# anands-repo/hello

Measured on AMD Instinct MI355X. Metric: candidate sites/sec (whole node), higher is better.
Workload: dtype f32

## Files before the change

hello_amd/compiler.py:

```python
from __future__ import annotations

from dataclasses import dataclass, field
from typing import Dict, List, Optional, Tuple

import numpy as np

from . import netspec as ns
from . import weights as wts

ROWS_READS0, ROWS_READS1, ROWS_ALLELES, ROWS_SITES = 0, 1, 2, 3
SEG_R0A, SEG_R1A, SEG_AS = 0, 1, 2
BUF_NONE, BUF_READS0, BUF_READS1, BUF_REF, BUF_FIRST_SCRATCH = -1, 0, 1, 2, 3
OP_XATTN_FRONT = 11
(OP_CONV1D, OP_MAXPOOL, OP_SEGSUM, OP_MIX, OP_HEAD, OP_CONCAT, OP_ADD, OP_READCONV_FUSED, OP_LAYERNORM,
 OP_COMPRESSOR_FUSED) = range(1, 11)
FLAG_RELU, FLAG_SRC_U8, FLAG_SOFTMAX, FLAG_MIX_REST, FLAG_SOFTPLUS, FLAG_WINOGRAD, FLAG_BF16X3, FLAG_BF16X3_32 = 1, 2, 4, 8, 16, 32, 64, 128
FLAG_LANE_SHIFT, MAX_LANES = 8, 8
OP_NAMES = {1: "conv1d", 2: "maxpool", 3: "segsum", 4: "mix", 5: "head", 6: "concat", 7: "add",
            8: "readconv_fused", 9: "layernorm", 10: "compressor_fused", 11: "xattn_front"}


@dataclass
class Value:
    vid: int
    domain: int
    length: int
    channels: int
    u8: bool = False

    @property
    def floats_per_row(self):
        return self.length * self.channels


@dataclass
class Op:
    kind: int
    domain: int
    src0: int = BUF_NONE
    src1: int = BUF_NONE
    dst: int = BUF_NONE
    res: int = BUF_NONE
    cin: int = 0
    cout: int = 0
    k: int = 0
    stride: int = 1
    pad: int = 0
    lin: int = 0
    lout: int = 0
    flags: int = 0
    seg: int = 0
    c1: int = 0
    a0: float = 0.0
    a1: float = 0.0
    w_off: int = 0
    b_off: int = 0
    name: str = ""
    macs_per_row: int = 0
    exec_macs_per_row: float = 0.0


@dataclass
class Program:
    spec_name: str
    window: int
    channels0: int
    channels1: int
    n_experts: int
    has_meta: bool
    uses_ref: bool
    ops: List[Op]
    buffers: List[Tuple[int, int]]
    weights: np.ndarray
    fused_read_convolver: bool = False
    fused_compressor: bool = False
    winograd: bool = False
    arithmetic: str = "fp32"
    n_lanes: int = 1

    def describe(self) -> str:
        lines = [f"program {self.spec_name}: {len(self.ops)} ops, {len(self.buffers)} buffers, "
                 f"{self.weights.nbytes / 1e6:.2f} MB weights"]
        for i, o in enumerate(self.ops):
            lines.append(f"  {i:3d} {OP_NAMES[o.kind]:14s} dom={o.domain} {o.src0}->{o.dst} "
                         f"cin={o.cin} cout={o.cout} k={o.k} s={o.stride} L {o.lin}->{o.lout} {o.name}")
        return "\n".join(lines)


class _WeightBlob:
    def __init__(self):
        self.parts: List[np.ndarray] = []
        self.size = 0

    def add(self, arr: np.ndarray) -> int:
        arr = np.ascontiguousarray(arr, dtype=np.float32).ravel()
        pad = (-self.size) % 4
        if pad:
            self.parts.append(np.zeros(pad, np.float32))
            self.size += pad
        off = self.size
        self.parts.append(arr)
        self.size += arr.size
        return off

    def finish(self) -> np.ndarray:
        return np.concatenate(self.parts) if self.parts else np.zeros(0, np.float32)


def grouped_native(node) -> bool:
    return (node.groups > 1 and node.cin % node.groups == 0 and node.cout % node.groups == 0
            and (node.cout // node.groups) % 128 == 0 and (node.cin // node.groups) % 16 == 0)


def pack_conv(w: np.ndarray, b: np.ndarray, groups: int = 1, expand: bool = True):
    cout, cg, k = w.shape
    cin = cg * groups if expand else cg
    dense = np.zeros((cout, cin, k), np.float32)
    og = cout // groups
    if expand:
        for g in range(groups):
            dense[g * og:(g + 1) * og, g * cg:(g + 1) * cg] = w[g * og:(g + 1) * og]
    else:
        dense[:] = w
    kreal = k * cin
    kpad = -(-kreal // 32) * 32
    cpad = -(-cout // 32) * 32
    packed = np.zeros((cpad, kpad), np.float32)
    packed[:cout, :kreal] = dense.transpose(0, 2, 1).reshape(cout, kreal)
    bias = np.zeros(cpad, np.float32)
    bias[:cout] = b
    return packed, bias


def winograd_outputs_per_tile(length: int) -> int:
    return 3 if length % 3 == 0 else 2


from .readconv_pack import winograd_taps_f33


def pack_conv_winograd(w: np.ndarray, b: np.ndarray, length: int):
    from .readconv_pack import winograd_taps
    cout, cin, k = w.shape
    assert k == 3 and cin % 8 == 0
    u = winograd_taps_f33(w) if winograd_outputs_per_tile(length) == 3 else winograd_taps(w)
    t = u.shape[-1]
    packed = u.reshape(cout, cin // 8, 8, t).transpose(0, 1, 3, 2).reshape(cout, t * cin)
    return np.ascontiguousarray(packed, dtype=np.float32), b.astype(np.float32)


def _canonical_read_convolver_extras(nodes, cin, act="relu") -> int:
    try:
        ref = ns.read_convolver("x", in_channels=cin, act=act)
    except Exception:
        return -1

    def sig(n):
        if isinstance(n, ns.Conv):
            return ("c", n.cin, n.cout, n.k, n.stride, n.pad, n.groups, n.act, n.norm == "ln")
        if isinstance(n, ns.MaxPool):
            return ("p", n.k, n.stride, n.pad)
        if isinstance(n, ns.Residual):
            return ("r", tuple(sig(m) for m in n.body), tuple(sig(m) for m in n.shortcut))
        return ("?", type(n).__name__)

    if len(nodes) < len(ref) or cin not in (6, 7):
        return -1
    if not all(sig(a) == sig(b) for a, b in zip(nodes, ref)):
        return -1
    extras = nodes[len(ref):]
    if not all(sig(x) == sig(ref[-1]) for x in extras):
        return -1
    return len(extras)


def _is_canonical_read_convolver(nodes, cin) -> bool:
    return _canonical_read_convolver_extras(nodes, cin) == 0


ARITHMETICS = ("fp32", "bf16x3", "bf16x3+32")


class _Lowering:
    def __init__(self, spec: ns.ModelSpec, state, fused: bool, winograd: bool = True, arithmetic: str = "fp32"):
        if arithmetic not in ARITHMETICS:
            raise ValueError(f"arithmetic must be one of {ARITHMETICS}, not {arithmetic!r}")
        self.arithmetic = arithmetic
        self.used_bf16x3 = False
        self.used_xattn_front = False
        self.spec = spec
        self.state = state
        self.folded = wts.fold(spec, state)
        self.fused = fused
        self.winograd = bool(winograd)
        self.ops: List[Op] = []
        self.values: Dict[int, Value] = {}
        self.blob = _WeightBlob()
        self.next_vid = 1000
        self.used_fused = False
        self.used_fused_compressor = False
        self.uses_ref = False

    def new(self, domain, length, channels) -> Value:
        v = Value(self.next_vid, domain, length, channels)
        self.values[v.vid] = v
        self.next_vid += 1
        return v

    def input(self, buf, domain, length, channels) -> Value:
        v = Value(buf, domain, length, channels, u8=True)
        self.values[buf] = v
        return v

    @staticmethod
    def _winograd_ok(node: ns.Conv, x: Value) -> bool:
        return (node.k == 3 and node.stride == 1 and node.pad == 1 and (node.groups == 1 or grouped_native(node))
                and node.dilation == 1 and not x.u8 and node.cin % 8 == 0 and node.cout % 64 == 0)

    def conv(self, node: ns.Conv, x: Value, res: Optional[Value] = None) -> Value:
        if node.act not in ("relu", "none", "softplus"):
            raise NotImplementedError(f"activation {node.act!r} is not implemented by the HIP engine")
        if node.dilation != 1:
            raise NotImplementedError("dilated convs are not implemented by the HIP engine")
        assert x.channels == node.cin, (node.key, x.channels, node.cin)
        w, b = self.folded[node.key]
        wino = self.winograd and self._winograd_ok(node, x)
        native = grouped_native(node) and not x.u8
        packed, bias = (pack_conv_winograd(w, b, x.length) if wino else pack_conv(w, b, node.groups, expand=not native))
        lout = ns.out_length([node], x.length)
        m = winograd_outputs_per_tile(lout)
        y = self.new(x.domain, lout, node.cout)
        act_flag = {"relu": FLAG_RELU, "softplus": FLAG_SOFTPLUS, "none": 0}[node.act]
        layer_norm = node.norm == "ln"
        self.ops.append(Op(
            OP_CONV1D, x.domain, src0=x.vid, dst=y.vid, res=res.vid if (res is not None and not layer_norm) else BUF_NONE,
            cin=node.cin, cout=node.cout, k=node.k, stride=node.stride, pad=node.pad,
            lin=x.length, lout=lout,
            flags=(0 if layer_norm else act_flag) | (FLAG_SRC_U8 if x.u8 else 0) | (FLAG_WINOGRAD if wino else 0),
            c1=node.groups if native else 0,
            w_off=self.blob.add(packed), b_off=self.blob.add(bias), name=node.key,
            macs_per_row=lout * node.cout * (node.cin // node.groups) * node.k,
            exec_macs_per_row=float(-(-lout // m) * (m + 2) * node.cout * (node.cin // node.groups)) if wino else 0.0))
        if layer_norm:
            gamma, beta, eps = wts.layer_norm_params(node, self.state)
            z = self.new(x.domain, lout, node.cout)
            self.ops.append(Op(OP_LAYERNORM, x.domain, src0=y.vid, dst=z.vid, res=res.vid if res is not None else BUF_NONE,
                               cin=node.cout, cout=node.cout, lin=lout, lout=lout, flags=act_flag, a0=float(eps),
                               w_off=self.blob.add(gamma), b_off=self.blob.add(beta), name=node.bn_key + ".normer"))
            return z
        return y

    def net(self, nodes, x, head_slot: Optional[int] = None, softmax=False):
        from . import readconv_pack
        if (self.fused is True and self.winograd and isinstance(x, Value) and not x.u8 and (x.length, x.channels) == (36, 64)
                and readconv_pack.compressor_blocks(nodes) in readconv_pack.COMPRESSOR_BLOCKS):
            blocks = readconv_pack.compressor_blocks(nodes)
            y = self.new(x.domain, 18, 128)
            w_off = self.blob.add(readconv_pack.pack_compressor(nodes, self.folded))
            self.ops.append(Op(OP_COMPRESSOR_FUSED, x.domain, src0=x.vid, dst=y.vid, cin=64, cout=128, k=blocks, lin=36, lout=18,
                               flags=FLAG_WINOGRAD | FLAG_RELU, w_off=w_off, b_off=w_off, name=nodes[0].key.rsplit(".network", 1)[0],
                               macs_per_row=ns.macs(nodes, 36), exec_macs_per_row=readconv_pack.compressor_executed_macs(blocks)))
            self.used_fused_compressor = True
            return y
        front = readconv_pack.xattn_front_match(nodes) if (self.fused is True and self.winograd and isinstance(x, tuple)) else None
        if front is not None:
            allele, sites = x
            site = sites[front[0].pick]
            if (site is not None and (allele.length, allele.channels) == (18, 128) and allele.domain == ROWS_ALLELES
                    and site.domain == ROWS_SITES):
                mix, conv11, blk = front
                y2, sc = self.new(ROWS_ALLELES, 9, 256), self.new(ROWS_ALLELES, 9, 256)
                w_off = self.blob.add(readconv_pack.pack_xattn_front(conv11, blk, self.folded))
                self.ops.append(Op(OP_XATTN_FRONT, ROWS_ALLELES, src0=allele.vid, src1=site.vid, dst=y2.vid, res=sc.vid,
                                   cin=128, cout=256, k=3, stride=2, pad=1, lin=18, lout=9, flags=FLAG_RELU, seg=SEG_AS,
                                   a0=float(mix.coeffs[0]), a1=float(mix.coeffs[1]), w_off=w_off, b_off=w_off,
                                   name=conv11.key.rsplit(".network", 1)[0] + ".front",
                                   macs_per_row=ns.macs([conv11], 18) + ns.macs([blk.body[0]], 18) + ns.macs(blk.shortcut, 18),
                                   exec_macs_per_row=readconv_pack.xattn_front_executed_macs()))
                self.used_xattn_front = True
                x = self.conv(blk.body[1], y2, res=sc)
                nodes = nodes[3:]
        for node in nodes:
            if isinstance(node, ns.Conv):
                x = self.conv(node, x)
            elif isinstance(node, ns.MaxPool):
                lout = ns.out_length([node], x.length)
                y = self.new(x.domain, lout, x.channels)
                self.ops.append(Op(OP_MAXPOOL, x.domain, src0=x.vid, dst=y.vid, cin=x.channels,
                                   cout=x.channels, k=node.k, stride=node.stride, pad=node.pad,
                                   lin=x.length, lout=lout))
                x = y
            elif isinstance(node, ns.Residual):
                short = self.net(node.shortcut, x) if node.shortcut else x
                h = x
                for i, sub in enumerate(node.body):
                    last = i == len(node.body) - 1
                    if not isinstance(sub, ns.Conv):
                        raise NotImplementedError("residual bodies must be conv stacks")
                    h = self.conv(sub, h, res=short if last else None)
                x = h
            elif isinstance(node, ns.Head):
                w, b = self.folded[node.key]
                assert head_slot is not None
                self.ops.append(Op(OP_HEAD, x.domain, src0=x.vid, dst=head_slot, cin=x.channels,
                                   cout=node.cout, lin=x.length, lout=1,
                                   flags=FLAG_SOFTMAX if softmax else 0,
                                   w_off=self.blob.add(w), b_off=self.blob.add(b), name=node.key,
                                   macs_per_row=node.cin * node.cout))
                x = None
            elif isinstance(node, ns.Mix):
                allele, sites = x
                site = sites[node.pick]
                assert site is not None and site.domain == ROWS_SITES and allele.domain == ROWS_ALLELES
                y = self.new(ROWS_ALLELES, allele.length, allele.channels)
# ... 27 lines not shown
    def add(self, a: Value, b: Value) -> Value:
        y = self.new(a.domain, a.length, a.channels)
        self.ops.append(Op(OP_ADD, a.domain, src0=a.vid, src1=b.vid, dst=y.vid, cin=a.channels,
                           lin=a.length, lout=a.length))
        return y

    def read_frames(self, tech: int, stem: str = "read_convolver", suffix: str = "") -> Value:
        spec = self.spec
        name = f"{stem}{tech}{suffix}"
        nodes = spec.nets[name]
        cin = spec.channels[tech]
        buf = BUF_READS0 if tech == 0 else BUF_READS1
        dom = ROWS_READS0 if tech == 0 else ROWS_READS1
        seg = SEG_R0A if tech == 0 else SEG_R1A
        x = self.input(buf, dom, spec.window, cin)
        from . import readconv_pack
        extras = _canonical_read_convolver_extras(nodes, cin)
        softplus = False
        if extras < 0 and _canonical_read_convolver_extras(nodes, cin, "softplus") == 0:
            extras, softplus = 0, True
        fusable = (self.fused and readconv_pack.AVAILABLE and extras in readconv_pack.EXTRA_BLOCKS
                   and spec.window in readconv_pack.WINDOWS)
        if fusable and (spec.window != 150 or softplus):
            fusable = self.fused is True and self.winograd and extras == 0 and not (softplus and spec.window != 150)
        wide_blocks = readconv_pack.wide_trunk_nodes(nodes, cin)
        if (self.fused in (True, "trunk") and self.winograd and spec.window == 150 and wide_blocks is not None
                and readconv_pack.AVAILABLE):
            y = self.new(ROWS_ALLELES, 36, 128)
            w_off = self.blob.add(readconv_pack.pack_wide(nodes, wide_blocks, self.folded))
            if self.fused == "trunk":
                pooled = self.net(nodes[:readconv_pack.TRUNK_FIRST_NODE], x)
                assert (pooled.length, pooled.channels) == (71, 64)
                self.ops.append(Op(OP_READCONV_FUSED, ROWS_ALLELES, src0=pooled.vid, dst=y.vid, cin=64, cout=128, k=0, lin=71,
                                   lout=36, seg=seg, w_off=w_off, b_off=w_off, name=name + ".trunk", flags=FLAG_WINOGRAD,
                                   macs_per_row=ns.macs(wide_blocks, 71),
                                   exec_macs_per_row=readconv_pack.wide_trunk_executed_macs()))
            else:
                self.ops.append(Op(OP_READCONV_FUSED, ROWS_ALLELES, src0=buf, dst=y.vid, cin=cin, cout=128, k=0, lin=spec.window,
                                   lout=36, seg=seg, w_off=w_off, b_off=w_off, name=name, flags=FLAG_SRC_U8 | FLAG_WINOGRAD,
                                   macs_per_row=ns.macs(nodes, spec.window),
                                   exec_macs_per_row=readconv_pack.wide_executed_macs(cin)))
            self.used_fused = True
            return y
        if fusable:
            _, l1, _, l2, _, _ = readconv_pack.geometry(spec.window)
            y = self.new(ROWS_ALLELES, l2, 64)
            packed = readconv_pack.pack(nodes, self.folded, cin, winograd=self.winograd, window=spec.window)
            wflag = FLAG_WINOGRAD if self.winograd else 0
            if (self.arithmetic != "fp32" and self.fused is True and self.winograd and spec.window == 150 and extras == 0
                    and not softplus):
                packed = np.concatenate([packed, readconv_pack.pack_bf16x3(nodes, self.folded)])
                wflag |= FLAG_BF16X3 | (FLAG_BF16X3_32 if "+32" in self.arithmetic else 0)
                self.used_bf16x3 = True
            w_off = self.blob.add(packed)
            if self.fused == "trunk":
                pooled = self.net(nodes[:readconv_pack.TRUNK_FIRST_NODE], x)
                assert (pooled.length, pooled.channels) == (l1, 32)
                self.ops.append(Op(OP_READCONV_FUSED, ROWS_ALLELES, src0=pooled.vid, dst=y.vid, cin=32, cout=64,
                                   k=extras, lin=l1, lout=l2, seg=seg, w_off=w_off, b_off=w_off, name=name + ".trunk",
                                   flags=wflag,
                                   macs_per_row=ns.macs(nodes[readconv_pack.TRUNK_FIRST_NODE:], l1)))
            else:
                self.ops.append(Op(OP_READCONV_FUSED, ROWS_ALLELES, src0=buf, dst=y.vid, cin=cin, cout=64,
                                   k=extras, lin=spec.window, lout=l2, seg=seg, w_off=w_off, b_off=w_off, name=name,
                                   flags=FLAG_SRC_U8 | wflag | (FLAG_SOFTPLUS if softplus else 0),
                                   macs_per_row=ns.macs(nodes, spec.window),
                                   exec_macs_per_row=readconv_pack.executed_macs_per_read(self.winograd, extras,
                                                                                          spec.window)))
            self.used_fused = True
            return y
        return self.segsum(self.net(nodes, x), seg)

    def compress_and_predict(self, frames: Value, idx: int, slot: Optional[int]):
        spec = self.spec
        comp = spec.nets[f"compressor{idx}"]
        ca = self.net(comp, frames)
        xattn = f"xattn{idx}"
        needs_cs0 = spec.has(xattn) and any(isinstance(n, ns.Mix) and n.pick == 0 for n in spec.nets[xattn])
        cs0 = self.net(comp, self.segsum(frames, SEG_AS)) if needs_cs0 else None
        cs1 = self.segsum(ca, SEG_AS)
        if spec.has(xattn):
            self.net(spec.nets[xattn], (ca, (cs0, cs1)), head_slot=slot)
        return (cs0, cs1), ca

    def lower_merged(self):
        spec = self.spec
        hybrid = spec.has("readConv1")
        additive = spec.use_additive
        if hybrid and not additive:
            raise ValueError("hybrid MoEMergedAdvanced with useAdditive=False: the reference's own forward raises on it "
                             "(MixtureOfExpertsAdvanced.py:436)")

        def mix(allele: Value, site: Value, a0, a1, flags=0) -> Value:
            x = self.new(ROWS_ALLELES, allele.length, allele.channels)
            self.ops.append(Op(OP_MIX, ROWS_ALLELES, src0=allele.vid, src1=site.vid, dst=x.vid,
                               cin=allele.channels, lin=allele.length, lout=allele.length,
                               a0=a0, a1=a1, seg=SEG_AS, flags=flags))
            return x

        def expert(idx, allele: Value, site: Value):
            from . import readconv_pack
            nodes = spec.nets[f"expert{idx}"]
            front = (readconv_pack.xattn_front_match(nodes, mixed_ahead=True)
                     if (additive and self.fused is True and self.winograd
                         and (allele.length, allele.channels) == (18, 128)) else None)
            if front is not None:
                _, conv11, blk = front
                y2, sc = self.new(ROWS_ALLELES, 9, 256), self.new(ROWS_ALLELES, 9, 256)
                w_off = self.blob.add(readconv_pack.pack_xattn_front(conv11, blk, self.folded))
                self.ops.append(Op(OP_XATTN_FRONT, ROWS_ALLELES, src0=allele.vid, src1=site.vid, dst=y2.vid, res=sc.vid,
                                   cin=128, cout=256, k=3, stride=2, pad=1, lin=18, lout=9, flags=FLAG_RELU | FLAG_MIX_REST, seg=SEG_AS,
                                   a0=2.0, a1=-1.0, w_off=w_off, b_off=w_off, name=conv11.key.rsplit(".network", 1)[0] + ".front",
                                   macs_per_row=ns.macs([conv11], 18) + ns.macs([blk.body[0]], 18) + ns.macs(blk.shortcut, 18),
                                   exec_macs_per_row=readconv_pack.xattn_front_executed_macs()))
                self.used_xattn_front = True
                self.net(nodes[2:], self.conv(blk.body[1], y2, res=sc), head_slot=idx)
                return
            if additive:
                x = mix(allele, site, 2.0, -1.0, FLAG_MIX_REST)
            else:
                rest = mix(allele, site, -1.0, 1.0)
# ... 170 lines not shown
        ready = [i for i in range(n) if i not in done and preds[i] <= done]
        pick = max(ready, key=lambda i: (bottom[i], -i))
        done.add(pick)
        order.append(pick)
    return [ops[i] for i in order]


def _allocate(ops: List[Op], values: Dict[int, Value], reuse: bool = True):
    last_use: Dict[int, int] = {}
    for i, o in enumerate(ops):
        for v in (o.src0, o.src1, o.res):
            if v >= 1000:
                last_use[v] = i
    phys: List[Tuple[int, int]] = [(0, 0)] * BUF_FIRST_SCRATCH
    free: Dict[int, List[int]] = {d: [] for d in range(4)}
    assigned: Dict[int, int] = {}
    def place(vid):
        v = values[vid]
        need = v.floats_per_row
        pool = free[v.domain]
        if pool:
            fits = [p for p in pool if phys[p][1] >= need]
            pick = min(fits, key=lambda p: phys[p][1]) if fits else max(pool, key=lambda p: phys[p][1])
            pool.remove(pick)
            phys[pick] = (v.domain, max(phys[pick][1], need))
        else:
            pick = len(phys)
            phys.append((v.domain, need))
        assigned[vid] = pick

    for i, o in enumerate(ops):
        if o.kind == OP_XATTN_FRONT:
            place(o.dst)
            place(o.res)
            for vsrc in {o.src0, o.src1}:
                if reuse and vsrc >= 1000 and last_use.get(vsrc) == i and vsrc in assigned:
                    free[values[vsrc].domain].append(assigned[vsrc])
            continue
        if o.kind != OP_HEAD:
            place(o.dst)
        for vsrc in {o.src0, o.src1, o.res}:
            if reuse and vsrc >= 1000 and last_use.get(vsrc) == i and vsrc in assigned:
                free[values[vsrc].domain].append(assigned[vsrc])
    for o in ops:
        o.src0 = assigned.get(o.src0, o.src0)
        o.src1 = assigned.get(o.src1, o.src1)
        o.res = assigned.get(o.res, o.res)
        if o.kind != OP_HEAD:
            o.dst = assigned[o.dst]
    return phys


def compile_model(spec: ns.ModelSpec, state, fused: bool = True, winograd: bool = True, arithmetic: str = "fp32",
                  fold_site_sums: bool = True, lanes: bool = False) -> Program:
    low = _Lowering(spec, state, fused, winograd, arithmetic)
    n_experts, has_meta = low.lower()
    if arithmetic != "fp32" and not low.used_bf16x3:
        raise ValueError("arithmetic='bf16x3' / 'bf16x3+32' exists for the canonical 150 bp ReLU read convolver in the whole-kernel "
                         "Winograd form (fused=True, winograd=True): this model / these options do not run it")
    if fold_site_sums:
        low.ops = _fold_site_sums(low.ops)
        low.ops = _fold_concats(low.ops)
    n_lanes = assign_lanes(low.ops) if lanes else 1
    if n_lanes > 1:
        low.ops = schedule_lanes(low.ops)
    buffers = _allocate(low.ops, low.values, reuse=n_lanes == 1)
    return Program(
        spec_name=spec.name, window=spec.window, channels0=spec.channels[0],
        channels1=spec.channels[1] if spec.hybrid_inputs else 0,
        n_experts=n_experts, has_meta=has_meta, uses_ref=low.uses_ref, ops=low.ops,
        buffers=buffers, weights=low.blob.finish(), fused_read_convolver=low.used_fused,
        fused_compressor=low.used_fused_compressor, winograd=low.winograd, arithmetic=arithmetic, n_lanes=n_lanes)
```

hello_amd/csrc/engine.hip:

```cpp
#include <hip/hip_runtime.h>

#include <cstdarg>
#include <cstdio>
#include <cstring>
#include <new>
#include <stdexcept>
#include <string>
#include <vector>

#include "../../include/hello_mi355x.h"
#include "kernels.h"

namespace {

thread_local std::string g_last_error;

int fail(int code, const char* fmt, ...) {
    char buf[512];
    va_list ap;
    va_start(ap, fmt);
    vsnprintf(buf, sizeof(buf), fmt, ap);
    va_end(ap);
    g_last_error = buf;
    return code;
// ... 305 lines not shown
                                             "and cout / groups a multiple of 128 (a workgroup's channel block lies inside one group)", i, o.c1);
            if ((o.lin + 2 * o.pad - o.k) / o.stride + 1 != o.lout)
                return fail(HELLO_ERR_MODEL, "op %d: lout inconsistent", i);
            if (o.flags & (HELLO_FLAG_BF16X3 | HELLO_FLAG_BF16X3_32))
                return fail(HELLO_ERR_MODEL, "op %d: the bf16x3 arithmetic modes exist for the fused read convolver only (ABI 2 "
                                             "dropped the split-operand CONV1D)", i);
        }
        if (o.kind == HELLO_OP_COMPRESSOR_FUSED &&
            !(o.cin == 64 && o.cout == 128 && o.lin == 36 && o.lout == 18 && hello::compressor_supports_blocks(o.k) &&
              (o.flags & HELLO_FLAG_WINOGRAD) && o.w_off >= 0))
            return fail(HELLO_ERR_MODEL, "op %d: the fused compressor maps [36][64] rows to [18][128] with 2 to 4 identity blocks, "
                                         "Winograd form", i);
        if (o.kind == HELLO_OP_XATTN_FRONT &&
            !(o.domain == HELLO_ROWS_ALLELES && o.cin == 128 && o.cout == 256 && o.lin == 18 && o.lout == 9 && o.k == 3 && o.stride == 2 &&
              o.pad == 1 && o.seg == HELLO_SEG_ALLELES_TO_SITES && o.w_off >= 0 &&
              o.res >= HELLO_BUF_FIRST_SCRATCH && o.res != o.dst && o.res != o.src0 && o.res != o.src1 && o.dst != o.src0 && o.dst != o.src1 &&
              d->buffers[o.res].domain == HELLO_ROWS_ALLELES && d->buffers[o.res].floats_per_row >= 9 * 256 &&
              (o.src1 == HELLO_BUF_NONE || d->buffers[o.src1].domain == HELLO_ROWS_SITES)))
            return fail(HELLO_ERR_MODEL, "op %d: the fused expert front maps [18][128] allele rows (src0) and site rows (src1, or none: "
                                         "the sites' sums of src0) to two distinct [9][256] allele buffers, dst and res", i);
        if (o.kind == HELLO_OP_LAYERNORM && (o.cin <= 0 || o.cin > 512 || o.lin <= 0 || o.w_off < 0 || o.b_off < 0 || !(o.a0 > 0.f)))
            return fail(HELLO_ERR_MODEL, "op %d: bad LayerNorm (1..512 channels, eps > 0)", i);
        if ((o.kind == HELLO_OP_SEGSUM || o.kind == HELLO_OP_MIX || o.kind == HELLO_OP_READCONV_FUSED) &&
            (o.seg < 0 || o.seg > 2))
            return fail(HELLO_ERR_MODEL, "op %d: bad segment kind", i);
        if (o.kind == HELLO_OP_CONV1D && (o.flags & HELLO_FLAG_WINOGRAD) &&
            !(o.k == 3 && o.stride == 1 && o.pad == 1 && o.lin == o.lout && !(o.flags & HELLO_FLAG_SRC_U8) &&
              o.cin % 8 == 0 && o.cout % 64 == 0))
            return fail(HELLO_ERR_MODEL, "op %d: this convolution has no Winograd form (needs k 3, stride 1, pad 1, "
                                         "cin %% 8 == 0, cout %% 64 == 0, float input)", i);
        if (o.kind == HELLO_OP_READCONV_FUSED) {
            if (!hello::readconv_supports_window(d->window))
                return fail(HELLO_ERR_MODEL, "op %d: the fused read convolver takes 150 or 250 bp windows, not %d", i, d->window);
            const bool wide = o.cout == 128;
            const bool wide_shape = (o.flags & HELLO_FLAG_SRC_U8) ? ((o.cin == 6 || o.cin == 7) && o.lin == 150) : (o.cin == 64 && o.lin == 71);
            if (wide && !(d->window == 150 && wide_shape && o.lout == 36 && o.k == 0 && (o.flags & HELLO_FLAG_WINOGRAD) &&
                          !(o.flags & HELLO_FLAG_SOFTPLUS)))
                return fail(HELLO_ERR_MODEL, "op %d: the wide read convolver maps pileup bytes [150][6|7] or pooled [71][64] rows to "
                                             "[36][128] frames (150 bp, Winograd form, ReLU, no extra blocks)", i);
            if (!wide && (o.lout != hello::readconv_frame_rows(d->window) || o.cout != 64))
                return fail(HELLO_ERR_MODEL, "op %d: the fused read convolver yields [%d][64] frames", i,
                            hello::readconv_frame_rows(d->window));
            if ((o.flags & HELLO_FLAG_SOFTPLUS) &&
                !(d->window == 150 && (o.flags & HELLO_FLAG_WINOGRAD) && (o.flags & HELLO_FLAG_SRC_U8) && o.k == 0))
                return fail(HELLO_ERR_MODEL, "op %d: the Softplus read convolver runs whole (from the bytes), in Winograd "
                                             "form, on 150 bp windows, without extra blocks", i);
            if ((o.flags & HELLO_FLAG_BF16X3_32) && !(o.flags & HELLO_FLAG_BF16X3))
                return fail(HELLO_ERR_MODEL, "op %d: HELLO_FLAG_BF16X3_32 extends HELLO_FLAG_BF16X3", i);
            if ((o.flags & HELLO_FLAG_BF16X3) &&
                !(d->window == 150 && !wide && (o.flags & HELLO_FLAG_WINOGRAD) && (o.flags & HELLO_FLAG_SRC_U8) && o.k == 0 &&
                  !(o.flags & HELLO_FLAG_SOFTPLUS)))
                return fail(HELLO_ERR_MODEL, "op %d: the bf16x3 arithmetic mode exists for the canonical read convolver run whole "
                                             "(from the bytes) in Winograd form on 150 bp windows, ReLU, without extra blocks", i);
            if (d->window == 250 && !((o.flags & HELLO_FLAG_WINOGRAD) && (o.flags & HELLO_FLAG_SRC_U8) && o.k == 0))
                return fail(HELLO_ERR_MODEL, "op %d: 250 bp windows run whole (from the bytes), in Winograd form, "
                                             "without extra blocks", i);
        }
        if (o.kind == HELLO_OP_READCONV_FUSED && !hello::readconv_supports_extra_blocks(o.k))
            return fail(HELLO_ERR_MODEL, "op %d: the fused read convolver takes 0 or 2 extra blocks (k), got %d", i, o.k);
        if (int rc = validate_op_buffers(d, o, i)) return rc;
    }
    return 0;
}

struct LanePlan {
    int n_lanes = 1;
    std::vector<std::vector<int>> op_waits;
    std::vector<int> lane_tail;
    std::vector<char> read_elsewhere;
};

int lane_of_op(const hello_op& o) { return (o.flags & HELLO_FLAG_LANE_MASK) >> HELLO_FLAG_LANE_SHIFT; }

int analyse_lanes(const hello_model_desc* d, LanePlan& plan) {
    const int n_ops = d->n_ops;
    auto lane_of = [&](int i) { return lane_of_op(d->ops[i]); };
    for (int i = 0; i < n_ops; ++i) plan.n_lanes = lane_of(i) + 1 > plan.n_lanes ? lane_of(i) + 1 : plan.n_lanes;
    if (plan.n_lanes == 1) return 0;
    std::vector<int> writer(d->n_buffers, -1);
    plan.op_waits.assign(n_ops, {});
    plan.lane_tail.assign(plan.n_lanes, -1);
    plan.read_elsewhere.assign(n_ops, 0);
    for (int i = 0; i < n_ops; ++i) {
        const hello_op& o = d->ops[i];
        const bool front = o.kind == HELLO_OP_XATTN_FRONT;
        const int reads[3] = {o.src0, o.src1, front ? HELLO_BUF_NONE : o.res};
        for (int b : reads) {
            if (b < HELLO_BUF_FIRST_SCRATCH) continue;
            const int w = writer[b];
            if (w < 0) return fail(HELLO_ERR_MODEL, "laned program: op %d reads buffer %d before any op wrote it", i, b);
            if (lane_of(w) != lane_of(i)) {
                plan.op_waits[i].push_back(w);
                plan.read_elsewhere[w] = 1;
            }
        }
        const int writes[2] = {o.kind == HELLO_OP_HEAD ? HELLO_BUF_NONE : o.dst, front ? o.res : HELLO_BUF_NONE};
        for (int b : writes) {
            if (b < HELLO_BUF_FIRST_SCRATCH) continue;
            if (writer[b] >= 0)
                return fail(HELLO_ERR_MODEL, "laned program: ops %d and %d both write buffer %d (a program with lanes may not reuse buffers)", writer[b], i, b);
            writer[b] = i;
        }
        plan.lane_tail[lane_of(i)] = i;
    }
    return 0;
}
// ... 6 lines not shown
}

}

extern "C" {

const char* hello_last_error(void) { return g_last_error.c_str(); }
int hello_abi_version(void) { return HELLO_ABI_VERSION; }

int hello_engine_create(const hello_model_desc* desc, const void* folded_weights, size_t nbytes,
                        int hip_device, hello_engine** out) try {
    if (!out) return fail(HELLO_ERR_ARG, "out is NULL");
    *out = nullptr;
    if (int rc = validate_model(desc)) return rc;
    LanePlan lanes;
    if (int rc = analyse_lanes(desc, lanes)) return rc;
    if (!folded_weights || nbytes == 0 || (nbytes % 4)) return fail(HELLO_ERR_ARG, "bad weight blob");
    int n_dev = 0;
    if (hipGetDeviceCount(&n_dev) != hipSuccess || n_dev <= 0)
        return fail(HELLO_ERR_NOGPU, "no HIP device visible: the HIP engine cannot run");
    if (hip_device < 0 || hip_device >= n_dev) return fail(HELLO_ERR_ARG, "device %d out of range", hip_device);
    hipDeviceProp_t prop;
    HIP_TRY(hipGetDeviceProperties(&prop, hip_device));
    if (strncmp(prop.gcnArchName, "gfx950", 6) != 0)
        return fail(HELLO_ERR_NOGPU, "device %d is %s; this engine is built for gfx950 only", hip_device,
                    prop.gcnArchName);
    HIP_TRY(hipSetDevice(hip_device));

    hello_engine* e = new hello_engine();
    e->device = hip_device;
    e->desc = *desc;
    e->ops.assign(desc->ops, desc->ops + desc->n_ops);
    e->buffers.assign(desc->buffers, desc->buffers + desc->n_buffers);
    e->desc.ops = e->ops.data();
    e->desc.buffers = e->buffers.data();
    e->n_weight_floats = nbytes / 4;
    for (const hello_op& o : e->ops) {
        size_t w_end = 0, b_end = 0;
        if (o.kind == HELLO_OP_CONV1D) {
            const bool wino = (o.flags & HELLO_FLAG_WINOGRAD) != 0;
            const size_t cpad = wino ? (size_t)o.cout : (size_t)((o.cout + 31) / 32) * 32;
            const int cing = o.cin / (o.c1 > 1 ? o.c1 : 1);
            const size_t kpad = wino ? (size_t)(hello::conv1d_wino_outputs_per_tile(o.lin) + 2) * cing
                                     : (size_t)((o.k * cing + 31) / 32) * 32;
            w_end = (size_t)o.w_off + cpad * kpad;
            b_end = (size_t)o.b_off + cpad;
        } else if (o.kind == HELLO_OP_HEAD) {
            w_end = (size_t)o.w_off + (size_t)o.cout * o.cin;
            b_end = (size_t)o.b_off + o.cout;
        } else if (o.kind == HELLO_OP_LAYERNORM) {
            w_end = (size_t)o.w_off + o.cin;
            b_end = (size_t)o.b_off + o.cin;
        } else if (o.kind == HELLO_OP_COMPRESSOR_FUSED) {
            w_end = (size_t)o.w_off + hello::compressor_weight_floats(o.k);
            b_end = (size_t)o.b_off;
        } else if (o.kind == HELLO_OP_XATTN_FRONT) {
            w_end = (size_t)o.w_off + hello::xattn_front_weight_floats();
            b_end = (size_t)o.b_off;
        } else if (o.kind == HELLO_OP_READCONV_FUSED) {
            w_end = (size_t)o.w_off + (o.cout == 128 ? hello::readconv_wide_weight_floats()
                                                     : hello::readconv_weight_floats(o.k, (o.flags & HELLO_FLAG_WINOGRAD) != 0, desc->window));
            b_end = (size_t)o.b_off;
            if (o.cout == 128) e->wide_trunk[o.seg == HELLO_SEG_READS1_TO_ALLELES ? 1 : 0] = true;
        }
        if (w_end > e->n_weight_floats || b_end > e->n_weight_floats) {
            delete e;
            return fail(HELLO_ERR_MODEL, "a weight block runs past the end of the blob");
        }
    }
    e->scratch.resize(desc->n_buffers);
    hipError_t err = hipMalloc((void**)&e->d_weights, nbytes);
    if (err == hipSuccess) err = hipMemcpy(e->d_weights, folded_weights, nbytes, hipMemcpyHostToDevice);
    if (err == hipSuccess) err = hipStreamCreateWithFlags(&e->own_stream, hipStreamNonBlocking);
    if (err == hipSuccess) err = hipEventCreateWithFlags(&e->ev_staged, hipEventDisableTiming);
    if (err == hipSuccess) err = hipEventCreate(&e->ev_start);
    if (err == hipSuccess) err = hipEventCreate(&e->ev_stop);
    if (err != hipSuccess) {
        hello_engine_destroy(e);
        return fail(HELLO_ERR_HIP, "engine setup failed: %s", hipGetErrorString(err));
    }
    const int n_ops = (int)e->ops.size();
    e->n_lanes = lanes.n_lanes;
    e->partial_of.assign(n_ops, -1);
    int n_partial = e->n_lanes > 1 ? 0 : 2;
    for (int i = 0; i < n_ops; ++i)
        if (e->ops[i].kind == HELLO_OP_READCONV_FUSED)
            e->partial_of[i] = e->n_lanes > 1 ? n_partial++ : (e->ops[i].seg == HELLO_SEG_READS1_TO_ALLELES ? 1 : 0);
    e->d_partial.resize(n_partial);
    if (e->n_lanes > 1) {
        auto lane_of = [&](int i) { return lane_of_op(e->ops[i]); };
        e->op_waits = std::move(lanes.op_waits);
        e->lane_tail = std::move(lanes.lane_tail);
        const std::vector<char>& read_elsewhere = lanes.read_elsewhere;
        e->op_done.assign(n_ops, nullptr);
        e->lane_streams.assign(e->n_lanes, nullptr);
        for (int l = 1; l < e->n_lanes && err == hipSuccess; ++l) err = hipStreamCreateWithFlags(&e->lane_streams[l], hipStreamNonBlocking);
        for (int i = 0; i < n_ops && err == hipSuccess; ++i)
            if (read_elsewhere[i] || (lane_of(i) > 0 && e->lane_tail[lane_of(i)] == i)) err = hipEventCreateWithFlags(&e->op_done[i], hipEventDisableTiming);
        if (err == hipSuccess) err = hipEventCreateWithFlags(&e->ev_lanes_go, hipEventDisableTiming);
        if (err != hipSuccess) {
            hello_engine_destroy(e);
            return fail(HELLO_ERR_HIP, "lane setup failed: %s", hipGetErrorString(err));
        }
    }
    *out = e;
    return HELLO_OK;
} catch (...) {
    return hello::exception_status("hello_engine_create");
}

void hello_engine_destroy(hello_engine* e) {
    if (!e) return;
    (void)hipSetDevice(e->device);
    (void)hipDeviceSynchronize();
// ... 455 lines not shown
                if (!a.src) return fail(HELLO_ERR_ARG, "op %d reads an input the caller did not supply", op_index);
                if (a.wino) {
                    a.kpad = (hello::conv1d_wino_outputs_per_tile(o.lin) + 2) * a.cin;
                    a.cout_pad = o.cout;
                    if (!hello::conv1d_wino_supported(a))
                        return fail(HELLO_ERR_MODEL, "op %d: this convolution has no Winograd form", op_index);
                    HIP_TRY(hello::launch_conv1d_wino(a, stream));
                    break;
                }
                HIP_TRY(hello::launch_conv1d(a, stream));
                break;
            }
            case HELLO_OP_MAXPOOL:
                HIP_TRY(hello::launch_maxpool((const float*)ptr(o.src0), (float*)ptr(o.dst), rows, o.lin, o.lout,
                                              o.cin, o.k, o.stride, o.pad, stream));
                break;
            case HELLO_OP_SEGSUM: {
                const int32_t* off = o.seg == HELLO_SEG_READS0_TO_ALLELES ? e->roff0
                                     : o.seg == HELLO_SEG_READS1_TO_ALLELES ? e->roff1 : e->aoff;
                HIP_TRY(hello::launch_segsum((const float*)ptr(o.src0), (float*)ptr(o.dst), off, (int)rows,
                                             o.lin * o.cin, stream));
                break;
            }
            case HELLO_OP_MIX:
                HIP_TRY(hello::launch_mix((const float*)ptr(o.src0), (const float*)ptr(o.src1), (float*)ptr(o.dst),
                                          e->site_of_allele, rows, o.lin * o.cin, o.a0, o.a1,
                                          (o.flags & HELLO_FLAG_MIX_REST) != 0, stream));
                break;
            case HELLO_OP_HEAD: {
                float* outp;
                long long so, sr;
                if (o.dst == 3) { outp = d_meta; so = 1; sr = 3; }
                else { outp = d_logits + (long long)o.dst * A; so = 0; sr = 1; }
                HIP_TRY(hello::launch_head((const float*)ptr(o.src0), e->d_weights + o.w_off, e->d_weights + o.b_off,
                                           outp, rows, o.lin, o.cin, o.cout, so, sr,
                                           (o.flags & HELLO_FLAG_SOFTMAX) ? 1 : 0, stream));
                break;
            }
            case HELLO_OP_CONCAT:
                HIP_TRY(hello::launch_concat((const float*)ptr(o.src0), (const float*)ptr(o.src1), (float*)ptr(o.dst),
                                             rows * o.lin, o.cin, o.c1, stream));
                break;
            case HELLO_OP_ADD:
                HIP_TRY(hello::launch_add((const float*)ptr(o.src0), (const float*)ptr(o.src1), (float*)ptr(o.dst),
                                          rows * o.lin * o.cin, stream));
                break;
            case HELLO_OP_COMPRESSOR_FUSED: {
                hello::CompressorArgs a{};
                a.frames = (const float*)ptr(o.src0);
                a.dst = (float*)ptr(o.dst);
                a.w = e->d_weights + o.w_off;
                a.n_items = rows;
                a.blocks = o.k;
                HIP_TRY(hello::launch_compressor_fused(a, stream));
                break;
            }
            case HELLO_OP_XATTN_FRONT: {
                hello::XattnFrontArgs a{};
                a.alleles = (const float*)ptr(o.src0);
                a.sites = o.src1 == HELLO_BUF_NONE ? nullptr : (const float*)ptr(o.src1);
                a.owner = e->site_of_allele;
                a.site_off = e->aoff;
                a.y2 = (float*)ptr(o.dst);
                a.sc = (float*)ptr(o.res);
                a.w = e->d_weights + o.w_off;
                a.n_items = rows;
                a.a0 = o.a0;
                a.a1 = o.a1;
                a.rest = (o.flags & HELLO_FLAG_MIX_REST) ? 1 : 0;
                HIP_TRY(hello::launch_xattn_front(a, stream));
                break;
            }
            case HELLO_OP_LAYERNORM:
                HIP_TRY(hello::launch_layernorm((const float*)ptr(o.src0), (const float*)ptr(o.res), (float*)ptr(o.dst),
                                                e->d_weights + o.w_off, e->d_weights + o.b_off, rows * o.lin, o.cin, o.a0,
                                                (o.flags & HELLO_FLAG_RELU) ? 1 : ((o.flags & HELLO_FLAG_SOFTPLUS) ? 2 : 0), stream));
                break;
            case HELLO_OP_READCONV_FUSED: {
                const bool t1 = o.seg == HELLO_SEG_READS1_TO_ALLELES;
                hello::ReadConvArgs a{};
                if (o.flags & HELLO_FLAG_SRC_U8) {
                    a.reads = (const uint8_t*)ptr(o.src0);
                    a.channels = o.cin;
                } else {
                    a.pooled = (const float*)ptr(o.src0);
                }
                if (!ptr(o.src0)) return fail(HELLO_ERR_ARG, "op %d reads an input the caller did not supply", op_index);
                a.w = e->d_weights + o.w_off;
                a.partial = (float*)e->d_partial[e->partial_of[op_index]].p;
                a.allele_of_read = t1 ? e->allele_of_read1 : e->allele_of_read0;
                a.slot_of_group = t1 ? e->group_slot1 : e->group_slot0;
                a.n_reads = t1 ? R1 : R0;
                a.window = d.window;
                a.softplus = (o.flags & HELLO_FLAG_SOFTPLUS) ? 1 : 0;
                a.extra_blocks = o.k;
                a.winograd = (o.flags & HELLO_FLAG_WINOGRAD) ? 1 : 0;
                a.bf16x3 = (o.flags & HELLO_FLAG_BF16X3) ? ((o.flags & HELLO_FLAG_BF16X3_32) ? 2 : 1) : 0;
                const bool wide = o.cout == 128;
                if ((size_t)o.w_off + (wide ? hello::readconv_wide_weight_floats() : hello::readconv_weight_floats(o.k, a.winograd, d.window)) +
                        (a.bf16x3 ? hello::readconv_bf16x3_extra_floats(o.k) : 0) > e->n_weight_floats)
                    return fail(HELLO_ERR_MODEL, "op %d: fused read-convolver weight block truncated", op_index);
                {
                    const hello::ReadConvPlan& plan = t1 ? e->plan1 : e->plan0;
                    const int G = hello::readconv_reads_per_group(d.window);
                    const long long total = a.n_reads;
                    const long long bulk_reads = plan.rest_wgs ? plan.bulk_wgs * plan.groups_per_wg * G : total;
                    a.groups_per_wg = plan.groups_per_wg;
                    a.n_reads = bulk_reads;
                    int32_t stamp_lay[5] = {0, 0, 0, 0, 0};
                    const int stamp_waves = hello::readconv_stamp_waves();
                    if ((e->stamp_mode & 1) && !t1 && total > 0) {
                        if (wide || !a.reads) return fail(HELLO_ERR_ARG, "stamps: the canonical fused read convolver from the bytes only");
                        const long long wgs = plan.rest_wgs ? plan.bulk_wgs + plan.rest_wgs : (long long)((total + (long long)G * plan.groups_per_wg - 1) / ((long long)G * plan.groups_per_wg));
                        const int slots = hello::readconv_stamp_slots();
                        const size_t bytes = (size_t)wgs * stamp_waves * plan.groups_per_wg * slots * sizeof(uint64_t);
                        if (bytes > e->d_stamps.cap) {
                            HIP_TRY(hipStreamSynchronize(stream));
                            if (e->d_stamps.ensure(bytes)) return fail(HELLO_ERR_HIP, "device allocation of %zu bytes failed", bytes);
                        }
                        HIP_TRY(hipMemsetAsync(e->d_stamps.p, 0, bytes, stream));
                        a.stamps = (unsigned long long*)e->d_stamps.p;
                        a.stamp_groups = plan.groups_per_wg;
                        a.stamp_mode = e->stamp_mode;
                        const int32_t lay[5] = {(int32_t)wgs, stamp_waves, plan.groups_per_wg, slots, (int32_t)(plan.rest_wgs ? plan.bulk_wgs : wgs)};
                        for (int i = 0; i < 5; ++i) stamp_lay[i] = lay[i];
                        e->stamp_layout[0] = 0;
                    }
                    HIP_TRY(wide ? hello::launch_readconv_wide(a, stream) : hello::launch_readconv_fused(a, stream));
                    if (plan.rest_wgs) {
                        hello::ReadConvArgs b = a;
                        if (b.stamps) b.stamps += (size_t)plan.bulk_wgs * stamp_waves * plan.groups_per_wg * hello::readconv_stamp_slots();
                        if (b.reads) b.reads += bulk_reads * d.window * o.cin;
                        else b.pooled += bulk_reads * (long long)o.lin * o.cin;
                        b.allele_of_read += bulk_reads;
                        b.slot_of_group += plan.bulk_wgs;
                        b.groups_per_wg = 1;
                        b.n_reads = total - bulk_reads;
                        HIP_TRY(wide ? hello::launch_readconv_wide(b, stream) : hello::launch_readconv_fused(b, stream));
                    }
                    if (a.stamps)
                        for (int i = 0; i < 5; ++i) e->stamp_layout[i] = stamp_lay[i];
                }
                HIP_TRY(hello::launch_readconv_finalize((const float*)e->d_partial[e->partial_of[op_index]].p, t1 ? e->slot_off1 : e->slot_off0,
                                                        (float*)ptr(o.dst), A, o.lout, o.cout, stream));
                break;
            }
        }
        if (op_index == e->debug_op) {
            const size_t per_row = o.kind == HELLO_OP_CONCAT ? (size_t)o.lout * (o.cin + o.c1)
                                   : (o.kind == HELLO_OP_CONV1D || o.kind == HELLO_OP_READCONV_FUSED || o.kind == HELLO_OP_COMPRESSOR_FUSED || o.kind == HELLO_OP_XATTN_FRONT) ? (size_t)o.lout * o.cout
                                   : (o.kind == HELLO_OP_MAXPOOL ? (size_t)o.lout * o.cin : (size_t)o.lin * o.cin);
            const size_t n = (size_t)rows * per_row;
            if (n * sizeof(float) > e->d_debug.cap) {
// ... 327 lines not shown
```

hello_amd/csrc/kernels.h:

```cpp
#pragma once
#include <hip/hip_runtime.h>
#include <stdint.h>

namespace hello {

int device_cus();

struct ConvArgs {
    const void* src;
    const float* src2;
    int split;
    float* dst;
    const float* res;
    const float* w;
    const float* bias;
    long long m_total;
    int lin, lout, cin, cout, k, stride, pad;
    int cin_stride;
    int groups;
    int kpad;
    int cout_pad;
    int relu;
    int src_u8;
    unsigned wino_rows;
    int wino;
};
hipError_t launch_conv1d(const ConvArgs& a, hipStream_t stream);
bool conv1d_wino_supported(const ConvArgs& a);
int conv1d_wino_outputs_per_tile(int length);
hipError_t launch_conv1d_wino(const ConvArgs& a, hipStream_t stream);

hipError_t launch_maxpool(const float* src, float* dst, long long rows, int lin, int lout, int c,
                          int k, int stride, int pad, hipStream_t stream);

hipError_t launch_segsum(const float* src, float* dst, const int32_t* off, int n_seg, int row_floats,
                         hipStream_t stream);

hipError_t launch_mix(const float* src0, const float* src1, float* dst, const int32_t* owner,
                      long long rows, int row_floats, float a0, float a1, bool rest, hipStream_t stream);

hipError_t launch_head(const float* src, const float* w, const float* b, float* out, long long rows,
                       int len, int c, int cout, long long out_stride_o, long long out_stride_row,
                       int softmax, hipStream_t stream);

hipError_t launch_concat(const float* src0, const float* src1, float* dst, long long rows_x_len, int c0,
                         int c1, hipStream_t stream);

hipError_t launch_add(const float* src0, const float* src1, float* dst, long long n, hipStream_t stream);

hipError_t launch_layernorm(const float* src, const float* res, float* dst, const float* gamma, const float* beta,
                            long long positions, int c, float eps, int act, hipStream_t stream);

hipError_t launch_rcl_to_rlc(const uint8_t* src, uint8_t* dst, long long rows, int len, int c,
                             hipStream_t stream);

hipError_t launch_posteriors(const float* logits, const float* meta, const int32_t* allele_off,
                             const int64_t* pair_off, int n_sites, long long n_alleles, int n_experts,
                             long long n_pairs_total, float* out, hipStream_t stream);

struct ReadConvArgs {
    const uint8_t* reads;
    const float* pooled;
    int channels;
    const float* w;
    float* partial;
    const int32_t* allele_of_read;
    const int32_t* slot_of_group;
    int groups_per_wg;
    long long n_reads;
    int extra_blocks;
    int winograd;
    int window;
    int softplus;
    int bf16x3;
    unsigned long long* stamps;
    int stamp_groups;
    int stamp_mode;
};
int readconv_stamp_slots();
int readconv_stamp_waves();
bool readconv_supports_window(int window);
int readconv_reads_per_group(int window);
int readconv_frame_rows(int window);
int readconv_groups_per_workgroup(long long n_reads, int window);
struct ReadConvPlan {
    int groups_per_wg;
    long long bulk_wgs;
    long long rest_wgs;
};
ReadConvPlan readconv_plan(long long n_reads, int window);
ReadConvPlan readconv_wide_plan(long long n_reads);
int readconv_weight_floats(int extra_blocks, bool winograd, int window);
int readconv_bf16x3_extra_floats(int extra_blocks);
bool readconv_supports_extra_blocks(int extra_blocks);
hipError_t launch_readconv_fused(const ReadConvArgs& a, hipStream_t stream);
hipError_t launch_readconv_finalize(const float* partial, const int32_t* slot_off, float* frames, int n_alleles,
                                    int frame_rows, int channels, hipStream_t stream);
int readconv_wide_weight_floats();
int readconv_wide_reads_per_group();
hipError_t launch_readconv_wide(const ReadConvArgs& a, hipStream_t stream);

struct CompressorArgs {
    const float* frames;
    float* dst;
    const float* w;
    long long n_items;
    int blocks;
    int items_per_wg;
};
int small_launch_items_per_wg(long long n_items, int most);
int compressor_weight_floats(int blocks);
bool compressor_supports_blocks(int blocks);
hipError_t launch_compressor_fused(const CompressorArgs& a, hipStream_t stream);

struct XattnFrontArgs {
    const float* alleles;
    const float* sites;
    const int32_t* owner;
    const int32_t* site_off;
    float* y2;
    float* sc;
    const float* w;
    long long n_items;
    float a0, a1;
    int rest;
    int items_per_wg;
};
int xattn_front_weight_floats();
hipError_t launch_xattn_front(const XattnFrontArgs& a, hipStream_t stream);

struct FeaturizeArgs {
    const uint8_t* bases;
    const uint8_t* quals;
    const long long* read_off;
    const uint32_t* cigars;
    const long long* cigar_off;
    const long long* ref_start;
    const uint8_t* mapq;
    const int8_t* orientation;
    const uint8_t* hp;
    const int32_t* site_of_read;
    const uint8_t* ref;
    const long long* ref_off;
    const long long* window_start;
    const long long* asm_start;
    const long long* asm_stop;
    long long n_reads;
    int length, channels;
    uint8_t* out;
};
hipError_t launch_featurize(const FeaturizeArgs& a, hipStream_t stream);

struct SupportArgs {
    const long long* cigar_off;
    const uint8_t* mapq;
    const int8_t* orientation;
    const long long* allele_off;
    long long n_reads, n_alleles;
    long long* out;
};
hipError_t launch_allele_support(const SupportArgs& a, hipStream_t stream);

struct EvidenceArgs {
    const uint8_t* quals;
// ... 16 lines not shown
```

hello_amd/csrc/readconv_fused.hip:

```cpp
#include <cstdlib>
#include <type_traits>

#include "kernels.h"

namespace hello {

typedef float f32x4 __attribute__((ext_vector_type(4)));

namespace rc {

constexpr int S1_STEPS = 6;
template <bool WINO, bool F33 = false>
struct Offs {
    static constexpr int KT = WINO ? 4 : 3;
    static constexpr int W3232 = 2 * KT * 2 * 256, W3264 = 4 * 3 * 2 * 256, W3264S = 4 * 1 * 2 * 256;
    static constexpr int W6464 = 4 * KT * 4 * 256;
    static constexpr int W6464D = F33 ? 4 * 5 * 4 * 256 : W6464;
    static constexpr int W3232D = F33 ? 2 * 5 * 2 * 256 : W3232;
    static constexpr int OFF_B = 0;
    static constexpr int OFF_C1 = OFF_B + 6 * (W3232D + 32);
    static constexpr int OFF_SC = OFF_C1 + W3264 + 64;
    static constexpr int OFF_C2 = OFF_SC + W3264S + 64;
    static constexpr int OFF_D = OFF_C2 + W6464D + 64;
    static constexpr int W_TRUNK = OFF_D + 6 * (W6464D + 64);
// ... 3 lines not shown
    static constexpr int W_TOTAL = OFF_S3 + 2 * KT * 256 + 32;
    static constexpr int off_d(int blk) {
        return blk < 3 ? OFF_D + 2 * blk * (W6464D + 64) : W_TOTAL + 2 * (blk - 3) * (W6464D + 64);
    }
};

constexpr int cmax(int a, int b) { return a > b ? a : b; }
constexpr int STAMP_SLOTS = 48;

enum { ACT_RELU = 0, ACT_SOFTPLUS = 1 };
template <int G_, int NW_, int WIN_ = 150, int ACT_ = ACT_RELU>
struct Cfg {
    static constexpr int ACT = ACT_;
    static __device__ __forceinline__ float act(float x) {
        if constexpr (ACT_ == ACT_RELU) return fmaxf(x, 0.f);
        else return x > 20.f ? x : __logf(1.f + __expf(x));
    }
    static constexpr int G = G_;
    static constexpr int NW = NW_;
    static constexpr int THREADS = 64 * NW_;
    static constexpr int WINDOW = WIN_;
    static constexpr int L1 = (WIN_ - 6 - 3) / 2 + 1;
    static constexpr int RS1 = L1 + 1;
    static constexpr int L2 = (L1 - 1) / 2 + 1;
    static constexpr bool COMPACT = (L2 % 2) == 0;
    static constexpr int RS2 = COMPACT ? L2 : L2 + 1;
    static constexpr bool F33 = COMPACT && (RS2 % 3) == 0 && ((RS2 * G_) % 48) == 0;
    static constexpr bool F33_32 = F33 && (RS1 % 3) == 0 && ((RS1 * G_) % 96) == 0;
    static constexpr int NTT = (L1 + 6) / 7;
    static constexpr int WPR = NW_ / G_;
    static_assert(RS1 % 2 == 0 && RS2 % 2 == 0 && NW_ % G_ == 0, "pairs of rows must not straddle reads");
    static constexpr int T1 = (RS1 * G_ + 15) / 16;
    static constexpr int T2 = (RS2 * G_ + 15) / 16;
    static constexpr int ROWS1 = RS1 * G_ + 1;
    static constexpr int ROWS2 = RS2 * G_ + 2;
    static constexpr int SB = G_;
    static constexpr int SROWS = WIN_ * SB;
    static constexpr int ST12 = ((SROWS + 15) / 16 + 3) / 4 * 4;
    static constexpr int BUF_FLOATS = cmax(cmax(ROWS2 * 64, ROWS1 * 32), SROWS * 16);
    static constexpr int U8_BYTES = ((ST12 * 16 + 8) * 7 + 15) / 16 * 16;

    static constexpr int NSREG = cmax((T2 * 4 + NW_ - 1) / NW_, 2 * ((RS2 * G_ / 2 + 15) / 16));
    static constexpr int LDS_BYTES = cmax(2 * BUF_FLOATS * 4 + 64 + U8_BYTES,
                                          BUF_FLOATS * 4 + (T2 * 16 + 2) * 256 + 64);
};
}

using Geometry = rc::Cfg<4, 4, 150>;
using Geometry250 = rc::Cfg<2, 4, 250>;
using GeometrySoftplus = rc::Cfg<4, 4, 150, rc::ACT_SOFTPLUS>;
static_assert(Geometry::F33 && GeometrySoftplus::F33 && !Geometry250::F33, "weight packing rule of readconv_pack.py");
static_assert(Geometry::F33_32 && GeometrySoftplus::F33_32, "weight packing rule of readconv_pack.py");
int readconv_bf16x3_extra_floats(int extra_blocks) { return (1 + 2 * (3 + extra_blocks)) * 12288 + 6 * 3072; }
int readconv_weight_floats(int extra_blocks, bool winograd, int window) {
    if (!winograd) return rc::Offs<false>::off_d(3 + extra_blocks);
    return window == 150 ? rc::Offs<true, true>::off_d(3 + extra_blocks) : rc::Offs<true>::off_d(3 + extra_blocks);
}
bool readconv_supports_extra_blocks(int extra_blocks) { return extra_blocks == 0 || extra_blocks == 2; }

bool readconv_supports_window(int window) { return window == 150 || window == 250; }
int readconv_reads_per_group(int window) { return window == 250 ? Geometry250::G : Geometry::G; }
int readconv_stamp_slots() { return rc::STAMP_SLOTS; }
int readconv_stamp_waves() { return Geometry::NW; }
int readconv_frame_rows(int window) { return window == 250 ? Geometry250::L2 : Geometry::L2; }
int readconv_groups_per_workgroup(long long n_reads, int window) {
    const long long slots = 2LL * device_cus();
    const int G = readconv_reads_per_group(window);
    const long long groups = (n_reads + G - 1) / G;
    int best = 1;
    double best_cost = 1e300;
    for (int n = 1; n <= 8; ++n) {
        const long long wgs = (groups + n - 1) / n;
        const double cost = (double)((wgs + slots - 1) / slots) * n * (n > 1 ? 0.988 : 1.0);
        if (cost <= best_cost) {
            best_cost = cost;
            best = n;
        }
    }
    return best;
}

ReadConvPlan readconv_plan(long long n_reads, int window) {
    const long long slots = 2LL * device_cus();
    const int G = readconv_reads_per_group(window);
    const long long groups = (n_reads + G - 1) / G;
    ReadConvPlan best{1, groups, 0};
    double best_cost = 1e300;
    for (int n = 1; n <= 8; ++n) {
        const long long rounds = (groups / n) / slots;
        if (rounds == 0) continue;
        const long long bulk = rounds * slots, rest = groups - bulk * n;
        const double cost = (double)rounds * n * (n > 1 ? 0.988 : 1.0) + (double)((rest + slots - 1) / slots);
        if (cost <= best_cost) {
            best_cost = cost;
            best = ReadConvPlan{n, bulk, rest};
        }
    }
    if (best_cost == 1e300) {
        const int n = readconv_groups_per_workgroup(n_reads, window);
        best = ReadConvPlan{n, (groups + n - 1) / n, 0};
    }
    return best;
}

template <int C>
__device__ __forceinline__ int swz(int row) {
// ... 516 lines not shown
        *(f32x4*)(po[2] + kk * TOFF) = y2;
    };
    issue(std::integral_constant<int, 0>{});
    static_for<0, NU>([&](auto uc) {
        constexpr int u = decltype(uc)::value;
        constexpr int m = u / NT, k = u % NT;
        if constexpr (u + 1 < NU) {
            if (!PARTIAL || (u + 1) % NT < live_tiles) issue(std::integral_constant<int, u + 1>{});
        }
        if constexpr (k == 0) {
            const float* nw = (m + 1 < M) ? wl + (m + 1) * 5 * 256 : next_wl;
            if constexpr (m + 1 < M || !LAST) {
#pragma unroll
                for (int c = 0; c < 5; ++c) w[(m + 1) & 1][c] = *(const f32x4*)(nw + c * 256);
            }
        }
        __builtin_amdgcn_sched_barrier(0);
        if constexpr (m == M - 1 && k >= 1) {
            if (!PARTIAL || k - 1 < live_tiles) epi_store(std::integral_constant<int, (k >= 1 ? k - 1 : 0)>{});
        }
        if (!PARTIAL || k < live_tiles) {
            const f32x4(&d)[5] = ring[u & 1];
            const f32x4 s31 = pk_sub(d[3], d[1]);
            const f32x4 t02 = pk_sub(d[0], d[2]), p12 = pk_add(d[1], d[2]), m12 = pk_sub(d[1], d[2]), t42 = pk_sub(d[4], d[2]);
            const f32x4 two = {2.f, 2.f, 2.f, 2.f}, three = {3.f, 3.f, 3.f, 3.f};
            const f32x4 v0 = __builtin_elementwise_fma(t02, two, s31);
            const f32x4 v1 = pk_sub(s31, p12);
            const f32x4 v2 = __builtin_elementwise_fma(m12, three, s31);
            const f32x4 v4 = __builtin_elementwise_fma(s31, -two, t42);
            asm volatile("s_nop 1");
            __builtin_amdgcn_sched_barrier(0);
            f32x4(&a)[5] = acc[k];
            const f32x4(&wm)[5] = w[m & 1];
#pragma unroll
            for (int e = 0; e < 4; ++e) {
                const bool first = (m == 0) && (e == 0);
                a[0] = __builtin_amdgcn_mfma_f32_16x16x4f32(wm[0][e], v0[e], first ? zero4 : a[0], 0, 0, 0);
                a[1] = __builtin_amdgcn_mfma_f32_16x16x4f32(wm[1][e], v1[e], first ? b4 : a[1], 0, 0, 0);
                a[2] = __builtin_amdgcn_mfma_f32_16x16x4f32(wm[2][e], v2[e], first ? zero4 : a[2], 0, 0, 0);
                a[3] = __builtin_amdgcn_mfma_f32_16x16x4f32(wm[3][e], s31[e], first ? zero4 : a[3], 0, 0, 0);
                a[4] = __builtin_amdgcn_mfma_f32_16x16x4f32(wm[4][e], v4[e], first ? zero4 : a[4], 0, 0, 0);
            }
        }
        if constexpr (MODE == MODE_RESID_INPLACE && m == M - 1) {
#pragma unroll
            for (int r = 0; r < 3; ++r) res[r] = *(const f32x4*)(po[r] + k * TOFF);
        }
        if constexpr (u == NU - 1) {
            if (!PARTIAL || NT - 1 < live_tiles) epi_store(std::integral_constant<int, NT - 1>{});
        }
    });
}

enum { BF_PLAIN = 0, BF_RESID = 1 };
constexpr int BF16_DEPTH = 2;
constexpr bool BF16_DEFER = true;
template <class CF, int MODE, bool LAST, bool OUT_F32>
__device__ __forceinline__ void bf16x3_layer(const unsigned char* __restrict__ in, unsigned char* __restrict__ out,
                                             bf16x8 (&wh)[6], bf16x8 (&wl)[6], const unsigned short* __restrict__ next_w,
                                             const float* __restrict__ bias, f32x4 (&xres)[CF::NSREG], int wave, int lane) {
    constexpr int RS = CF::RS2, NT = RS * CF::G / 16, NU = NT * 6;
    static_assert(CF::COMPACT && (RS * CF::G) % 16 == 0 && CF::NW == 4 && NT <= CF::NSREG, "the compact 150 bp geometry");
    const int cb = wave, j = lane & 15, q = lane >> 4;
    const f32x4 b4 = *(const f32x4*)(bias + cb * 16 + 4 * q);
    const f32x4 zero4 = {0.f, 0.f, 0.f, 0.f};
    const unsigned char* ph[6];
    const unsigned char* pl[6];
#pragma unroll
    for (int s = 0; s < 6; ++s) {
        ph[s] = in + split_off(j + s / 2, 4 * (s & 1) + q, 0);
        pl[s] = in + split_off(j + s / 2, 4 * (s & 1) + q, 1);
    }
    const unsigned char* const zrow = in + 16 * q;
    constexpr int DEPTH = BF16_DEPTH;
    bf16x8 rh[DEPTH + 1], rl[DEPTH + 1];
    auto issue = [&](auto uc) {
        constexpr int u = decltype(uc)::value;
        constexpr int k = u / 6, s = u % 6, tap = s / 2;
        const unsigned char* a_h = ph[s] + k * 16 * 256;
        const unsigned char* a_l = pl[s] + k * 16 * 256;
        constexpr int first = ((16 * k + RS - 1) / RS) * RS - 16 * k, last = ((16 * k + RS) / RS) * RS - 1 - 16 * k;
        if constexpr (tap == 0 && 16 * k + first > 0 && first >= 0 && first < 16) {
            a_h = (j == first) ? zrow : a_h;
            a_l = (j == first) ? zrow : a_l;
        }
        if constexpr (tap == 2 && last < 16 && 16 * k + last < RS * CF::G - 1) {
            a_h = (j == last) ? zrow : a_h;
            a_l = (j == last) ? zrow : a_l;
        }
        rh[u % (DEPTH + 1)] = *(const bf16x8*)a_h;
        rl[u % (DEPTH + 1)] = *(const bf16x8*)a_l;
    };
    f32x4 acc_a[2] = {b4, b4}, acc_b[2] = {zero4, zero4};
    auto epilogue = [&](auto kc) {
        constexpr int k = decltype(kc)::value;
        f32x4 y;
#pragma unroll
        for (int e = 0; e < 4; ++e) y[e] = CF::act(acc_a[k & 1][e] + acc_b[k & 1][e]);
        if constexpr (MODE == BF_RESID) {
            y = y + xres[k];
            xres[k] = y;
        }
        if constexpr (OUT_F32) *(f32x4*)((float*)out + img_off<64, SW_3>(16 * k + j + 1, 4 * cb + q)) = y;
        else store_split(out, 16 * k + j + 1, 4 * cb + q, y);
        acc_a[k & 1] = b4;
        acc_b[k & 1] = zero4;
// ... 36 lines not shown
    for (int s = 0; s < 3; ++s) {
        ph[s] = in + 16 * pg * 128 + split_off32(j + s, q, 0);
        pl[s] = in + 16 * pg * 128 + split_off32(j + s, q, 1);
    }
    unsigned zmask = 0;
#pragma unroll
    for (int k = 0; k < NT; ++k) zmask |= ((((pg + 2 * k) * 16 + j) % RS) == RS - 1 ? 1u : 0u) << k;
    constexpr int DEPTH = BF16_DEPTH;
    bf16x8 rh[DEPTH + 1], rl[DEPTH + 1];
    auto issue = [&](auto uc) {
        constexpr int u = decltype(uc)::value;
        constexpr int k = u / 3, s = u % 3;
        rh[u % (DEPTH + 1)] = *(const bf16x8*)(ph[s] + k * 32 * 128);
        rl[u % (DEPTH + 1)] = *(const bf16x8*)(pl[s] + k * 32 * 128);
    };
    f32x4 acc_a[2] = {b4, b4}, acc_b[2] = {zero4, zero4};
    auto epilogue = [&](auto kc) {
        constexpr int k = decltype(kc)::value;
        f32x4 y;
#pragma unroll
        for (int e = 0; e < 4; ++e) y[e] = CF::act(acc_a[k & 1][e] + acc_b[k & 1][e]);
        if constexpr (MODE == BF_RESID) y = y + xres[k];
        if ((zmask >> k) & 1u) y = zero4;
        if constexpr (MODE == BF_RESID) xres[k] = y;
        const int row = 16 * (pg + 2 * k) + j + 1;
        if constexpr (OUT_F32) *(f32x4*)((float*)out + img_off<32, SW_W>(row, 4 * cb + q)) = y;
        else store_split32(out, row, 4 * cb + q, y);
        acc_a[k & 1] = b4;
        acc_b[k & 1] = zero4;
    };
    static_for<0, DEPTH>(issue);
    static_for<0, NU>([&](auto uc) {
        constexpr int u = decltype(uc)::value;
        constexpr int k = u / 3, s = u % 3;
        if constexpr (u + DEPTH < NU) issue(std::integral_constant<int, u + DEPTH>{});
        __builtin_amdgcn_sched_barrier(0);
        const bf16x8 xh = rh[u % (DEPTH + 1)], xl = rl[u % (DEPTH + 1)];
        acc_a[k & 1] = __builtin_amdgcn_mfma_f32_16x16x32_bf16(wh[s], xh, acc_a[k & 1], 0, 0, 0);
        acc_b[k & 1] = __builtin_amdgcn_mfma_f32_16x16x32_bf16(wh[s], xl, acc_b[k & 1], 0, 0, 0);
        acc_b[k & 1] = __builtin_amdgcn_mfma_f32_16x16x32_bf16(wl[s], xh, acc_b[k & 1], 0, 0, 0);
        if constexpr (!LAST && k == NT - 1) {
            wh[s] = *(const bf16x8*)(next_w + (s * 2) * 512);
            wl[s] = *(const bf16x8*)(next_w + (s * 2 + 1) * 512);
        }
        if constexpr (BF16_DEFER) {
            if constexpr (s == 1 && k >= 1) epilogue(std::integral_constant<int, (k >= 1 ? k - 1 : 0)>{});
            if constexpr (u == NU - 1) epilogue(std::integral_constant<int, NT - 1>{});
        } else if constexpr (u % (NU / NT) == NU / NT - 1) {
            epilogue(std::integral_constant<int, k>{});
        }
    });
}

template <class CF>
__device__ __forceinline__ void stem_conv1(const unsigned char* __restrict__ s_u8, float* __restrict__ c1,
                                           const float* __restrict__ W, int ch, float* __restrict__ dump, int wave,
                                           int lane) {
    using namespace rc;
    constexpr int NPAIR = CF::ST12 / 8;
    static_assert(CF::ST12 % 8 == 0, "stem tiles must split into pairs over 4 waves");
    const int j = lane & 15, q = lane >> 4;
    float w1[S1_STEPS];
#pragma unroll
    for (int s = 0; s < S1_STEPS; ++s) w1[s] = W[s * 64 + lane];
    const f32x4 b4 = *(const f32x4*)(W + S1_STEPS * 64 + 4 * q);
    const unsigned char* base = s_u8 + (16 * wave + j) * ch + q;
    const int tile_bytes = 16 * ch;
    unsigned char cur0[S1_STEPS], cur1[S1_STEPS], nxt0[S1_STEPS], nxt1[S1_STEPS];
#pragma unroll
    for (int s = 0; s < S1_STEPS; ++s) {
        cur0[s] = base[4 * s];
        cur1[s] = base[4 * tile_bytes + 4 * s];
    }
#pragma unroll
    for (int i = 0; i < NPAIR; ++i) {
        if (i + 1 < NPAIR) {
#pragma unroll
            for (int s = 0; s < S1_STEPS; ++s) {
                nxt0[s] = base[(8 * (i + 1)) * tile_bytes + 4 * s];
                nxt1[s] = base[(8 * (i + 1) + 4) * tile_bytes + 4 * s];
            }
        }
        __builtin_amdgcn_sched_barrier(0);
        f32x4 a0 = {0.f, 0.f, 0.f, 0.f}, a1 = {0.f, 0.f, 0.f, 0.f};
#pragma unroll
        for (int s = 0; s < S1_STEPS; ++s) {
            a0 = __builtin_amdgcn_mfma_f32_16x16x4f32(w1[s], (float)cur0[s], a0, 0, 0, 0);
            a1 = __builtin_amdgcn_mfma_f32_16x16x4f32(w1[s], (float)cur1[s], a1, 0, 0, 0);
        }
        const int r0 = 16 * (wave + 8 * i) + j, r1 = r0 + 64;
        f32x4 v0, v1;
#pragma unroll
        for (int e = 0; e < 4; ++e) {
            v0[e] = CF::act(a0[e] + b4[e]);
            v1[e] = CF::act(a1[e] + b4[e]);
        }
        *(f32x4*)(r0 < CF::SROWS ? c1 + r0 * 16 + 4 * (q ^ swz<16>(r0)) : dump) = v0;
        *(f32x4*)(r1 < CF::SROWS ? c1 + r1 * 16 + 4 * (q ^ swz<16>(r1)) : dump) = v1;
#pragma unroll
        for (int s = 0; s < S1_STEPS; ++s) {
            cur0[s] = nxt0[s];
            cur1[s] = nxt1[s];
        }
    }
}

template <class CF, int SOUT>
__device__ __forceinline__ void stem_conv3_pool(const float* __restrict__ in, float* __restrict__ out,
                                                const float* __restrict__ W3, float* __restrict__ dump, int wave,
                                                int lane, int n_here) {
    constexpr int WPR = CF::WPR;
    constexpr int NTT = CF::NTT / WPR;
    static_assert(CF::NTT % WPR == 0, "the pool tiles of a read must split evenly over its waves");
    const int j = lane & 15, q = lane >> 4;
    const int rd = wave / WPR, half = wave % WPR;
    f32x4 w[2][3];
#pragma unroll
    for (int blk = 0; blk < 2; ++blk)
#pragma unroll
        for (int tap = 0; tap < 3; ++tap) w[blk][tap] = *(const f32x4*)(W3 + ((blk * 3 + tap) * 64 + lane) * 4);
    f32x4 b4[2];
#pragma unroll
    for (int blk = 0; blk < 2; ++blk) b4[blk] = *(const f32x4*)(W3 + 2 * 3 * 256 + blk * 16 + 4 * q);
    const int lrow = rd * CF::WINDOW + 14 * half + j;
    const float* pin[8];
#pragma unroll
    for (int k = 0; k < 8; ++k) pin[k] = in + lrow * 16 + 4 * (q ^ (2 * (((lrow + k) >> 2) & 1)));
    const int orow = 1 + rd * CF::RS1 + 7 * half + (j >> 1);
    const bool lane_ok = ((j & 1) == 0) && (j <= 12) && (rd < n_here);
    const f32x4 zero4 = {0.f, 0.f, 0.f, 0.f};

    f32x4 ring[2][3];
    f32x4 acc[2][2][2];
    auto issue = [&](auto tc) {
        constexpr int tt = decltype(tc)::value;
#pragma unroll
        for (int tap = 0; tap < 3; ++tap) {
            constexpr int c0 = 14 * WPR * tt;
            ring[tt & 1][tap] = *(const f32x4*)(pin[(c0 + tap) & 7] + (c0 + tap) * 16);
        }
    };
    auto epilogue = [&](auto tc) {
        constexpr int tt = decltype(tc)::value;
        const int row = orow + 7 * WPR * tt;
        const bool ok = lane_ok && (row - 1 - rd * CF::RS1 < CF::L1);
#pragma unroll
        for (int blk = 0; blk < 2; ++blk) {
            const f32x4 sum = acc[tt & 1][blk][0] + acc[tt & 1][blk][1];
            f32x4 v;
#pragma unroll
            for (int e = 0; e < 4; ++e) {
                v[e] = CF::act(fmaxf(fmaxf(sum[e], row_shl(sum[e], 1)), row_shl(sum[e], 2)));
            }
// ... 121 lines not shown
    auto issue = [&](auto tc) {
        constexpr int k = decltype(tc)::value;
#pragma unroll
        for (int i = 0; i < 4; ++i) {
            constexpr int c0 = 30 * WPR * k;
            ring[k & 1][i] = *(const f32x4*)(pin[(c0 + i) & 7] + (c0 + i) * 16);
        }
    };
    auto epilogue = [&](auto tc) {
        constexpr int k = decltype(tc)::value;
        const int pos = opos + 15 * WPR * k;
        const bool ok = lane_ok && (pos < CF::L1);
#pragma unroll
        for (int blk = 0; blk < 2; ++blk) {
            const f32x4(&a)[4] = acc[k & 1][blk];
            const f32x4 y0 = (a[0] + a[1]) + a[2];
            const f32x4 y1 = (a[1] - a[2]) - a[3];
            f32x4 v;
#pragma unroll
            for (int e = 0; e < 4; ++e) v[e] = CF::act(fmaxf(fmaxf(y0[e], y1[e]), row_shl(y0[e], 1)));
            float* ptr = out + img_off<32, SOUT>(1 + rd * CF::RS1 + pos, 4 * blk + q);
            *(f32x4*)(ok ? ptr : dump) = v;
        }
    };
    issue(std::integral_constant<int, 0>{});
    static_for<0, NK>([&](auto tc) {
        constexpr int k = decltype(tc)::value;
        constexpr bool tail = (k == NK - 1) && (NTR % WPR != 0);
        if constexpr (k + 1 < NK) issue(std::integral_constant<int, k + 1>{});
        __builtin_amdgcn_sched_barrier(0);
        if constexpr (k >= 1) epilogue(std::integral_constant<int, (k >= 1 ? k - 1 : 0)>{});
        if (!tail || last_here) {
            const f32x4 d0 = ring[k & 1][0], d1 = ring[k & 1][1], d2 = ring[k & 1][2], d3 = ring[k & 1][3];
            const f32x4 t0 = pk_sub(d0, d2), t1 = pk_add(d1, d2), t2 = pk_sub(d2, d1), t3 = pk_sub(d1, d3);
            asm volatile("s_nop 1");
            __builtin_amdgcn_sched_barrier(0);
#pragma unroll
            for (int e = 0; e < 4; ++e)
#pragma unroll
                for (int blk = 0; blk < 2; ++blk) {
                    f32x4(&a)[4] = acc[k & 1][blk];
                    a[0] = __builtin_amdgcn_mfma_f32_16x16x4f32(w[blk][0][e], t0[e], e == 0 ? zero4 : a[0], 0, 0, 0);
                    a[1] = __builtin_amdgcn_mfma_f32_16x16x4f32(w[blk][1][e], t1[e], e == 0 ? b4[blk] : a[1], 0, 0, 0);
                    a[2] = __builtin_amdgcn_mfma_f32_16x16x4f32(w[blk][2][e], t2[e], e == 0 ? zero4 : a[2], 0, 0, 0);
                    a[3] = __builtin_amdgcn_mfma_f32_16x16x4f32(w[blk][3][e], t3[e], e == 0 ? zero4 : a[3], 0, 0, 0);
                }
        }
        if constexpr (k == NK - 1) {
            if (!tail || last_here) epilogue(std::integral_constant<int, NK - 1>{});
        }
    });
}

template <class CF, bool STEM, int NB64, bool WINO, bool BF16 = false, bool BF16_32 = false, bool STAMP = false>
__global__ __launch_bounds__(CF::THREADS, 2) void readconv_kernel(ReadConvArgs a) {
    using namespace rc;
    constexpr bool F33 = WINO && CF::F33;
    static_assert(!BF16 || (F33 && CF::ACT == ACT_RELU), "bf16x3: the 150 bp ReLU geometry of the Winograd kernel");
    static_assert(!BF16_32 || BF16, "the 32-channel split layers extend the bf16x3 mode");
    using O = Offs<WINO, F33>;
    constexpr int L1 = CF::L1, RS1 = CF::RS1, L2 = CF::L2, RS2 = CF::RS2;
    static_assert(CF::COMPACT || WINO, "the zero-row 64-channel geometry is implemented for the Winograd form only");
    constexpr int W3232 = O::W3232, W3264 = O::W3264, W3264S = O::W3264S, W6464 = O::W6464;
    constexpr int OFF_B = O::OFF_B, OFF_C1 = O::OFF_C1, OFF_SC = O::OFF_SC, OFF_C2 = O::OFF_C2;
    constexpr int OFF_S1 = O::OFF_S1, OFF_S2 = O::OFF_S2, OFF_S3 = O::OFF_S3;
    constexpr int SWX = WINO ? SW_W : SW_OLD;
    constexpr int NVA = WINO ? 8 : 6, NVB = WINO ? 16 : 12;
    constexpr int G = CF::G, T1 = CF::T1, T2 = CF::T2, BUF_FLOATS = CF::BUF_FLOATS, THREADS = CF::THREADS;
    static_assert(CF::NW == 4, "the layer schedule below maps 4 waves to (2 blocks x 2 groups) / (4 blocks)");
    extern __shared__ __attribute__((aligned(16))) float smem[];
    float* bufA = smem;
    float* bufB = smem + BUF_FLOATS;
    float* dump = smem + 2 * BUF_FLOATS + 12;
    unsigned char* s_u8 = (unsigned char*)(smem + 2 * BUF_FLOATS + 16);

    const int tid0 = threadIdx.x;
    const int wave0 = __builtin_amdgcn_readfirstlane(tid0 >> 6);
    const float* __restrict__ W = a.w;

    unsigned pad1 = 0, pad1f = 0;
    unsigned pad2 = 0, pad2w = 0;
    if (!CF::COMPACT) {
        const int j = tid0 & 15;
#pragma unroll
        for (int k = 0; k < T2; ++k) pad2 |= (((k * 16 + j) % RS2) >= L2 ? 1u : 0u) << k;
#pragma unroll
        for (int k = 0; k < (RS2 * G / 2 + 15) / 16; ++k) pad2w |= (((k * 16 + j) % (RS2 / 2)) == RS2 / 2 - 1 ? 1u : 0u) << k;
    }
    {
        const int j = tid0 & 15;
        const int pg1 = wave0 / 2;
        if (WINO) {
#pragma unroll
            for (int k = 0; k < (T1 / 2 + 1) / 2; ++k) {
                pad1 |= ((((pg1 + 2 * k) * 16 + j) % (RS1 / 2)) == RS1 / 2 - 1 ? 1u : 0u) << k;
                pad1f |= ((((1 - pg1 + 2 * k) * 16 + j) % (RS1 / 2)) == RS1 / 2 - 1 ? 1u : 0u) << k;
            }
        } else {
#pragma unroll
            for (int k = 0; k < T1 / 2; ++k) pad1 |= ((((pg1 + 2 * k) * 16 + j) % RS1) >= L1 ? 1u : 0u) << k;
        }
    }

    float* const X = STEM ? bufB : bufA;
    float* const H = STEM ? bufA : bufB;
    f32x4 sreg[CF::NSREG];
    f32x4 wA[NVA], wB[NVB], w2[2];
    f32x4 w3[2][5];
    f32x4 (&w6)[6] = reinterpret_cast<f32x4 (&)[6]>(wA);
    f32x4 (&w12)[12] = reinterpret_cast<f32x4 (&)[12]>(wB);
// ... 5 lines not shown
    constexpr int NF = (L2 * 16 + THREADS - 1) / THREADS;
    f32x4 carry[NF];
#pragma unroll
    for (int i = 0; i < NF; ++i) carry[i] = f32x4{0.f, 0.f, 0.f, 0.f};
    auto flush = [&]() {
#pragma unroll
        for (int i = 0; i < NF; ++i) {
            const int f = tid0 + THREADS * i;
            if (f < L2 * 16)
                *(f32x4*)(a.partial + ((long long)(slot0 + cur - first_allele) * L2 + (f >> 4)) * 64 + 4 * (f & 15)) = carry[i];
            carry[i] = f32x4{0.f, 0.f, 0.f, 0.f};
        }
    };

    for (int grp = 0; grp < a.groups_per_wg; ++grp) {
    int opaque_zero;
    asm volatile("s_mov_b32 %0, 0" : "=s"(opaque_zero));
    const int tid = tid0 + opaque_zero;
    const int wave = __builtin_amdgcn_readfirstlane(wave0 + opaque_zero);
    const int lane = tid & 63;
    const int cb2 = wave % 2, cb4 = wave;
    const long long read0 = wg_read0 + (long long)grp * G;
    if (read0 >= a.n_reads) break;
    unsigned long long* const stamp_base = STAMP ? a.stamps + (((long long)blockIdx.x * CF::NW + wave) * a.stamp_groups + grp) * STAMP_SLOTS : nullptr;
    auto stamp = [&](int slot) {
        if constexpr (STAMP) {
            const unsigned long long t = __builtin_amdgcn_s_memtime();
            if (grp < a.stamp_groups && lane == 0) stamp_base[slot] = t;
        }
    };
    auto barrier = [&](int id) {
        stamp(1 + 2 * id);
        __syncthreads();
        stamp(2 + 2 * id);
    };
    if constexpr (STAMP) {
        stamp(0);
        const unsigned long long rt = __builtin_amdgcn_s_memrealtime();
        const unsigned hw = __builtin_amdgcn_s_getreg((31 << 11) | 4), xcc = __builtin_amdgcn_s_getreg((31 << 11) | 20);
        if (grp < a.stamp_groups && lane == 0) {
            stamp_base[41] = (unsigned long long)hw | ((unsigned long long)xcc << 32);
            stamp_base[42] = rt;
        }
    }
    const int n_here = (int)((a.n_reads - read0) < G ? (a.n_reads - read0) : G);
    if constexpr (F33) {
        static_assert(!F33 || CF::F33_32, "the F(3,3) kernel runs its 32-channel blocks in F(3,3) form too");
#pragma unroll
        for (int c = 0; c < 5; ++c) w3[0][c] = *(const f32x4*)(W + OFF_B + cb2 * (10 * 256) + lane * 4 + c * 256);
    } else {
        load_weights<NVA>(wA, W + OFF_B, cb2, lane);
    }
    if (STEM) {
        const int ch = a.channels;
        const int n_bytes = n_here * CF::WINDOW * ch;
        const unsigned char* src = a.reads + read0 * CF::WINDOW * ch;
        constexpr int NDW = (CF::U8_BYTES / 4 + THREADS - 1) / THREADS;
        if ((reinterpret_cast<unsigned long long>(src) & 3ull) == 0) {
            unsigned v[NDW];
#pragma unroll
            for (int k = 0; k < NDW; ++k) {
                const int d = tid + THREADS * k;
                unsigned x = 0;
                if (4 * d + 4 <= n_bytes) {
                    x = ((const unsigned*)src)[d];
                } else if (4 * d < n_bytes) {
                    for (int b = 0; b < n_bytes - 4 * d; ++b) x |= (unsigned)src[4 * d + b] << (8 * b);
                }
                v[k] = x;
            }
#pragma unroll
            for (int k = 0; k < NDW; ++k) {
                const int d = tid + THREADS * k;
                if (4 * d < CF::U8_BYTES) ((unsigned*)s_u8)[d] = v[k];
            }
        } else {
            for (int i = tid; i < CF::U8_BYTES; i += THREADS) s_u8[i] = (i < n_bytes) ? src[i] : (unsigned char)0;
        }
        f32x4 ws2[3];
        if constexpr (!WINO) load_weights<3>(ws2, W + OFF_S2, 0, lane);
        barrier(0);
        stem_conv1<CF>(s_u8, bufB, W + OFF_S1, ch, dump, wave, lane);
        barrier(1);
        if constexpr (WINO) stem_conv2_wino<CF>(bufB, bufA, W + OFF_S2, dump, wave, lane);
        else conv_layer<CF, 16, 16, 3, 1, 0, 1, 1, 0, CF::ST12, MODE_PLAIN, false, GEOM_STEM, 16, CF::SROWS>(
            bufB, bufA, ws2, nullptr, W + OFF_S2 + 3 * 256, sreg, 0u, dump, wave, lane);
        barrier(2);
        if (tid < 8 * (G + 1)) {
            const int row = (tid >> 3) * RS1;
            *(f32x4*)(X + img_off<32, SWX>(row, tid & 7)) = f32x4{0.f, 0.f, 0.f, 0.f};
        }
        if constexpr (WINO) stem_conv3_pool_wino<CF, SWX>(bufA, X, W + OFF_S3, dump, wave, lane, n_here);
        else stem_conv3_pool<CF, SWX>(bufA, X, W + OFF_S3, dump, wave, lane, n_here);
        barrier(3);
        if (tid < 8) ((f32x4*)H)[tid] = f32x4{0.f, 0.f, 0.f, 0.f};
    } else {
        for (int i = tid; i < BUF_FLOATS / 4; i += THREADS) ((f32x4*)bufA)[i] = f32x4{0.f, 0.f, 0.f, 0.f};
        if (tid < 16) ((f32x4*)bufB)[tid] = f32x4{0.f, 0.f, 0.f, 0.f};
        barrier(0);
        const f32x4* src = (const f32x4*)(a.pooled + read0 * (L1 * 32));
        const int n4 = n_here * L1 * 8;
        for (int f = tid; f < n4; f += THREADS) {
            const int rd = f / (L1 * 8);
            const int rem = f - rd * (L1 * 8);
            const int p = rem >> 3, c = rem & 7;
            const int row = 1 + rd * RS1 + p;
            *(f32x4*)(bufA + img_off<32, SWX>(row, c)) = src[f];
        }
    }

    auto slice = [&](int off, int cb, int nv) { return W + off + cb * nv * 256 + lane * 4; };

    if constexpr (STEM && !BF16_32) {
        stamp(1 + 2 * 4);
        stamp(2 + 2 * 4);
    } else {
        barrier(4);
    }
    const unsigned short* const WS32 = (const unsigned short*)(W + O::off_d(NB64)) + (1 + 2 * NB64) * 24576 + cb2 * 3072 + lane * 8;
    bf16x8 cwh[3], cwl[3];
    if constexpr (BF16_32) {
        const int j = lane & 15, q = lane >> 4, pg = wave / 2;
#pragma unroll
        for (int st = 0; st < 3; ++st) {
            cwh[st] = *(const bf16x8*)(WS32 + (st * 2) * 512);
            cwl[st] = *(const bf16x8*)(WS32 + (st * 2 + 1) * 512);
        }
#pragma unroll
        for (int k = 0; k < RS1 * G / 32; ++k)
            sreg[k] = *(const f32x4*)(X + img_off<32, SWX>(16 * (pg + 2 * k) + j + 1, 4 * cb2 + q));
        __syncthreads();
#pragma unroll
        for (int k = 0; k < RS1 * G / 32; ++k) store_split32((unsigned char*)X, 16 * (pg + 2 * k) + j + 1, 4 * cb2 + q, sreg[k]);
        __syncthreads();
    }
#pragma unroll
    for (int blk = 0; blk < 3; ++blk) {
        const int off_a = OFF_B + (2 * blk) * (O::W3232D + 32), off_b = off_a + (O::W3232D + 32);
        if constexpr (BF16_32) {
            bf16x3_layer32<CF, BF_PLAIN, false, false>((const unsigned char*)X, (unsigned char*)H, cwh, cwl,
                                                       WS32 + (2 * blk + 1) * 6144, W + off_a + O::W3232D, sreg, wave, lane);
            __syncthreads();
            if (blk < 2)
                bf16x3_layer32<CF, BF_RESID, false, false>((const unsigned char*)H, (unsigned char*)X, cwh, cwl,
                                                           WS32 + (2 * blk + 2) * 6144, W + off_b + O::W3232D, sreg, wave, lane);
            else
                bf16x3_layer32<CF, BF_RESID, true, true>((const unsigned char*)H, (unsigned char*)X, cwh, cwl, nullptr,
                                                         W + off_b + O::W3232D, sreg, wave, lane);
            __syncthreads();
            continue;
        }
        const float* nxt = (blk < 2) ? slice(off_b + (W3232 + 32), cb2, NVA) : slice(OFF_C1, cb4, 6);
        if constexpr (F33) {
            auto slice32 = [&](int off) { return W + off + cb2 * (10 * 256) + lane * 4; };
            wino3_layer<CF, 32, MODE_PLAIN, false>(X, H, w3, slice32(off_a), slice32(off_b), W + off_a + O::W3232D, wave, lane);
            barrier(5 + 2 * blk);
            if (blk < 2)
                wino3_layer<CF, 32, MODE_RESID_INPLACE, false>(H, X, w3, slice32(off_b), slice32(off_b + (O::W3232D + 32)),
                                                               W + off_b + O::W3232D, wave, lane);
            else
                wino3_layer<CF, 32, MODE_RESID_INPLACE, true>(H, X, w3, slice32(off_b), nullptr, W + off_b + O::W3232D, wave, lane);
        } else if constexpr (WINO) {
            wino_layer<CF, 32, MODE_PLAIN, true>(X, H, wA, slice(off_b, cb2, NVA), W + off_a + W3232, pad1, dump, wave, lane);
            barrier(5 + 2 * blk);
            wino_layer<CF, 32, MODE_RESID_INPLACE, true, true>(H, X, wA, nxt, W + off_b + W3232, pad1f, dump, wave, lane);
        } else {
            conv_layer<CF, 32, 32, 3, 1, 1, RS1, RS1, L1, T1, MODE_PLAIN, true>(
                X, H, w6, slice(off_b, cb2, 6), W + off_a + W3232, sreg, pad1, dump, wave, lane);
            barrier(5 + 2 * blk);
            conv_layer<CF, 32, 32, 3, 1, 1, RS1, RS1, L1, T1, MODE_RESID_INPLACE, true>(
                H, X, w6, nxt, W + off_b + W3232, sreg, pad1, dump, wave, lane);
        }
        barrier(6 + 2 * blk);
    }

    if constexpr (F33) {
        load_weights<6>(w6, W + OFF_C1, cb4, lane);
    } else {
        load_weights<NVB>(wB, W + OFF_C2, cb4, lane);
    }
    load_weights<2>(w2, W + OFF_SC, cb4, lane);
    if (tid < 32) ((f32x4*)H)[(tid & 15) + (tid >> 4) * (RS2 * G + 1) * 16] = f32x4{0.f, 0.f, 0.f, 0.f};
    conv_layer<CF, 32, 64, 3, 2, 1, RS1, RS2, L2, T2, MODE_PLAIN, false, GEOM_TRUNK, 16, RS2 * CF::G, false, SWX,
               BF16 ? SW_SPLIT : (F33 ? SW_3 : SWX)>(X, H, w6, nullptr, W + OFF_C1 + W3264, sreg, pad2, dump, wave, lane);
    const unsigned short* const WS16 = (const unsigned short*)(W + O::off_d(NB64)) + cb4 * 6144 + lane * 8;
    bf16x8 bwh[6], bwl[6];
    if constexpr (BF16) {
        conv_layer<CF, 32, 64, 1, 2, 0, RS1, RS2, L2, T2, MODE_TO_REGS, false, GEOM_TRUNK, 16, RS2 * CF::G, false, SWX, SWX>(
            X, nullptr, w2, nullptr, W + OFF_SC + W3264S, sreg, pad2, dump, wave, lane);
#pragma unroll
        for (int st = 0; st < 6; ++st) {
            bwh[st] = *(const bf16x8*)(WS16 + (st * 2) * 512);
            bwl[st] = *(const bf16x8*)(WS16 + (st * 2 + 1) * 512);
        }
    } else if constexpr (F33) {
        static_assert(!F33 || CF::NSREG >= 3 * (RS2 * CF::G / 48), "shortcut tiles kept in registers");
        conv_layer<CF, 32, 64, 1, 2, 0, RS1, RS2, L2, 3 * (RS2 * CF::G / 48), MODE_TO_REGS, false, GEOM_WTRIPLE, 16, RS2 * CF::G,
                   false, SWX, SWX>(X, nullptr, w2, nullptr, W + OFF_SC + W3264S, sreg, pad2, dump, wave, lane);
#pragma unroll
        for (int c = 0; c < 5; ++c) w3[0][c] = *(const f32x4*)(W + OFF_C2 + cb4 * (20 * 256) + lane * 4 + c * 256);
    } else if constexpr (WINO) {
        conv_layer<CF, 32, 64, 1, 2, 0, RS1, RS2, L2, CF::NSREG, MODE_TO_REGS, false, GEOM_WPAIR, 16, RS2 * CF::G, false, SWX,
                   SWX>(X, nullptr, w2, nullptr, W + OFF_SC + W3264S, sreg, pad2, dump, wave, lane);
    } else {
        conv_layer<CF, 32, 64, 1, 2, 0, RS1, RS2, L2, T2, MODE_TO_REGS, false, GEOM_TRUNK, 16, RS2 * CF::G, false, SWX, SWX>(
            X, nullptr, w2, nullptr, W + OFF_SC + W3264S, sreg, pad2, dump, wave, lane);
    }
    barrier(11);
    if (tid < 32) ((f32x4*)X)[(tid & 15) + (tid >> 4) * (RS2 * G + 1) * 16] = f32x4{0.f, 0.f, 0.f, 0.f};
    auto slice3 = [&](int off) { return W + off + cb4 * (20 * 256) + lane * 4; };
    if constexpr (BF16) {
        bf16x3_layer<CF, BF_RESID, false, false>((const unsigned char*)H, (unsigned char*)X, bwh, bwl, WS16 + 24576,
                                                 W + OFF_C2 + O::W6464D, sreg, wave, lane);
    } else if constexpr (F33) {
        {
            const int j = lane & 15, q = lane >> 4;
#pragma unroll
            for (int t = 0; t < 3 * (RS2 * G / 48); ++t)
                *(f32x4*)(X + img_off_triple<64, SW_3>(t / 3, j, (t % 3) + 1, 4 * cb4 + q)) = sreg[t];
        }
        wino3_layer<CF, 64, MODE_RESID_INPLACE, false>(H, X, w3, slice3(OFF_C2), slice3(O::off_d(0)), W + OFF_C2 + O::W6464D, wave,
                                                       lane);
    } else if constexpr (WINO) {
        wino_layer<CF, 64, MODE_ADD_REGS, true>(H, X, wB, slice(O::off_d(0), cb4, NVB), W + OFF_C2 + W6464, pad2w, dump, wave,
                                                lane, sreg);
    } else {
        conv_layer<CF, 64, 64, 3, 1, 1, RS2, RS2, L2, T2, MODE_ADD_REGS, true, GEOM_TRUNK, 16, RS2 * CF::G, true, SWX, SWX>(
            H, X, w12, slice(O::off_d(0), cb4, NVB), W + OFF_C2 + W6464, sreg, pad2, dump, wave, lane);
    }
    barrier(12);

#pragma unroll
    for (int blk = 0; blk < NB64; ++blk) {
        const int off_a = O::off_d(blk), off_b = off_a + (O::W6464D + 64);
        if constexpr (BF16) {
            bf16x3_layer<CF, BF_PLAIN, false, false>((const unsigned char*)X, (unsigned char*)H, bwh, bwl,
                                                     WS16 + (2 + 2 * blk) * 24576, W + off_a + O::W6464D, sreg, wave, lane);
            __syncthreads();
            if (blk < NB64 - 1)
                bf16x3_layer<CF, BF_RESID, false, false>((const unsigned char*)H, (unsigned char*)X, bwh, bwl,
                                                         WS16 + (3 + 2 * blk) * 24576, W + off_b + O::W6464D, sreg, wave, lane);
            else
                bf16x3_layer<CF, BF_RESID, true, true>((const unsigned char*)H, (unsigned char*)X, bwh, bwl, nullptr,
                                                       W + off_b + O::W6464D, sreg, wave, lane);
        } else if constexpr (F33) {
            wino3_layer<CF, 64, MODE_PLAIN, false>(X, H, w3, slice3(off_a), slice3(off_b), W + off_a + O::W6464D, wave, lane);
            barrier(13 + 2 * blk);
// ... 12 lines not shown
                wino_layer<CF, 64, MODE_RESID_INPLACE, false>(H, X, wB, nullptr, W + off_b + W6464, pad2w, dump, wave, lane);
        } else {
            conv_layer<CF, 64, 64, 3, 1, 1, RS2, RS2, L2, T2, MODE_PLAIN, true, GEOM_TRUNK, 16, RS2 * CF::G, true>(
                X, H, w12, slice(off_b, cb4, 12), W + off_a + W6464, sreg, pad2, dump, wave, lane);
            barrier(13 + 2 * blk);
            if (blk < NB64 - 1)
                conv_layer<CF, 64, 64, 3, 1, 1, RS2, RS2, L2, T2, MODE_RESID_INPLACE, true, GEOM_TRUNK, 16, RS2 * CF::G, true>(
                    H, X, w12, slice(O::off_d(blk + 1), cb4, 12), W + off_b + W6464, sreg, pad2, dump, wave, lane);
            else
                conv_layer<CF, 64, 64, 3, 1, 1, RS2, RS2, L2, T2, MODE_RESID_INPLACE, false, GEOM_TRUNK, 16, RS2 * CF::G, true>(
                    H, X, w12, nullptr, W + off_b + W6464, sreg, pad2, dump, wave, lane);
        }
        barrier(14 + 2 * blk);
    }

    static_assert(G <= 4, "the allele select below");
    int allele_of[G];
#pragma unroll
    for (int rd = 0; rd < G; ++rd) {
        const long long r = read0 + rd < a.n_reads ? read0 + rd : a.n_reads - 1;
        allele_of[rd] = __builtin_amdgcn_readfirstlane(a.allele_of_read[r]);
    }
#pragma nounroll
    for (int rd = 0; rd < n_here; ++rd) {
        const int al = rd == 0 ? allele_of[0] : rd == 1 ? allele_of[1 % G] : rd == 2 ? allele_of[2 % G] : allele_of[3 % G];
        if (al != cur) {
            flush();
            cur = al;
        }
#pragma unroll
        for (int i = 0; i < NF; ++i) {
            const int f = tid + THREADS * i;
            if (f < L2 * 16) {
                const f32x4 v = *(const f32x4*)(X + img_off<64, F33 ? SW_3 : SWX>(1 + rd * RS2 + (f >> 4), f & 15));
#pragma unroll
                for (int e = 0; e < 4; ++e) carry[i][e] += v[e];
            }
        }
    }
    barrier(19);
    if constexpr (STAMP) {
        const unsigned long long rt = __builtin_amdgcn_s_memrealtime();
        if (grp < a.stamp_groups && lane == 0) stamp_base[43] = rt;
    }
    }
    flush();
    if constexpr (STAMP) {
        static_assert(!STAMP || (NB64 == 3 && STEM && WINO && !BF16), "stamps: the default fp32 Winograd schedule (20 barriers per group)");
        const unsigned long long t = __builtin_amdgcn_s_memtime();
        if ((tid0 & 63) == 0) a.stamps[(((long long)blockIdx.x * CF::NW + wave0) * a.stamp_groups) * STAMP_SLOTS + 44] = t;
    }
}

template <class CF, int NB64, bool WINO, bool STEM_ONLY = false, bool BF16 = false, bool BF16_32 = false>
static hipError_t launch_cfg(const ReadConvArgs& a, hipStream_t stream) {
    static bool configured_on[64] = {};
    int dev = 0;
    if (hipGetDevice(&dev) != hipSuccess || dev < 0 || dev >= 64) return hipErrorInvalidDevice;
    bool& configured = configured_on[dev];
    if (!configured) {
        hipError_t e = hipSuccess;
        if constexpr (!STEM_ONLY)
            e = hipFuncSetAttribute((const void*)readconv_kernel<CF, false, NB64, WINO, BF16, BF16_32>,
                                    hipFuncAttributeMaxDynamicSharedMemorySize, CF::LDS_BYTES);
        if (e == hipSuccess)
            e = hipFuncSetAttribute((const void*)readconv_kernel<CF, true, NB64, WINO, BF16, BF16_32>,
                                    hipFuncAttributeMaxDynamicSharedMemorySize, CF::LDS_BYTES);
        if (e != hipSuccess) return e;
        configured = true;
    }
    if (a.groups_per_wg < 1) return hipErrorInvalidValue;
    const long long per_wg = (long long)CF::G * a.groups_per_wg;
    const unsigned groups = (unsigned)((a.n_reads + per_wg - 1) / per_wg);
    if (a.stamps) {
        if constexpr (std::is_same<CF, Geometry>::value && NB64 == 3 && WINO && !BF16 && !STEM_ONLY) {
            if (!a.reads || (a.channels != 6 && a.channels != 7) || a.stamp_groups < 1) return hipErrorInvalidValue;
            static bool stamped_on[64] = {};
            if (!stamped_on[dev]) {
                const hipError_t e = hipFuncSetAttribute((const void*)readconv_kernel<CF, true, NB64, WINO, false, false, true>,
                                                         hipFuncAttributeMaxDynamicSharedMemorySize, 100 * 1024);
                if (e != hipSuccess) return e;
                stamped_on[dev] = true;
            }
            const int lds = (a.stamp_mode & 2) ? 100 * 1024 : CF::LDS_BYTES;
            hipLaunchKernelGGL((readconv_kernel<CF, true, NB64, WINO, false, false, true>), dim3(groups), dim3(CF::THREADS), lds, stream, a);
            return hipGetLastError();
        } else {
            return hipErrorInvalidValue;
        }
    }
    if (a.reads) {
        if (a.channels != 6 && a.channels != 7) return hipErrorInvalidValue;
        hipLaunchKernelGGL((readconv_kernel<CF, true, NB64, WINO, BF16, BF16_32>), dim3(groups), dim3(CF::THREADS), CF::LDS_BYTES, stream, a);
    } else if constexpr (!STEM_ONLY) {
        hipLaunchKernelGGL((readconv_kernel<CF, false, NB64, WINO, BF16, BF16_32>), dim3(groups), dim3(CF::THREADS), CF::LDS_BYTES, stream, a);
    } else {
        return hipErrorInvalidValue;
    }
    return hipGetLastError();
}

hipError_t launch_readconv_fused(const ReadConvArgs& a, hipStream_t stream) {
    if (a.n_reads <= 0) return hipSuccess;
    if (a.window == 250) {
        if (!a.reads || !a.winograd || a.extra_blocks != 0) return hipErrorInvalidValue;
        return launch_cfg<Geometry250, 3, true, true>(a, stream);
    }
    if (a.window != 150) return hipErrorInvalidValue;
    if (a.bf16x3) {
        if (!a.reads || !a.winograd || a.extra_blocks != 0 || a.softplus) return hipErrorInvalidValue;
        return a.bf16x3 > 1 ? launch_cfg<Geometry, 3, true, true, true, true>(a, stream)
                            : launch_cfg<Geometry, 3, true, true, true, false>(a, stream);
    }
    if (a.softplus) {
        if (!a.reads || !a.winograd || a.extra_blocks != 0) return hipErrorInvalidValue;
        return launch_cfg<GeometrySoftplus, 3, true, true>(a, stream);
    }
    if (a.extra_blocks == 0) return a.winograd ? launch_cfg<Geometry, 3, true>(a, stream) : launch_cfg<Geometry, 3, false>(a, stream);
    if (a.extra_blocks == 2) return a.winograd ? launch_cfg<Geometry, 5, true>(a, stream) : launch_cfg<Geometry, 5, false>(a, stream);
    return hipErrorInvalidValue;
}

__global__ void readconv_finalize_kernel(const float* __restrict__ partial, const int32_t* __restrict__ slot_off,
                                         float* __restrict__ frames, int frame_f4) {
    const int al = blockIdx.x;
    const int lo = slot_off[al], hi = slot_off[al + 1];
    for (int f = threadIdx.x; f < frame_f4; f += blockDim.x) {
        f32x4 acc = *(const f32x4*)(partial + ((long long)lo * frame_f4 + f) * 4);
        for (int s = lo + 1; s < hi; ++s) {
            const f32x4 v = *(const f32x4*)(partial + ((long long)s * frame_f4 + f) * 4);
#pragma unroll
            for (int e = 0; e < 4; ++e) acc[e] += v[e];
        }
        *(f32x4*)(frames + ((long long)al * frame_f4 + f) * 4) = acc;
    }
}

hipError_t launch_readconv_finalize(const float* partial, const int32_t* slot_off, float* frames, int n_alleles,
                                    int frame_rows, int channels, hipStream_t stream) {
    if (n_alleles <= 0) return hipSuccess;
    if (channels <= 0 || (channels % 4)) return hipErrorInvalidValue;
    hipLaunchKernelGGL(readconv_finalize_kernel, dim3(n_alleles), dim3(192), 0, stream, partial, slot_off, frames,
                       frame_rows * (channels / 4));
    return hipGetLastError();
}

namespace cc {
struct Cfg {
    static constexpr int ACT = rc::ACT_RELU;
    static __device__ __forceinline__ float act(float x) { return fmaxf(x, 0.f); }
    static constexpr int G = 8;
    static constexpr int NW = 8;
    static constexpr int THREADS = 64 * NW;
    static constexpr int L0 = 36, L1 = 18;
    static constexpr int NSREG = 3 * (L1 * G / 48);
    static constexpr int BUF_FLOATS = rc::cmax((L0 * G + 2) * 64, (L1 * G + 2) * 128);
    static constexpr int LDS_BYTES = 2 * BUF_FLOATS * 4 + 64;
    static constexpr int W11 = 4 * 1 * 4 * 256, WS = 8 * 3 * 4 * 256, WSC = 8 * 1 * 4 * 256, WB = 8 * 8 * 5 * 256;
    static constexpr int OFF_11 = 0, OFF_S = OFF_11 + W11 + 64, OFF_SC = OFF_S + WS + 128, OFF_B = OFF_SC + WSC + 128;
    static constexpr int off_conv(int i) { return OFF_B + i * (WB + 128); }
    static constexpr int total(int blocks) { return off_conv(1 + 2 * blocks); }
};
}

int compressor_weight_floats(int blocks) { return cc::Cfg::total(blocks); }
bool compressor_supports_blocks(int blocks) { return blocks >= 2 && blocks <= 4; }

template <int NB>
__global__ __launch_bounds__(cc::Cfg::THREADS, 2) void compressor_kernel(CompressorArgs a) {
    using CF = cc::Cfg;
    constexpr int G = CF::G, L0 = CF::L0, L1 = CF::L1;
    extern __shared__ __attribute__((aligned(16))) float smem[];
    float* const bufA = smem;
    float* const bufB = smem + CF::BUF_FLOATS;
    float* const dump = smem + 2 * CF::BUF_FLOATS;
    const int tid = threadIdx.x, lane = tid & 63;
    const int wave = __builtin_amdgcn_readfirstlane(tid >> 6);
    const long long item0 = (long long)blockIdx.x * a.items_per_wg;
    const int n_here = (int)((a.n_items - item0) < a.items_per_wg ? (a.n_items - item0) : a.items_per_wg);
    const float* __restrict__ W = a.w;
    const f32x4 zero4 = {0.f, 0.f, 0.f, 0.f};

    f32x4 w11[4];
    load_weights<4>(w11, W + CF::OFF_11, wave % 4, lane);
    {
        const f32x4* src = (const f32x4*)(a.frames + item0 * (L0 * 64));
        constexpr int NLD = G * L0 * 16 / CF::THREADS;
        static_assert(NLD * CF::THREADS == G * L0 * 16, "the input image divides evenly over the threads");
        f32x4 v[NLD];
#pragma unroll
        for (int k = 0; k < NLD; ++k) {
            const int f = tid + CF::THREADS * k;
            v[k] = (f / (L0 * 16)) < n_here ? src[f] : zero4;
        }
#pragma unroll
        for (int k = 0; k < NLD; ++k) {
            const int f = tid + CF::THREADS * k;
            *(f32x4*)(bufA + img_off<64, SW_OLD>(1 + (f >> 4), f & 15)) = v[k];
        }
        if (tid < 16) ((f32x4*)bufA)[tid] = zero4;
        else if (tid < 32) ((f32x4*)bufB)[tid - 16] = zero4;
    }
    __syncthreads();
    f32x4 sreg[CF::NSREG];
    const bool full = n_here == G;
    const int live0 = (n_here * L0 + 15) / 16, live1 = (n_here * L1 + 15) / 16;
    if (full)
        conv_layer<CF, 64, 64, 1, 1, 0, L0, L0, L0, L0 * G / 16, MODE_PLAIN, false, GEOM_TRUNK, 16, L0 * G, false, SW_OLD, SW_W>(
            bufA, bufB, w11, nullptr, W + CF::OFF_11 + CF::W11, sreg, 0u, dump, wave, lane);
    else
        conv_layer<CF, 64, 64, 1, 1, 0, L0, L0, L0, L0 * G / 16, MODE_PLAIN, false, GEOM_TRUNK, 16, L0 * G, false, SW_OLD, SW_W, true>(
            bufA, bufB, w11, nullptr, W + CF::OFF_11 + CF::W11, sreg, 0u, dump, wave, lane, 0, (live0 - wave / 4 + 1) / 2);
    f32x4 ws[12], wsc[4];
    load_weights<12>(ws, W + CF::OFF_S, wave, lane);
    load_weights<4>(wsc, W + CF::OFF_SC, wave, lane);
    __syncthreads();
    if (tid < 64) ((f32x4*)bufA)[(tid & 31) + (tid >> 5) * (L1 * G + 1) * 32] = zero4;
    if (full)
        conv_layer<CF, 64, 128, 3, 2, 1, L0, L1, L1, L1 * G / 16, MODE_PLAIN, false, GEOM_TRUNK, 16, L1 * G, true, SW_W, SW_3>(
            bufB, bufA, ws, nullptr, W + CF::OFF_S + CF::WS, sreg, 0u, dump, wave, lane);
    else
        conv_layer<CF, 64, 128, 3, 2, 1, L0, L1, L1, L1 * G / 16, MODE_PLAIN, false, GEOM_TRUNK, 16, L1 * G, true, SW_W, SW_3, true>(
            bufB, bufA, ws, nullptr, W + CF::OFF_S + CF::WS, sreg, 0u, dump, wave, lane, 0, live1);
    conv_layer<CF, 64, 128, 1, 2, 0, L0, L1, L1, CF::NSREG, MODE_TO_REGS, false, GEOM_WTRIPLE, 16, L1 * G, false, SW_W, SW_3>(
        bufB, nullptr, wsc, nullptr, W + CF::OFF_SC + CF::WSC, sreg, 0u, dump, wave, lane);
    f32x4 w3[2][5];
    auto slice = [&](int off) { return W + off + wave * (8 * 5 * 256) + lane * 4; };
#pragma unroll
    for (int c = 0; c < 5; ++c) w3[0][c] = *(const f32x4*)(slice(CF::off_conv(0)) + c * 256);
    __syncthreads();
    if (tid < 64) ((f32x4*)bufB)[(tid & 31) + (tid >> 5) * (L1 * G + 1) * 32] = zero4;
    {
        const int j = lane & 15, q = lane >> 4;
#pragma unroll
        for (int t = 0; t < CF::NSREG; ++t)
            *(f32x4*)(bufB + img_off_triple<128, SW_3>(t / 3, j, (t % 3) + 1, 4 * wave + q)) = sreg[t];
    }
    const int live_tiles = (6 * n_here + 15) / 16;
    auto f33_layers = [&](auto partial) {
        constexpr bool PARTIAL = decltype(partial)::value;
        wino3_layer<CF, 128, MODE_RESID_INPLACE, false, L1, SW_3, true, PARTIAL>(
            bufA, bufB, w3, slice(CF::off_conv(0)), slice(CF::off_conv(1)), W + CF::off_conv(0) + CF::WB, wave, lane, live_tiles);
        __syncthreads();
        static_for<0, NB>([&](auto bc) {
            constexpr int blk = decltype(bc)::value;
            constexpr int off_a = CF::off_conv(1 + 2 * blk), off_b = CF::off_conv(2 + 2 * blk);
            wino3_layer<CF, 128, MODE_PLAIN, false, L1, SW_3, true, PARTIAL>(bufB, bufA, w3, slice(off_a), slice(off_b),
                                                                            W + off_a + CF::WB, wave, lane, live_tiles);
            __syncthreads();
            if constexpr (blk < NB - 1)
                wino3_layer<CF, 128, MODE_RESID_INPLACE, false, L1, SW_3, true, PARTIAL>(
                    bufA, bufB, w3, slice(off_b), slice(CF::off_conv(3 + 2 * blk)), W + off_b + CF::WB, wave, lane, live_tiles);
            else
                wino3_layer<CF, 128, MODE_RESID_INPLACE, true, L1, SW_3, true, PARTIAL>(bufA, bufB, w3, slice(off_b), nullptr,
                                                                                       W + off_b + CF::WB, wave, lane, live_tiles);
            __syncthreads();
        });
    };
    if (live_tiles == L1 * G / 48) f33_layers(std::false_type{});
    else f33_layers(std::true_type{});
    f32x4* dst = (f32x4*)(a.dst + item0 * (L1 * 128));
    for (int f = tid; f < n_here * L1 * 32; f += CF::THREADS)
        dst[f] = *(const f32x4*)(bufB + img_off<128, SW_3>(1 + (f >> 5), f & 31));
}

int small_launch_items_per_wg(long long n_items, int most) {
    const long long cus = device_cus();
    const long long n = (n_items + cus - 1) / cus;
    return (int)(n < 1 ? 1 : (n <= 2 ? n : most));
}

hipError_t launch_compressor_fused(const CompressorArgs& args, hipStream_t stream) {
    if (args.n_items <= 0) return hipSuccess;
    CompressorArgs a = args;
    if (a.items_per_wg == 0) a.items_per_wg = small_launch_items_per_wg(a.n_items, cc::Cfg::G);
    if (!compressor_supports_blocks(a.blocks) || !a.frames || !a.dst || !a.w || a.items_per_wg < 1 || a.items_per_wg > cc::Cfg::G) return hipErrorInvalidValue;
    static bool configured_on[64] = {};
    int dev = 0;
    if (hipGetDevice(&dev) != hipSuccess || dev < 0 || dev >= 64) return hipErrorInvalidDevice;
    if (!configured_on[dev]) {
        hipError_t e = hipFuncSetAttribute((const void*)compressor_kernel<2>, hipFuncAttributeMaxDynamicSharedMemorySize, cc::Cfg::LDS_BYTES);
        if (e == hipSuccess)
            e = hipFuncSetAttribute((const void*)compressor_kernel<3>, hipFuncAttributeMaxDynamicSharedMemorySize, cc::Cfg::LDS_BYTES);
        if (e == hipSuccess)
            e = hipFuncSetAttribute((const void*)compressor_kernel<4>, hipFuncAttributeMaxDynamicSharedMemorySize, cc::Cfg::LDS_BYTES);
        if (e != hipSuccess) return e;
        configured_on[dev] = true;
    }
    const unsigned grid = (unsigned)((a.n_items + a.items_per_wg - 1) / a.items_per_wg);
    if (a.blocks == 2) hipLaunchKernelGGL(compressor_kernel<2>, dim3(grid), dim3(cc::Cfg::THREADS), cc::Cfg::LDS_BYTES, stream, a);
    else if (a.blocks == 3) hipLaunchKernelGGL(compressor_kernel<3>, dim3(grid), dim3(cc::Cfg::THREADS), cc::Cfg::LDS_BYTES, stream, a);
    else hipLaunchKernelGGL(compressor_kernel<4>, dim3(grid), dim3(cc::Cfg::THREADS), cc::Cfg::LDS_BYTES, stream, a);
    return hipGetLastError();
}


namespace xf {
struct Cfg {
    static constexpr int ACT = rc::ACT_RELU;
    static __device__ __forceinline__ float act(float x) { return fmaxf(x, 0.f); }
    static constexpr int G = 8, NW = 8, THREADS = 64 * NW;
    static constexpr int L = 18, LO = 9;
    static constexpr int NSREG = 1;
    static constexpr int A_FLOATS = (L * G + 2) * 128;
    static constexpr int B_ROWS = 2 * (16 * 5) + 2;
    static constexpr int LDS_BYTES = (A_FLOATS + B_ROWS * 128) * 4 + 64;
    static constexpr int W11 = 8 * 1 * 8 * 256, WS = 16 * 3 * 8 * 256, WSC = 16 * 1 * 8 * 256;
    static constexpr int OFF_11 = 0, OFF_S = OFF_11 + W11 + 128, OFF_SC = OFF_S + WS + 256, TOTAL = OFF_SC + WSC + 256;
};
struct Cfg16 : Cfg {
    static constexpr int NW = 16;
};
struct CfgLinear : Cfg16 {
    static __device__ __forceinline__ float act(float x) { return x; }
};
}

int xattn_front_weight_floats() { return xf::Cfg::TOTAL; }

__global__ __launch_bounds__(xf::Cfg::THREADS, 2) void xattn_front_kernel(XattnFrontArgs a) {
    using CF = xf::Cfg;
    using CF16 = xf::Cfg16;
    constexpr int G = CF::G, L = CF::L, LO = CF::LO;
    extern __shared__ __attribute__((aligned(16))) float smem[];
    float* const bufA = smem;
    float* const bufB = smem + CF::A_FLOATS;
    float* const dump = smem + CF::A_FLOATS + CF::B_ROWS * 128;
    const int tid = threadIdx.x, lane = tid & 63;
    const int wave = __builtin_amdgcn_readfirstlane(tid >> 6);
    const long long item0 = (long long)blockIdx.x * a.items_per_wg;
    const int n_here = (int)((a.n_items - item0) < a.items_per_wg ? (a.n_items - item0) : a.items_per_wg);
    const float* __restrict__ W = a.w;
    const f32x4 zero4 = {0.f, 0.f, 0.f, 0.f};
    f32x4 sreg[CF::NSREG];

    f32x4 w11[8];
    load_weights<8>(w11, W + CF::OFF_11, wave, lane);
    {
        constexpr int NLD = G * L * 32 / CF::THREADS;
        static_assert(NLD * CF::THREADS == G * L * 32, "the input image divides evenly over the threads");
        const f32x4* src = (const f32x4*)(a.alleles + item0 * (L * 128));
        f32x4 va[NLD], vs[NLD];
// ... 459 lines not shown
```

hello_amd/engine.py:

```python
from __future__ import annotations

import ctypes as C
import logging
import os
from typing import Optional, Sequence, Tuple

import numpy as np

from . import compiler
from . import netspec as ns

_log = logging.getLogger(__name__)

_LIB_PATH = os.environ.get("HELLO_LIB") or os.path.join(os.path.dirname(os.path.abspath(__file__)),
                                                        "libhello_mi355x.so")
HELLO_IN_DEVICE, HELLO_OUT_DEVICE, HELLO_LAYOUT_RCL = 1, 2, 4
ABI_VERSION = 2
LANES_MAX_SITES = 64

class HelloOp(C.Structure):
    _fields_ = [("kind", C.c_int32), ("domain", C.c_int32), ("src0", C.c_int32), ("src1", C.c_int32),
                ("dst", C.c_int32), ("res", C.c_int32), ("cin", C.c_int32), ("cout", C.c_int32),
                ("k", C.c_int32), ("stride", C.c_int32), ("pad", C.c_int32), ("lin", C.c_int32),
                ("lout", C.c_int32), ("flags", C.c_int32), ("seg", C.c_int32), ("c1", C.c_int32),
# ... 51 lines not shown
        lib.hello_engine_allele_support.restype = C.c_int
    if hasattr(lib, "hello_engine_allele_evidence"):
        lib.hello_engine_allele_evidence.argtypes = [vp] * 11 + [i64, i64, i64, vp, i32, vp]
        lib.hello_engine_allele_evidence.restype = C.c_int
    lib.hello_engine_stream.argtypes = [vp]
    lib.hello_engine_stream.restype = C.c_void_p
    lib.hello_engine_destroy.argtypes = [vp]
    lib.hello_engine_destroy.restype = None
    for fn in ("hello_engine_create", "hello_engine_forward", "hello_engine_posteriors",
               "hello_engine_synchronize", "hello_engine_last_forward_ms", "hello_engine_set_profiling",
               "hello_engine_op_times_ms", "hello_engine_set_profiling_filter", "hello_engine_debug_capture",
               "hello_engine_debug_read") + diagnostics:
        getattr(lib, fn).restype = C.c_int
    _lib = lib
    return lib


def _check(rc):
    if rc != 0:
        raise RuntimeError(f"hello_mi355x: {load_library().hello_last_error().decode()} (status {rc})")


def _is_torch(x):
    return type(x).__module__.startswith("torch")


def _i32_host(x) -> np.ndarray:
    if _is_torch(x):
        x = x.detach().cpu().numpy()
    return np.ascontiguousarray(np.asarray(x), dtype=np.int32)


def n_pairs(alleles_per_site) -> int:
    a = np.asarray(alleles_per_site, dtype=np.int64)
    return int((a * (a + 1) // 2).sum())


def model_desc(program: "compiler.Program"):
    ops = (HelloOp * len(program.ops))()
    for dst, o in zip(ops, program.ops):
        for name, _ in HelloOp._fields_:
            setattr(dst, name, getattr(o, name))
    bufs = (HelloBuffer * len(program.buffers))()
    for dst, (dom, fpr) in zip(bufs, program.buffers):
        dst.domain, dst.floats_per_row = dom, fpr
    desc = HelloModelDesc(ABI_VERSION, program.window, program.channels0, program.channels1, program.n_experts, int(program.has_meta),
                          int(program.uses_ref), len(program.buffers), bufs, len(program.ops), ops)
    return desc, (ops, bufs)


class Engine:

    def __init__(self, spec: ns.ModelSpec, state, device: int = 0, fused: bool = True, winograd: bool = True,
                 program: Optional["compiler.Program"] = None, arithmetic: Optional[str] = None, lanes_max_sites: Optional[int] = None):
        self.lib = load_library()
        self.spec = spec
        self.lanes_max_sites = lanes_max_sites
        self._lanes_recipe = None if program is not None else dict(state=state, fused=fused, winograd=winograd, arithmetic=arithmetic or "fp32")
        if program is None:
            program = compiler.compile_model(spec, state, fused=fused, winograd=winograd, arithmetic=arithmetic or "fp32")
        self.program = program
        p = self.program
        self.device = device
        self.handle, self._desc_arrays = self._create(p)
        self.lanes_handle = None
        self.lanes_program = None
        self._sequential_only = 0
        self.n_experts = p.n_experts
        self.has_meta = p.has_meta
        self._own = None

    def _create(self, program):
        desc, keep = model_desc(program)
        blob = np.ascontiguousarray(program.weights, dtype=np.float32)
        handle = C.c_void_p()
        _check(self.lib.hello_engine_create(C.byref(desc), blob.ctypes.data, blob.nbytes, self.device, C.byref(handle)))
        return handle, keep

    def small_launch_handle(self):
        if self._sequential_only or self._lanes_recipe is None:
            return self.handle
        if self.lanes_handle is None:
            r = self._lanes_recipe
            prog = compiler.compile_model(self.spec, r["state"], fused=r["fused"], winograd=r["winograd"], arithmetic=r["arithmetic"], lanes=True)
            if prog.n_lanes == 1:
                self._lanes_recipe = None
                return self.handle
            self.lanes_handle, self._lanes_desc_arrays = self._create(prog)
            self.lanes_program = prog
            self._lanes_recipe = dict(r, state=None)
        return self.lanes_handle

    class _OnStream:

        def __init__(self, engine, device, stream):
            import torch
            self.current = None
            if not stream:
                cur = torch.cuda.current_stream(device)
                if cur.cuda_stream == 0:
                    if engine._own is None:
                        engine._own = torch.cuda.ExternalStream(engine.lib.hello_engine_stream(engine.handle), device=device)
                    self.current, self.own = cur, engine._own
                    stream = engine._own.cuda_stream
                else:
                    stream = cur.cuda_stream
            self.handle = stream

        def __enter__(self):
            if self.current is not None:
                self.own.wait_stream(self.current)
            return self.handle

        def __exit__(self, *exc):
            if self.current is not None:
                self.current.wait_stream(self.own)
            return False

    def on_stream(self, device, stream=None):
        return Engine._OnStream(self, device, stream)

    def close(self):
        if getattr(self, "lanes_handle", None):
            self.lib.hello_engine_destroy(self.lanes_handle)
            self.lanes_handle = None
        if getattr(self, "handle", None):
            self.lib.hello_engine_destroy(self.handle)
            self.handle = None

    def __del__(self):
        try:
            self.close()
        except Exception:
            pass

    def forward(self, reads0, reads_per_allele0, alleles_per_site, reads1=None, reads_per_allele1=None,
                ref_onehot=None, stream: Optional[int] = None, layout_rcl: bool = False,
# ... 186 lines not shown
```

hello_amd/readconv_pack.py:

```python
import numpy as np

from . import netspec as ns

AVAILABLE = True
TRUNK_FIRST_NODE = 4
EXTRA_BLOCKS = (0, 2)


def _pack_conv(w: np.ndarray, b: np.ndarray) -> np.ndarray:
    cout, cin, k = w.shape
    lanes = np.arange(64)
    out_idx = (np.arange(cout // 16)[:, None] * 16 + (lanes & 15)[None, :])
    in_idx = (np.arange(cin // 16)[:, None, None] * 16 + 4 * (lanes >> 4)[None, :, None]
              + np.arange(4)[None, None, :])
    packed = w[out_idx[:, None, None, :, None], in_idx[None, None, :, :, :], np.arange(k)[None, :, None, None, None]]
    return np.concatenate([packed.astype(np.float32).ravel(), b.astype(np.float32).ravel()])


def trunk_convs(nodes):
    blocks = nodes[TRUNK_FIRST_NODE:TRUNK_FIRST_NODE + 7]
    assert len(blocks) == 7 and all(isinstance(b, ns.Residual) for b in blocks)
    order = []
    for blk in blocks[:3]:
        order += [blk.body[0], blk.body[1]]
    strided = blocks[3]
    order += [strided.body[0], strided.shortcut[0], strided.body[1]]
    for blk in blocks[4:]:
        order += [blk.body[0], blk.body[1]]
    return order


def _pack_first_conv(w: np.ndarray, b: np.ndarray, steps: int = 6) -> np.ndarray:
    cout, cin, k = w.shape
    assert cout == 16 and k == 3 and 3 * cin <= 4 * steps
    flat = np.zeros((cout, 4 * steps), np.float32)
    flat[:, :3 * cin] = w.transpose(0, 2, 1).reshape(cout, 3 * cin)
    lanes = np.arange(64)
    packed = flat[(lanes & 15)[None, :], 4 * np.arange(steps)[:, None] + (lanes >> 4)[None, :]]
    return np.concatenate([packed.ravel(), b.astype(np.float32).ravel()])


WINDOWS = (150, 250)


def geometry(window: int):
    l1 = (window - 9) // 2 + 1
    l2 = (l1 - 1) // 2 + 1
    return (4 if window == 150 else 2), l1, l1 + 1, l2, (l2 if l2 % 2 == 0 else l2 + 1), (l1 + 6) // 7


def executed_macs_per_read(winograd: bool, extra_blocks: int = 0, window: int = 150) -> float:
    g, l1, rs1, _, rs2, ntt = geometry(window)
    t_stem12 = -(-(-(-window * g // 16)) // 4) * 4
    conv3 = g * (-(-l1 // 15)) * 2 * 4 * 4 if winograd else g * ntt * 2 * 3 * 4
    conv2 = -(-(-(-(window * g // 2) // 16)) // 4) * 4 * 16 if winograd else t_stem12 * 3 * 4
    stem = t_stem12 * 6 + conv2 + conv3
    t1, t2 = -(-rs1 * g // 16), -(-rs2 * g // 16)
    n64 = 6 + 2 * extra_blocks
    if winograd:
        w1, w2 = -(-(rs1 // 2) * g // 16), -(-(rs2 // 2) * g // 16)
        strided = t2 * 4 * 6 * 4 + 2 * w2 * 4 * 2 * 4 + w2 * 4 * 4 * 16
        if f33(winograd, window):
            strided = t2 * 4 * 6 * 4 + 3 * (rs2 * g // 48) * 4 * 2 * 4 + (rs2 * g // 48) * 4 * 4 * 20
        per64 = (rs2 * g // 48) * 4 * 4 * 20 if f33(winograd, window) else w2 * 4 * 4 * 16
        per32 = (rs1 * g // 48) * 2 * 2 * 20 if f33(winograd, window) else w1 * 2 * 2 * 16
        blocks = 6 * per32 + n64 * per64
    else:
        strided = t2 * 4 * 6 * 4 + t2 * 4 * 2 * 4 + t2 * 4 * 12 * 4
        blocks = 6 * (t1 * 2 * 6 * 4) + n64 * (t2 * 4 * 12 * 4)
    return (stem + strided + blocks) * 1024.0 / g


def winograd_taps(w: np.ndarray) -> np.ndarray:
    g = w.astype(np.float64)
    u = np.stack([g[..., 0], (g[..., 0] + g[..., 1] + g[..., 2]) / 2, (g[..., 0] - g[..., 1] + g[..., 2]) / 2,
                  g[..., 2]], axis=-1)
    return u.astype(np.float32)


def winograd_taps_f33(w: np.ndarray) -> np.ndarray:
    g = w.astype(np.float64)
    g0, g1, g2 = g[..., 0], g[..., 1], g[..., 2]
    u = np.stack([g0 / 2, -(g0 + g1 + g2) / 2, (-g0 + g1 - g2) / 6, (g0 + 2 * g1 + 4 * g2) / 6, g2], axis=-1)
    return u.astype(np.float32)


def f33(winograd: bool, window: int) -> bool:
    return bool(winograd) and window == 150


def _pack_conv_f33(w: np.ndarray, b: np.ndarray) -> np.ndarray:
    u = winograd_taps_f33(w)
    cout, cin, _ = u.shape
    n = (cout // 16) * 5 * (cin // 16) * 256
    blocks = _pack_conv(u, b)[:n].reshape(cout // 16, 5, cin // 16, 64, 4)
    return np.concatenate([blocks.transpose(0, 2, 1, 3, 4).ravel(), b.astype(np.float32).ravel()])


def pack(nodes, folded, cin=None, winograd: bool = False, window: int = 150) -> np.ndarray:
    convs = trunk_convs(nodes)
    strided = {6, 7}
    use33 = f33(winograd, window)

    def one(i, c):
        w, b = folded[c.key]
        if use33 and i not in strided:
            return _pack_conv_f33(w, b)
        return _pack_conv(winograd_taps(w), b) if (winograd and i not in strided) else _pack_conv(w, b)

    parts = [one(i, c) for i, c in enumerate(convs)]
    stem = nodes[:3]
    parts.append(_pack_first_conv(*folded[stem[0].key]))
    w2, b2 = folded[stem[1].key]
    parts.append(_pack_conv(winograd_taps(w2), b2) if winograd else _pack_conv(w2, b2))
    w3, b3 = folded[stem[2].key]
    parts.append(_pack_conv(winograd_taps(w3), b3) if winograd else _pack_conv(w3, b3))
    extras = nodes[TRUNK_FIRST_NODE + 7:]
    assert len(extras) in EXTRA_BLOCKS
    for blk in extras:
        parts += [one(9, blk.body[0]), one(9, blk.body[1])]
    blob = np.concatenate(parts)
    kt = 4 if winograd else 3
    w32, w64 = 2 * kt * 2 * 256, 4 * kt * 4 * 256
# ... 55 lines not shown
                    for part in (hi, lo):
                        parts.append(part[out_idx[cb][:, None], in_idx[h], tap].ravel())
    out32 = np.arange(2)[:, None] * 16 + (lanes & 15)[None, :]
    in32 = 8 * (lanes >> 4)[:, None] + np.arange(8)[None, :]
    for c in convs[:6]:
        w, _ = folded[c.key]
        assert w.shape == (32, 32, 3), w.shape
        w = w.astype(np.float32)
        hi = to_bf16_bits(w)
        lo = to_bf16_bits(w - (hi.astype(np.uint32) << np.uint32(16)).view(np.float32))
        for cb in range(2):
            for tap in range(3):
                for part in (hi, lo):
                    parts.append(part[out32[cb][:, None], in32, tap].ravel())
    bits = np.concatenate(parts).astype(np.uint16)
    assert bits.size == len(layers) * 24576 + 6 * 6144
    return bits.view(np.float32).copy()


COMPRESSOR_BLOCKS = (2, 3, 4)


def compressor_blocks(nodes) -> int:
    def conv_is(n, cin, cout, k, stride, pad, act):
        return (isinstance(n, ns.Conv) and (n.cin, n.cout, n.k, n.stride, n.pad, n.dilation, n.groups, n.act) ==
                (cin, cout, k, stride, pad, 1, 1, act) and n.norm != "ln")
    if len(nodes) < 3 or not conv_is(nodes[0], 64, 64, 1, 1, 0, "relu"):
        return -1
    st = nodes[1]
    if not (isinstance(st, ns.Residual) and len(st.body) == 2 and len(st.shortcut) == 1 and
            conv_is(st.body[0], 64, 128, 3, 2, 1, "relu") and conv_is(st.body[1], 128, 128, 3, 1, 1, "relu") and
            conv_is(st.shortcut[0], 64, 128, 1, 2, 0, "none")):
        return -1
    for blk in nodes[2:]:
        if not (isinstance(blk, ns.Residual) and len(blk.body) == 2 and not blk.shortcut and
                all(conv_is(c, 128, 128, 3, 1, 1, "relu") for c in blk.body)):
            return -1
    return len(nodes) - 2


def pack_compressor(nodes, folded) -> np.ndarray:
    assert compressor_blocks(nodes) in COMPRESSOR_BLOCKS
    st = nodes[1]
    parts = [_pack_conv(*folded[nodes[0].key]), _pack_conv(*folded[st.body[0].key]), _pack_conv(*folded[st.shortcut[0].key]),
             _pack_conv_f33(*folded[st.body[1].key])]
    for blk in nodes[2:]:
        parts += [_pack_conv_f33(*folded[blk.body[0].key]), _pack_conv_f33(*folded[blk.body[1].key])]
    blob = np.concatenate(parts)
    n = len(nodes) - 2
    assert blob.size == (4096 + 64) + (24576 + 128) + (8192 + 128) + (1 + 2 * n) * (81920 + 128), blob.size
    return blob


def compressor_executed_macs(blocks: int) -> float:
    return 36 * 64 * 64 + 18 * 128 * 192 + 18 * 128 * 64 + (1 + 2 * blocks) * 6 * 5 * 128 * 128


def wide_trunk_nodes(nodes, cin):
    def conv_is(n, ci, co, k, stride, pad, act):
        return (isinstance(n, ns.Conv) and (n.cin, n.cout, n.k, n.stride, n.pad, n.dilation, n.groups, n.act) ==
                (ci, co, k, stride, pad, 1, 1, act) and n.norm != "ln")
    if len(nodes) != TRUNK_FIRST_NODE + 7 or cin not in (6, 7):
        return None
    stem = nodes[:TRUNK_FIRST_NODE]
    if not (conv_is(stem[0], cin, 32, 3, 1, 0, "relu") and conv_is(stem[1], 32, 32, 3, 1, 0, "relu") and
            conv_is(stem[2], 32, 64, 3, 1, 0, "relu") and isinstance(stem[3], ns.MaxPool) and
            (stem[3].k, stem[3].stride, stem[3].pad) == (3, 2, 0)):
        return None
    blocks = nodes[TRUNK_FIRST_NODE:]

    def identity(blk, c):
        return (isinstance(blk, ns.Residual) and len(blk.body) == 2 and not blk.shortcut and
                all(conv_is(x, c, c, 3, 1, 1, "relu") for x in blk.body))
    st = blocks[3]
    if not (all(identity(b, 64) for b in blocks[:3]) and all(identity(b, 128) for b in blocks[4:]) and
            isinstance(st, ns.Residual) and len(st.body) == 2 and len(st.shortcut) == 1 and
            conv_is(st.body[0], 64, 128, 3, 2, 1, "relu") and conv_is(st.body[1], 128, 128, 3, 1, 1, "relu") and
            conv_is(st.shortcut[0], 64, 128, 1, 2, 0, "none")):
        return None
    return blocks


def _pack_first_conv_wide(w: np.ndarray, b: np.ndarray, steps: int = 6) -> np.ndarray:
    cout, cin, k = w.shape
    assert cout == 32 and k == 3 and 3 * cin <= 4 * steps
    flat = np.zeros((cout, 4 * steps), np.float32)
    flat[:, :3 * cin] = w.transpose(0, 2, 1).reshape(cout, 3 * cin)
    lanes = np.arange(64)
    packed = flat[(16 * np.arange(2)[:, None, None] + (lanes & 15)[None, None, :]),
                  (4 * np.arange(steps)[None, :, None] + (lanes >> 4)[None, None, :])]
    return np.concatenate([packed.ravel(), b.astype(np.float32).ravel()])


def pack_wide(nodes, blocks, folded) -> np.ndarray:
    stem = nodes[:3]
    parts = [pack_wide_trunk(blocks, folded), _pack_first_conv_wide(*folded[stem[0].key])]
    for conv in stem[1:]:
        w, b = folded[conv.key]
        parts.append(_pack_conv(winograd_taps(w), b))
    blob = np.concatenate(parts)
    assert blob.size == parts[0].size + (768 + 32) + (4096 + 32) + (8192 + 64), blob.size
    return blob


def wide_executed_macs(cin: int) -> float:
    return wide_trunk_executed_macs() + 40 * 16 * 24 * 32 / 4 + 19 * 16 * 4 * 32 * 32 / 4 + 5 * 16 * 4 * 32 * 64


# ... 16 lines not shown
```

include/hello_mi355x.h:

```cpp
#ifndef HELLO_MI355X_H
#define HELLO_MI355X_H

#include <stddef.h>
#include <stdint.h>

#ifdef __cplusplus
extern "C" {
#endif

#define HELLO_ABI_VERSION 2

typedef enum hello_status {
    HELLO_OK = 0,
    HELLO_ERR_ARG = -1,
    HELLO_ERR_SHAPE = -2,
    HELLO_ERR_MODEL = -3,
    HELLO_ERR_HIP = -4,
    HELLO_ERR_NOGPU = -5,
    HELLO_ERR_NOMEM = -6
} hello_status;


typedef enum hello_domain {
    HELLO_ROWS_READS0 = 0,
    HELLO_ROWS_READS1 = 1,
    HELLO_ROWS_ALLELES = 2,
    HELLO_ROWS_SITES = 3
} hello_domain;

typedef enum hello_segment {
    HELLO_SEG_READS0_TO_ALLELES = 0,
    HELLO_SEG_READS1_TO_ALLELES = 1,
    HELLO_SEG_ALLELES_TO_SITES = 2
} hello_segment;

#define HELLO_BUF_NONE   (-1)
#define HELLO_BUF_READS0 0
#define HELLO_BUF_READS1 1
#define HELLO_BUF_REF    2
#define HELLO_BUF_FIRST_SCRATCH 3

typedef enum hello_op_kind {
    HELLO_OP_CONV1D = 1,
    HELLO_OP_MAXPOOL = 2,
    HELLO_OP_SEGSUM = 3,
    HELLO_OP_MIX = 4,
    HELLO_OP_HEAD = 5,
    HELLO_OP_CONCAT = 6,
    HELLO_OP_ADD = 7,
    HELLO_OP_READCONV_FUSED = 8
    ,
    HELLO_OP_LAYERNORM = 9
    ,
    HELLO_OP_COMPRESSOR_FUSED = 10
    ,
    HELLO_OP_XATTN_FRONT = 11
} hello_op_kind;

#define HELLO_FLAG_RELU     1
#define HELLO_FLAG_SRC_U8   2
#define HELLO_FLAG_SOFTMAX  4
#define HELLO_FLAG_SOFTPLUS 16
#define HELLO_FLAG_WINOGRAD 32
#define HELLO_FLAG_BF16X3   64
#define HELLO_FLAG_BF16X3_32 128
#define HELLO_FLAG_MIX_REST 8
#define HELLO_FLAG_LANE_SHIFT 8
#define HELLO_FLAG_LANE_MASK  (7 << HELLO_FLAG_LANE_SHIFT)
#define HELLO_MAX_LANES 8

typedef struct hello_op {
    int32_t kind;
    int32_t domain;
    int32_t src0, src1;
    int32_t dst;
    int32_t res;
    int32_t cin, cout;
    int32_t k, stride, pad;
    int32_t lin, lout;
    int32_t flags;
    int32_t seg;
    int32_t c1;
    float a0, a1;
    int64_t w_off;
    int64_t b_off;
} hello_op;

typedef struct hello_buffer {
    int32_t domain;
    int32_t floats_per_row;
} hello_buffer;

typedef struct hello_model_desc {
    int32_t abi_version;
    int32_t window;
    int32_t channels0, channels1;
    int32_t n_experts;
    int32_t has_meta;
    int32_t uses_ref;
    int32_t n_buffers;
    const hello_buffer* buffers;
    int32_t n_ops;
    const hello_op* ops;
} hello_model_desc;

typedef struct hello_engine hello_engine;

#define HELLO_IN_DEVICE   1
#define HELLO_OUT_DEVICE  2
#define HELLO_LAYOUT_RCL  4

int hello_engine_create(const hello_model_desc* desc, const void* folded_weights, size_t nbytes,
                        int hip_device, hello_engine** out);

int hello_engine_forward(hello_engine* engine,
                         const uint8_t* reads0, const int32_t* reads_per_allele0,
                         const uint8_t* reads1, const int32_t* reads_per_allele1,
                         const int32_t* alleles_per_site, const uint8_t* ref_onehot,
                         int32_t n_sites, int32_t n_alleles, int64_t n_reads0, int64_t n_reads1,
// ... 386 lines not shown
```

Measured before the change: 489,500.

## Add polyphase Winograd form for stride-2 convolutions in read convolver and compressor

```diff
diff --git a/hello_amd/compiler.py b/hello_amd/compiler.py
--- a/hello_amd/compiler.py
+++ b/hello_amd/compiler.py
@@ -15,6 +15,7 @@
 (OP_CONV1D, OP_MAXPOOL, OP_SEGSUM, OP_MIX, OP_HEAD, OP_CONCAT, OP_ADD, OP_READCONV_FUSED, OP_LAYERNORM,
  OP_COMPRESSOR_FUSED) = range(1, 11)
 FLAG_RELU, FLAG_SRC_U8, FLAG_SOFTMAX, FLAG_MIX_REST, FLAG_SOFTPLUS, FLAG_WINOGRAD, FLAG_BF16X3, FLAG_BF16X3_32 = 1, 2, 4, 8, 16, 32, 64, 128
+FLAG_POLYPHASE = 2048
 FLAG_LANE_SHIFT, MAX_LANES = 8, 8
 OP_NAMES = {1: "conv1d", 2: "maxpool", 3: "segsum", 4: "mix", 5: "head", 6: "concat", 7: "add",
             8: "readconv_fused", 9: "layernorm", 10: "compressor_fused", 11: "xattn_front"}
@@ -76,6 +77,7 @@
     fused_compressor: bool = False
     winograd: bool = False
     arithmetic: str = "fp32"
+    strided: str = "direct"
     n_lanes: int = 1
 
     def describe(self) -> str:
@@ -182,10 +184,17 @@
 
 
 class _Lowering:
-    def __init__(self, spec: ns.ModelSpec, state, fused: bool, winograd: bool = True, arithmetic: str = "fp32"):
+    def __init__(self, spec: ns.ModelSpec, state, fused: bool, winograd: bool = True, arithmetic: str = "fp32",
+                 strided: str = "polyphase"):
         if arithmetic not in ARITHMETICS:
             raise ValueError(f"arithmetic must be one of {ARITHMETICS}, not {arithmetic!r}")
+        from .readconv_pack import STRIDED_FORMS
+        if strided not in STRIDED_FORMS:
+            raise ValueError(f"strided must be one of {STRIDED_FORMS}, not {strided!r}")
         self.arithmetic = arithmetic
+        self.strided = strided
+        self.used_polyphase = False
+        self.used_polyphase_compressor = False
         self.used_bf16x3 = False
         self.used_xattn_front = False
         self.spec = spec
@@ -256,10 +265,16 @@
                 and readconv_pack.compressor_blocks(nodes) in readconv_pack.COMPRESSOR_BLOCKS):
             blocks = readconv_pack.compressor_blocks(nodes)
             y = self.new(x.domain, 18, 128)
-            w_off = self.blob.add(readconv_pack.pack_compressor(nodes, self.folded))
+            packed = readconv_pack.pack_compressor(nodes, self.folded)
+            poly = self.strided == "polyphase+compressor"
+            if poly:
+                packed = np.concatenate([packed, readconv_pack.pack_compressor_polyphase(nodes, self.folded)])
+                self.used_polyphase_compressor = True
+            w_off = self.blob.add(packed)
             self.ops.append(Op(OP_COMPRESSOR_FUSED, x.domain, src0=x.vid, dst=y.vid, cin=64, cout=128, k=blocks, lin=36, lout=18,
-                               flags=FLAG_WINOGRAD | FLAG_RELU, w_off=w_off, b_off=w_off, name=nodes[0].key.rsplit(".network", 1)[0],
-                               macs_per_row=ns.macs(nodes, 36), exec_macs_per_row=readconv_pack.compressor_executed_macs(blocks)))
+                               flags=FLAG_WINOGRAD | FLAG_RELU | (FLAG_POLYPHASE if poly else 0), w_off=w_off, b_off=w_off,
+                               name=nodes[0].key.rsplit(".network", 1)[0], macs_per_row=ns.macs(nodes, 36),
+                               exec_macs_per_row=readconv_pack.compressor_executed_macs(blocks, polyphase=poly)))
             self.used_fused_compressor = True
             return y
         front = readconv_pack.xattn_front_match(nodes) if (self.fused is True and self.winograd and isinstance(x, tuple)) else None
@@ -393,6 +408,14 @@
                 packed = np.concatenate([packed, readconv_pack.pack_bf16x3(nodes, self.folded)])
                 wflag |= FLAG_BF16X3 | (FLAG_BF16X3_32 if "+32" in self.arithmetic else 0)
                 self.used_bf16x3 = True
+            carry = (self.strided != "direct" and self.fused is True and
+                     readconv_pack.polyphase_available(self.winograd, spec.window, extras, softplus))
+            poly = carry and not (wflag & FLAG_BF16X3)
+            if carry:
+                packed = np.concatenate([packed, readconv_pack.pack_polyphase(nodes, self.folded)])
+            if poly:
+                wflag |= FLAG_POLYPHASE
+                self.used_polyphase = True
             w_off = self.blob.add(packed)
             if self.fused == "trunk":
                 pooled = self.net(nodes[:readconv_pack.TRUNK_FIRST_NODE], x)
@@ -406,8 +429,8 @@
                                    k=extras, lin=spec.window, lout=l2, seg=seg, w_off=w_off, b_off=w_off, name=name,
                                    flags=FLAG_SRC_U8 | wflag | (FLAG_SOFTPLUS if softplus else 0),
                                    macs_per_row=ns.macs(nodes, spec.window),
-                                   exec_macs_per_row=readconv_pack.executed_macs_per_read(self.winograd, extras,
-                                                                                          spec.window)))
+                                   exec_macs_per_row=(readconv_pack.polyphase_executed_macs_per_read(cin, extras) if poly else
+                                                      readconv_pack.executed_macs_per_read(self.winograd, extras, spec.window))))
             self.used_fused = True
             return y
         return self.segsum(self.net(nodes, x), seg)
@@ -684,8 +707,8 @@
 
 
 def compile_model(spec: ns.ModelSpec, state, fused: bool = True, winograd: bool = True, arithmetic: str = "fp32",
-                  fold_site_sums: bool = True, lanes: bool = False) -> Program:
-    low = _Lowering(spec, state, fused, winograd, arithmetic)
+                  fold_site_sums: bool = True, lanes: bool = False, strided: str = "polyphase") -> Program:
+    low = _Lowering(spec, state, fused, winograd, arithmetic, strided)
     n_experts, has_meta = low.lower()
     if arithmetic != "fp32" and not low.used_bf16x3:
         raise ValueError("arithmetic='bf16x3' / 'bf16x3+32' exists for the canonical 150 bp ReLU read convolver in the whole-kernel "
@@ -702,4 +725,6 @@
         channels1=spec.channels[1] if spec.hybrid_inputs else 0,
         n_experts=n_experts, has_meta=has_meta, uses_ref=low.uses_ref, ops=low.ops,
         buffers=buffers, weights=low.blob.finish(), fused_read_convolver=low.used_fused,
-        fused_compressor=low.used_fused_compressor, winograd=low.winograd, arithmetic=arithmetic, n_lanes=n_lanes)
+        fused_compressor=low.used_fused_compressor, winograd=low.winograd, arithmetic=arithmetic,
+        strided=("polyphase+compressor" if low.used_polyphase_compressor else "polyphase" if low.used_polyphase else "direct"),
+        n_lanes=n_lanes)
diff --git a/hello_amd/csrc/engine.hip b/hello_amd/csrc/engine.hip
--- a/hello_amd/csrc/engine.hip
+++ b/hello_amd/csrc/engine.hip
@@ -381,6 +381,11 @@
                   !(o.flags & HELLO_FLAG_SOFTPLUS)))
                 return fail(HELLO_ERR_MODEL, "op %d: the bf16x3 arithmetic mode exists for the canonical read convolver run whole "
                                              "(from the bytes) in Winograd form on 150 bp windows, ReLU, without extra blocks", i);
+            if ((o.flags & HELLO_FLAG_POLYPHASE) &&
+                !(d->window == 150 && !wide && (o.flags & HELLO_FLAG_WINOGRAD) && (o.flags & HELLO_FLAG_SRC_U8) &&
+                  !(o.flags & (HELLO_FLAG_SOFTPLUS | HELLO_FLAG_BF16X3))))
+                return fail(HELLO_ERR_MODEL, "op %d: the polyphase strided convolution exists for the canonical read convolver run whole "
+                                             "(from the bytes) in fp32 Winograd form on 150 bp windows, ReLU", i);
             if (d->window == 250 && !((o.flags & HELLO_FLAG_WINOGRAD) && (o.flags & HELLO_FLAG_SRC_U8) && o.k == 0))
                 return fail(HELLO_ERR_MODEL, "op %d: 250 bp windows run whole (from the bytes), in Winograd form, "
                                              "without extra blocks", i);
@@ -493,7 +498,8 @@
             w_end = (size_t)o.w_off + o.cin;
             b_end = (size_t)o.b_off + o.cin;
         } else if (o.kind == HELLO_OP_COMPRESSOR_FUSED) {
-            w_end = (size_t)o.w_off + hello::compressor_weight_floats(o.k);
+            w_end = (size_t)o.w_off + hello::compressor_weight_floats(o.k) +
+                    ((o.flags & HELLO_FLAG_POLYPHASE) ? hello::compressor_polyphase_extra_floats() : 0);
             b_end = (size_t)o.b_off;
         } else if (o.kind == HELLO_OP_XATTN_FRONT) {
             w_end = (size_t)o.w_off + hello::xattn_front_weight_floats();
@@ -501,6 +507,7 @@
         } else if (o.kind == HELLO_OP_READCONV_FUSED) {
             w_end = (size_t)o.w_off + (o.cout == 128 ? hello::readconv_wide_weight_floats()
                                                      : hello::readconv_weight_floats(o.k, (o.flags & HELLO_FLAG_WINOGRAD) != 0, desc->window));
+            if (o.flags & HELLO_FLAG_POLYPHASE) w_end += hello::readconv_polyphase_extra_floats();
             b_end = (size_t)o.b_off;
             if (o.cout == 128) e->wide_trunk[o.seg == HELLO_SEG_READS1_TO_ALLELES ? 1 : 0] = true;
         }
@@ -1062,6 +1069,7 @@
                 a.w = e->d_weights + o.w_off;
                 a.n_items = rows;
                 a.blocks = o.k;
+                a.polyphase = (o.flags & HELLO_FLAG_POLYPHASE) ? 1 : 0;
                 HIP_TRY(hello::launch_compressor_fused(a, stream));
                 break;
             }
@@ -1106,9 +1114,11 @@
                 a.extra_blocks = o.k;
                 a.winograd = (o.flags & HELLO_FLAG_WINOGRAD) ? 1 : 0;
                 a.bf16x3 = (o.flags & HELLO_FLAG_BF16X3) ? ((o.flags & HELLO_FLAG_BF16X3_32) ? 2 : 1) : 0;
+                a.polyphase = (o.flags & HELLO_FLAG_POLYPHASE) ? 1 : 0;
                 const bool wide = o.cout == 128;
                 if ((size_t)o.w_off + (wide ? hello::readconv_wide_weight_floats() : hello::readconv_weight_floats(o.k, a.winograd, d.window)) +
-                        (a.bf16x3 ? hello::readconv_bf16x3_extra_floats(o.k) : 0) > e->n_weight_floats)
+                        (a.bf16x3 ? hello::readconv_bf16x3_extra_floats(o.k) : 0) +
+                        (a.polyphase ? hello::readconv_polyphase_extra_floats() : 0) > e->n_weight_floats)
                     return fail(HELLO_ERR_MODEL, "op %d: fused read-convolver weight block truncated", op_index);
                 {
                     const hello::ReadConvPlan& plan = t1 ? e->plan1 : e->plan0;
diff --git a/hello_amd/csrc/kernels.h b/hello_amd/csrc/kernels.h
--- a/hello_amd/csrc/kernels.h
+++ b/hello_amd/csrc/kernels.h
@@ -73,6 +73,7 @@
     int window;
     int softplus;
     int bf16x3;
+    int polyphase;
     unsigned long long* stamps;
     int stamp_groups;
     int stamp_mode;
@@ -92,6 +93,7 @@
 ReadConvPlan readconv_wide_plan(long long n_reads);
 int readconv_weight_floats(int extra_blocks, bool winograd, int window);
 int readconv_bf16x3_extra_floats(int extra_blocks);
+int readconv_polyphase_extra_floats();
 bool readconv_supports_extra_blocks(int extra_blocks);
 hipError_t launch_readconv_fused(const ReadConvArgs& a, hipStream_t stream);
 hipError_t launch_readconv_finalize(const float* partial, const int32_t* slot_off, float* frames, int n_alleles,
@@ -107,9 +109,11 @@
     long long n_items;
     int blocks;
     int items_per_wg;
+    int polyphase;
 };
 int small_launch_items_per_wg(long long n_items, int most);
 int compressor_weight_floats(int blocks);
+int compressor_polyphase_extra_floats();
 bool compressor_supports_blocks(int blocks);
 hipError_t launch_compressor_fused(const CompressorArgs& a, hipStream_t stream);
 
diff --git a/hello_amd/csrc/readconv_fused.hip b/hello_amd/csrc/readconv_fused.hip
--- a/hello_amd/csrc/readconv_fused.hip
+++ b/hello_amd/csrc/readconv_fused.hip
@@ -79,6 +79,10 @@
 static_assert(Geometry::F33 && GeometrySoftplus::F33 && !Geometry250::F33, "weight packing rule of readconv_pack.py");
 static_assert(Geometry::F33_32 && GeometrySoftplus::F33_32, "weight packing rule of readconv_pack.py");
 int readconv_bf16x3_extra_floats(int extra_blocks) { return (1 + 2 * (3 + extra_blocks)) * 12288 + 6 * 3072; }
+namespace rc {
+constexpr int POLY_W1 = 4 * 2 * 256, POLY_U = 4 * 2 * 4 * 256;
+}
+int readconv_polyphase_extra_floats() { return rc::POLY_W1 + rc::POLY_U; }
 int readconv_weight_floats(int extra_blocks, bool winograd, int window) {
     if (!winograd) return rc::Offs<false>::off_d(3 + extra_blocks);
     return window == 150 ? rc::Offs<true, true>::off_d(3 + extra_blocks) : rc::Offs<true>::off_d(3 + extra_blocks);
@@ -701,6 +705,132 @@
     });
 }
 
+template <class CF, int CIN, int RS_OUT, bool MASK = false, bool PARTIAL = false>
+__device__ __forceinline__ void poly_odd_layer(const float* __restrict__ in, const f32x4 (&w)[CIN / 16][4], f32x4 (&acc)[3][4],
+                                               int lane, int live_tiles = 1 << 30) {
+    static_assert(RS_OUT % 3 == 0 && RS_OUT * CF::G == 144 && (CIN == 32 || CIN == 64), "3 tiles of 16 triples of whole items");
+    constexpr int NT = 3, M = CIN / 16, NU = M * NT, TOFF = 96 * CIN;
+    constexpr int TPI = RS_OUT / 3;
+    const int j = lane & 15, q = lane >> 4;
+    const f32x4 zero4 = {0.f, 0.f, 0.f, 0.f};
+    const float* pin[M][4];
+#pragma unroll
+    for (int m = 0; m < M; ++m)
+#pragma unroll
+        for (int i = 0; i < 4; ++i) pin[m][i] = in + img_off<CIN, SW_W>(6 * j + 2 * i, 4 * m + q);
+    f32x4 ring[2][4];
+    auto issue = [&](auto uc) {
+        constexpr int u = decltype(uc)::value;
+        constexpr int m = u / NT, k = u % NT;
+        bool first = false;
+        if constexpr (MASK) {
+            static_for<0, 16>([&](auto jc) {
+                constexpr int jj = decltype(jc)::value;
+                if constexpr ((16 * k + jj) % TPI == 0) first = first || (j == jj);
+            });
+        }
+#pragma unroll
+        for (int i = 0; i < 4; ++i) {
+            const float* ptr = pin[m][i] + k * TOFF;
+            if (MASK && i == 0) ptr = first ? in + 4 * (4 * m + q) : ptr;
+            ring[u & 1][i] = *(const f32x4*)ptr;
+        }
+    };
+    issue(std::integral_constant<int, 0>{});
+    static_for<0, NU>([&](auto uc) {
+        constexpr int u = decltype(uc)::value;
+        constexpr int m = u / NT, k = u % NT;
+        if constexpr (u + 1 < NU) {
+            if (!PARTIAL || (u + 1) % NT < live_tiles) issue(std::integral_constant<int, u + 1>{});
+        }
+        __builtin_amdgcn_sched_barrier(0);
+        if (PARTIAL && k >= live_tiles) return;
+        const f32x4(&d)[4] = ring[u & 1];
+        const f32x4 v0 = pk_sub(d[0], d[2]), v1 = pk_add(d[1], d[2]), v2 = pk_sub(d[2], d[1]), v3 = pk_sub(d[3], d[1]);
+        asm volatile("s_nop 1");
+        __builtin_amdgcn_sched_barrier(0);
+        f32x4(&a)[4] = acc[k];
+#pragma unroll
+        for (int e = 0; e < 4; ++e) {
+            const bool first = (m == 0) && (e == 0);
+            a[0] = __builtin_amdgcn_mfma_f32_16x16x4f32(w[m][0][e], v0[e], first ? zero4 : a[0], 0, 0, 0);
+            a[1] = __builtin_amdgcn_mfma_f32_16x16x4f32(w[m][1][e], v1[e], first ? zero4 : a[1], 0, 0, 0);
+            a[2] = __builtin_amdgcn_mfma_f32_16x16x4f32(w[m][2][e], v2[e], first ? zero4 : a[2], 0, 0, 0);
+            a[3] = __builtin_amdgcn_mfma_f32_16x16x4f32(w[m][3][e], v3[e], first ? zero4 : a[3], 0, 0, 0);
+        }
+    });
+}
+
+template <class CF, int CIN, int COUT, bool PARTIAL = false>
+__device__ __forceinline__ void poly_even_layer(const float* __restrict__ in, float* __restrict__ out, const f32x4 (&wc)[CIN / 16],
+                                                const f32x4 (&wsc)[CIN / 16], const float* __restrict__ bias_c,
+                                                const float* __restrict__ bias_sc, const f32x4 (&z)[3][4],
+                                                f32x4 (&sreg)[CF::NSREG], int wave, int lane, int live_tiles = 1 << 30) {
+    static_assert(CF::NW * 16 == COUT && CF::NSREG >= 9 && (CIN == 32 || CIN == 64), "a wave per 16-channel block, 3 tiles of 16 triples");
+    constexpr int NT = 3, M = CIN / 16, NU = NT * M, TIN = 96 * CIN, TOUT = 48 * COUT;
+    const int cb = wave, j = lane & 15, q = lane >> 4;
+    const f32x4 b4c = *(const f32x4*)(bias_c + cb * 16 + 4 * q), b4s = *(const f32x4*)(bias_sc + cb * 16 + 4 * q);
+    const float* pin[M][3];
+#pragma unroll
+    for (int m = 0; m < M; ++m)
+#pragma unroll
+        for (int u = 0; u < 3; ++u) pin[m][u] = in + img_off<CIN, SW_W>(6 * j + 2 * u + 1, 4 * m + q);
+    float* po[3];
+#pragma unroll
+    for (int u = 0; u < 3; ++u) po[u] = out + img_off_triple<COUT, SW_3>(0, j, 1 + u, 4 * cb + q);
+    f32x4 ring[2][3], cen[2][3];
+    auto issue = [&](auto sc) {
+        constexpr int s = decltype(sc)::value;
+        constexpr int t = s / M, m = s % M;
+#pragma unroll
+        for (int u = 0; u < 3; ++u) ring[s & 1][u] = *(const f32x4*)(pin[m][u] + t * TIN);
+    };
+    auto epi_store = [&](auto tc) {
+        constexpr int tt = decltype(tc)::value;
+        const f32x4(&a)[4] = z[tt];
+        const f32x4 sum = a[1] + a[2];
+        f32x4 y0 = (a[0] + sum) + cen[tt & 1][0];
+        f32x4 y1 = (a[1] - a[2]) + cen[tt & 1][1];
+        f32x4 y2 = (sum + a[3]) + cen[tt & 1][2];
+#pragma unroll
+        for (int e = 0; e < 4; ++e) {
+            y0[e] = CF::act(y0[e]);
+            y1[e] = CF::act(y1[e]);
+            y2[e] = CF::act(y2[e]);
+        }
+        *(f32x4*)(po[0] + tt * TOUT) = y0;
+        *(f32x4*)(po[1] + tt * TOUT) = y1;
+        *(f32x4*)(po[2] + tt * TOUT) = y2;
+    };
+    issue(std::integral_constant<int, 0>{});
+    static_for<0, NU>([&](auto sc) {
+        constexpr int s = decltype(sc)::value;
+        constexpr int t = s / M, m = s % M;
+        if constexpr (s + 1 < NU) {
+            if (!PARTIAL || (s + 1) / M < live_tiles) issue(std::integral_constant<int, s + 1>{});
+        }
+        __builtin_amdgcn_sched_barrier(0);
+        if constexpr (m == 1 && t >= 1) {
+            if (!PARTIAL || t - 1 < live_tiles) epi_store(std::integral_constant<int, (t >= 1 ? t - 1 : 0)>{});
+        }
+        if (!PARTIAL || t < live_tiles) {
+            const f32x4(&x)[3] = ring[s & 1];
+#pragma unroll
+            for (int e = 0; e < 4; ++e) {
+                const bool first = (m == 0) && (e == 0);
+#pragma unroll
+                for (int u = 0; u < 3; ++u) {
+                    sreg[3 * t + u] = __builtin_amdgcn_mfma_f32_16x16x4f32(wsc[m][e], x[u][e], first ? b4s : sreg[3 * t + u], 0, 0, 0);
+                    cen[t & 1][u] = __builtin_amdgcn_mfma_f32_16x16x4f32(wc[m][e], x[u][e], first ? b4c : cen[t & 1][u], 0, 0, 0);
+                }
+            }
+        }
+        if constexpr (s == NU - 1) {
+            if (!PARTIAL || NT - 1 < live_tiles) epi_store(std::integral_constant<int, NT - 1>{});
+        }
+    });
+}
+
 enum { BF_PLAIN = 0, BF_RESID = 1 };
 constexpr int BF16_DEPTH = 2;
 constexpr bool BF16_DEFER = true;
@@ -843,23 +973,22 @@
     });
 }
 
-template <class CF>
+template <class CF, int NSTEP = rc::S1_STEPS>
 __device__ __forceinline__ void stem_conv1(const unsigned char* __restrict__ s_u8, float* __restrict__ c1,
                                            const float* __restrict__ W, int ch, float* __restrict__ dump, int wave,
                                            int lane) {
-    using namespace rc;
     constexpr int NPAIR = CF::ST12 / 8;
     static_assert(CF::ST12 % 8 == 0, "stem tiles must split into pairs over 4 waves");
     const int j = lane & 15, q = lane >> 4;
-    float w1[S1_STEPS];
-#pragma unroll
-    for (int s = 0; s < S1_STEPS; ++s) w1[s] = W[s * 64 + lane];
-    const f32x4 b4 = *(const f32x4*)(W + S1_STEPS * 64 + 4 * q);
+    float w1[NSTEP];
+#pragma unroll
+    for (int s = 0; s < NSTEP; ++s) w1[s] = W[s * 64 + lane];
+    const f32x4 b4 = *(const f32x4*)(W + rc::S1_STEPS * 64 + 4 * q);
     const unsigned char* base = s_u8 + (16 * wave + j) * ch + q;
     const int tile_bytes = 16 * ch;
-    unsigned char cur0[S1_STEPS], cur1[S1_STEPS], nxt0[S1_STEPS], nxt1[S1_STEPS];
-#pragma unroll
-    for (int s = 0; s < S1_STEPS; ++s) {
+    unsigned char cur0[NSTEP], cur1[NSTEP], nxt0[NSTEP], nxt1[NSTEP];
+#pragma unroll
+    for (int s = 0; s < NSTEP; ++s) {
         cur0[s] = base[4 * s];
         cur1[s] = base[4 * tile_bytes + 4 * s];
     }
@@ -867,7 +996,7 @@
     for (int i = 0; i < NPAIR; ++i) {
         if (i + 1 < NPAIR) {
 #pragma unroll
-            for (int s = 0; s < S1_STEPS; ++s) {
+            for (int s = 0; s < NSTEP; ++s) {
                 nxt0[s] = base[(8 * (i + 1)) * tile_bytes + 4 * s];
                 nxt1[s] = base[(8 * (i + 1) + 4) * tile_bytes + 4 * s];
             }
@@ -875,7 +1004,7 @@
         __builtin_amdgcn_sched_barrier(0);
         f32x4 a0 = {0.f, 0.f, 0.f, 0.f}, a1 = {0.f, 0.f, 0.f, 0.f};
 #pragma unroll
-        for (int s = 0; s < S1_STEPS; ++s) {
+        for (int s = 0; s < NSTEP; ++s) {
             a0 = __builtin_amdgcn_mfma_f32_16x16x4f32(w1[s], (float)cur0[s], a0, 0, 0, 0);
             a1 = __builtin_amdgcn_mfma_f32_16x16x4f32(w1[s], (float)cur1[s], a1, 0, 0, 0);
         }
@@ -889,7 +1018,7 @@
         *(f32x4*)(r0 < CF::SROWS ? c1 + r0 * 16 + 4 * (q ^ swz<16>(r0)) : dump) = v0;
         *(f32x4*)(r1 < CF::SROWS ? c1 + r1 * 16 + 4 * (q ^ swz<16>(r1)) : dump) = v1;
 #pragma unroll
-        for (int s = 0; s < S1_STEPS; ++s) {
+        for (int s = 0; s < NSTEP; ++s) {
             cur0[s] = nxt0[s];
             cur1[s] = nxt1[s];
         }
@@ -1117,10 +1246,11 @@
     });
 }
 
-template <class CF, bool STEM, int NB64, bool WINO, bool BF16 = false, bool BF16_32 = false, bool STAMP = false>
-__global__ __launch_bounds__(CF::THREADS, 2) void readconv_kernel(ReadConvArgs a) {
+template <class CF, bool STEM, int NB64, bool WINO, bool BF16, bool BF16_32, bool STAMP, bool POLY = false, int CH = 0>
+__device__ __forceinline__ void readconv_body(const ReadConvArgs& a) {
     using namespace rc;
     constexpr bool F33 = WINO && CF::F33;
+    static_assert(!POLY || (F33 && STEM && !BF16 && (CH == 6 || CH == 7)), "polyphase: the fp32 F(3,3) kernel from the bytes");
     static_assert(!BF16 || (F33 && CF::ACT == ACT_RELU), "bf16x3: the 150 bp ReLU geometry of the Winograd kernel");
     static_assert(!BF16_32 || BF16, "the 32-channel split layers extend the bf16x3 mode");
     using O = Offs<WINO, F33>;
@@ -1232,7 +1362,7 @@
         load_weights<NVA>(wA, W + OFF_B, cb2, lane);
     }
     if (STEM) {
-        const int ch = a.channels;
+        const int ch = CH ? CH : a.channels;
         const int n_bytes = n_here * CF::WINDOW * ch;
         const unsigned char* src = a.reads + read0 * CF::WINDOW * ch;
         constexpr int NDW = (CF::U8_BYTES / 4 + THREADS - 1) / THREADS;
@@ -1260,7 +1390,7 @@
         f32x4 ws2[3];
         if constexpr (!WINO) load_weights<3>(ws2, W + OFF_S2, 0, lane);
         barrier(0);
-        stem_conv1<CF>(s_u8, bufB, W + OFF_S1, ch, dump, wave, lane);
+        stem_conv1<CF, (CH == 6 ? 5 : S1_STEPS)>(s_u8, bufB, W + OFF_S1, ch, dump, wave, lane);
         barrier(1);
         if constexpr (WINO) stem_conv2_wino<CF>(bufB, bufA, W + OFF_S2, dump, wave, lane);
         else conv_layer<CF, 16, 16, 3, 1, 0, 1, 1, 0, CF::ST12, MODE_PLAIN, false, GEOM_STEM, 16, CF::SROWS>(
@@ -1354,6 +1484,22 @@
         barrier(6 + 2 * blk);
     }
 
+    if constexpr (POLY) {
+        const float* const WP = W + O::off_d(NB64);
+        f32x4 wu[2][4], wc[2];
+#pragma unroll
+        for (int m = 0; m < 2; ++m)
+#pragma unroll
+            for (int c = 0; c < 4; ++c) wu[m][c] = *(const f32x4*)(WP + POLY_W1 + (((cb4 * 2 + m) * 4 + c) * 64 + lane) * 4);
+        load_weights<2>(wc, WP, cb4, lane);
+        load_weights<2>(w2, W + OFF_SC, cb4, lane);
+        if (tid < 32) ((f32x4*)H)[(tid & 15) + (tid >> 4) * (RS2 * G + 1) * 16] = f32x4{0.f, 0.f, 0.f, 0.f};
+        f32x4 zacc[3][4];
+        poly_odd_layer<CF, 32, RS2>(X, wu, zacc, lane);
+        poly_even_layer<CF, 32, 64>(X, H, wc, w2, W + OFF_C1 + W3264, W + OFF_SC + W3264S, zacc, sreg, wave, lane);
+#pragma unroll
+        for (int c = 0; c < 5; ++c) w3[0][c] = *(const f32x4*)(W + OFF_C2 + cb4 * (20 * 256) + lane * 4 + c * 256);
+    } else {
     if constexpr (F33) {
         load_weights<6>(w6, W + OFF_C1, cb4, lane);
     } else {
@@ -1363,6 +1509,7 @@
     if (tid < 32) ((f32x4*)H)[(tid & 15) + (tid >> 4) * (RS2 * G + 1) * 16] = f32x4{0.f, 0.f, 0.f, 0.f};
     conv_layer<CF, 32, 64, 3, 2, 1, RS1, RS2, L2, T2, MODE_PLAIN, false, GEOM_TRUNK, 16, RS2 * CF::G, false, SWX,
                BF16 ? SW_SPLIT : (F33 ? SW_3 : SWX)>(X, H, w6, nullptr, W + OFF_C1 + W3264, sreg, pad2, dump, wave, lane);
+    }
     const unsigned short* const WS16 = (const unsigned short*)(W + O::off_d(NB64)) + cb4 * 6144 + lane * 8;
     bf16x8 bwh[6], bwl[6];
     if constexpr (BF16) {
@@ -1373,6 +1520,7 @@
             bwh[st] = *(const bf16x8*)(WS16 + (st * 2) * 512);
             bwl[st] = *(const bf16x8*)(WS16 + (st * 2 + 1) * 512);
         }
+    } else if constexpr (POLY) {
     } else if constexpr (F33) {
         static_assert(!F33 || CF::NSREG >= 3 * (RS2 * CF::G / 48), "shortcut tiles kept in registers");
         conv_layer<CF, 32, 64, 1, 2, 0, RS1, RS2, L2, 3 * (RS2 * CF::G / 48), MODE_TO_REGS, false, GEOM_WTRIPLE, 16, RS2 * CF::G,
@@ -1491,52 +1639,71 @@
     }
 }
 
+template <class CF, bool STEM, int NB64, bool WINO, bool BF16 = false, bool BF16_32 = false, bool STAMP = false>
+__global__ __launch_bounds__(CF::THREADS, 2) void readconv_kernel(ReadConvArgs a) {
+    readconv_body<CF, STEM, NB64, WINO, BF16, BF16_32, STAMP>(a);
+}
+
+template <class CF, int NB64, int CH, bool STAMP = false>
+__global__ __launch_bounds__(CF::THREADS, 2) void readconv_poly_kernel(ReadConvArgs a) {
+    readconv_body<CF, true, NB64, true, false, false, STAMP, true, CH>(a);
+}
+
+using RcEntry = void (*)(ReadConvArgs);
+static hipError_t launch_entries(RcEntry stem, RcEntry trunk, RcEntry stamped, int reads_per_group, int threads, int lds_bytes,
+                                 bool (&configured_on)[64], bool (&stamped_on)[64], const ReadConvArgs& a, hipStream_t stream) {
+    int dev = 0;
+    if (hipGetDevice(&dev) != hipSuccess || dev < 0 || dev >= 64) return hipErrorInvalidDevice;
+    if (!configured_on[dev]) {
+        for (RcEntry k : {trunk, stem}) {
+            if (!k) continue;
+            const hipError_t e = hipFuncSetAttribute((const void*)k, hipFuncAttributeMaxDynamicSharedMemorySize, lds_bytes);
+            if (e != hipSuccess) return e;
+        }
+        configured_on[dev] = true;
+    }
+    if (a.groups_per_wg < 1) return hipErrorInvalidValue;
+    const long long per_wg = (long long)reads_per_group * a.groups_per_wg;
+    const unsigned groups = (unsigned)((a.n_reads + per_wg - 1) / per_wg);
+    if (a.stamps) {
+        if (!stamped || !a.reads || (a.channels != 6 && a.channels != 7) || a.stamp_groups < 1) return hipErrorInvalidValue;
+        if (!stamped_on[dev]) {
+            const hipError_t e = hipFuncSetAttribute((const void*)stamped, hipFuncAttributeMaxDynamicSharedMemorySize, 100 * 1024);
+            if (e != hipSuccess) return e;
+            stamped_on[dev] = true;
+        }
+        hipLaunchKernelGGL(stamped, dim3(groups), dim3(threads), (a.stamp_mode & 2) ? 100 * 1024 : lds_bytes, stream, a);
+        return hipGetLastError();
+    }
+    RcEntry k = trunk;
+    if (a.reads) {
+        if (a.channels != 6 && a.channels != 7) return hipErrorInvalidValue;
+        k = stem;
+    }
+    if (!k) return hipErrorInvalidValue;
+    hipLaunchKernelGGL(k, dim3(groups), dim3(threads), lds_bytes, stream, a);
+    return hipGetLastError();
+}
+
+template <int NB64, int CH>
+static hipError_t launch_poly(const ReadConvArgs& a, hipStream_t stream) {
+    using CF = Geometry;
+    static bool configured_on[64] = {}, stamped_on[64] = {};
+    RcEntry stamped = nullptr;
+    if constexpr (NB64 == 3) stamped = readconv_poly_kernel<CF, NB64, CH, true>;
+    return launch_entries(readconv_poly_kernel<CF, NB64, CH>, nullptr, stamped, CF::G, CF::THREADS, CF::LDS_BYTES, configured_on,
+                          stamped_on, a, stream);
+}
+
 template <class CF, int NB64, bool WINO, bool STEM_ONLY = false, bool BF16 = false, bool BF16_32 = false>
 static hipError_t launch_cfg(const ReadConvArgs& a, hipStream_t stream) {
-    static bool configured_on[64] = {};
-    int dev = 0;
-    if (hipGetDevice(&dev) != hipSuccess || dev < 0 || dev >= 64) return hipErrorInvalidDevice;
-    bool& configured = configured_on[dev];
-    if (!configured) {
-        hipError_t e = hipSuccess;
-        if constexpr (!STEM_ONLY)
-            e = hipFuncSetAttribute((const void*)readconv_kernel<CF, false, NB64, WINO, BF16, BF16_32>,
-                                    hipFuncAttributeMaxDynamicSharedMemorySize, CF::LDS_BYTES);
-        if (e == hipSuccess)
-            e = hipFuncSetAttribute((const void*)readconv_kernel<CF, true, NB64, WINO, BF16, BF16_32>,
-                                    hipFuncAttributeMaxDynamicSharedMemorySize, CF::LDS_BYTES);
-        if (e != hipSuccess) return e;
-        configured = true;
-    }
-    if (a.groups_per_wg < 1) return hipErrorInvalidValue;
-    const long long per_wg = (long long)CF::G * a.groups_per_wg;
-    const unsigned groups = (unsigned)((a.n_reads + per_wg - 1) / per_wg);
-    if (a.stamps) {
-        if constexpr (std::is_same<CF, Geometry>::value && NB64 == 3 && WINO && !BF16 && !STEM_ONLY) {
-            if (!a.reads || (a.channels != 6 && a.channels != 7) || a.stamp_groups < 1) return hipErrorInvalidValue;
-            static bool stamped_on[64] = {};
-            if (!stamped_on[dev]) {
-                const hipError_t e = hipFuncSetAttribute((const void*)readconv_kernel<CF, true, NB64, WINO, false, false, true>,
-                                                         hipFuncAttributeMaxDynamicSharedMemorySize, 100 * 1024);
-                if (e != hipSuccess) return e;
-                stamped_on[dev] = true;
-            }
-            const int lds = (a.stamp_mode & 2) ? 100 * 1024 : CF::LDS_BYTES;
-            hipLaunchKernelGGL((readconv_kernel<CF, true, NB64, WINO, false, false, true>), dim3(groups), dim3(CF::THREADS), lds, stream, a);
-            return hipGetLastError();
-        } else {
-            return hipErrorInvalidValue;
-        }
-    }
-    if (a.reads) {
-        if (a.channels != 6 && a.channels != 7) return hipErrorInvalidValue;
-        hipLaunchKernelGGL((readconv_kernel<CF, true, NB64, WINO, BF16, BF16_32>), dim3(groups), dim3(CF::THREADS), CF::LDS_BYTES, stream, a);
-    } else if constexpr (!STEM_ONLY) {
-        hipLaunchKernelGGL((readconv_kernel<CF, false, NB64, WINO, BF16, BF16_32>), dim3(groups), dim3(CF::THREADS), CF::LDS_BYTES, stream, a);
-    } else {
-        return hipErrorInvalidValue;
-    }
-    return hipGetLastError();
+    static bool configured_on[64] = {}, stamped_on[64] = {};
+    RcEntry trunk = nullptr, stamped = nullptr;
+    if constexpr (!STEM_ONLY) trunk = readconv_kernel<CF, false, NB64, WINO, BF16, BF16_32>;
+    if constexpr (std::is_same<CF, Geometry>::value && NB64 == 3 && WINO && !BF16 && !STEM_ONLY)
+        stamped = readconv_kernel<CF, true, NB64, WINO, false, false, true>;
+    return launch_entries(readconv_kernel<CF, true, NB64, WINO, BF16, BF16_32>, trunk, stamped, CF::G, CF::THREADS, CF::LDS_BYTES,
+                          configured_on, stamped_on, a, stream);
 }
 
 hipError_t launch_readconv_fused(const ReadConvArgs& a, hipStream_t stream) {
@@ -1554,6 +1721,12 @@
     if (a.softplus) {
         if (!a.reads || !a.winograd || a.extra_blocks != 0) return hipErrorInvalidValue;
         return launch_cfg<GeometrySoftplus, 3, true, true>(a, stream);
+    }
+    if (a.polyphase) {
+        if (!a.reads || !a.winograd || (a.channels != 6 && a.channels != 7)) return hipErrorInvalidValue;
+        if (a.extra_blocks == 0) return a.channels == 6 ? launch_poly<3, 6>(a, stream) : launch_poly<3, 7>(a, stream);
+        if (a.extra_blocks == 2) return a.channels == 6 ? launch_poly<5, 6>(a, stream) : launch_poly<5, 7>(a, stream);
+        return hipErrorInvalidValue;
     }
     if (a.extra_blocks == 0) return a.winograd ? launch_cfg<Geometry, 3, true>(a, stream) : launch_cfg<Geometry, 3, false>(a, stream);
     if (a.extra_blocks == 2) return a.winograd ? launch_cfg<Geometry, 5, true>(a, stream) : launch_cfg<Geometry, 5, false>(a, stream);
@@ -1599,14 +1772,16 @@
     static constexpr int OFF_11 = 0, OFF_S = OFF_11 + W11 + 64, OFF_SC = OFF_S + WS + 128, OFF_B = OFF_SC + WSC + 128;
     static constexpr int off_conv(int i) { return OFF_B + i * (WB + 128); }
     static constexpr int total(int blocks) { return off_conv(1 + 2 * blocks); }
+    static constexpr int POLY_W1 = 8 * 4 * 256, POLY_U = 8 * 4 * 4 * 256;
 };
 }
 
 int compressor_weight_floats(int blocks) { return cc::Cfg::total(blocks); }
+int compressor_polyphase_extra_floats() { return cc::Cfg::POLY_W1 + cc::Cfg::POLY_U; }
 bool compressor_supports_blocks(int blocks) { return blocks >= 2 && blocks <= 4; }
 
-template <int NB>
-__global__ __launch_bounds__(cc::Cfg::THREADS, 2) void compressor_kernel(CompressorArgs a) {
+template <int NB, bool POLY>
+__device__ __forceinline__ void compressor_body(const CompressorArgs& a) {
     using CF = cc::Cfg;
     constexpr int G = CF::G, L0 = CF::L0, L1 = CF::L1;
     extern __shared__ __attribute__((aligned(16))) float smem[];
@@ -1650,9 +1825,33 @@
     else
         conv_layer<CF, 64, 64, 1, 1, 0, L0, L0, L0, L0 * G / 16, MODE_PLAIN, false, GEOM_TRUNK, 16, L0 * G, false, SW_OLD, SW_W, true>(
             bufA, bufB, w11, nullptr, W + CF::OFF_11 + CF::W11, sreg, 0u, dump, wave, lane, 0, (live0 - wave / 4 + 1) / 2);
-    f32x4 ws[12], wsc[4];
+    f32x4 wsc[4];
+    load_weights<4>(wsc, W + CF::OFF_SC, wave, lane);
+    if constexpr (POLY) {
+        const float* const WP = W + CF::total(NB);
+        f32x4 wu[4][4], wc[4];
+#pragma unroll
+        for (int m = 0; m < 4; ++m)
+#pragma unroll
+            for (int c = 0; c < 4; ++c) wu[m][c] = *(const f32x4*)(WP + CF::POLY_W1 + (((wave * 4 + m) * 4 + c) * 64 + lane) * 4);
+        load_weights<4>(wc, WP, wave, lane);
+        __syncthreads();
+        if (tid < 64) ((f32x4*)bufA)[(tid & 31) + (tid >> 5) * (L1 * G + 1) * 32] = zero4;
+        f32x4 zacc[3][4];
+        if (full) {
+            poly_odd_layer<CF, 64, L1, true>(bufB, wu, zacc, lane);
+            poly_even_layer<CF, 64, 128>(bufB, bufA, wc, wsc, W + CF::OFF_S + CF::WS, W + CF::OFF_SC + CF::WSC, zacc, sreg, wave, lane);
+        } else {
+            const int live3 = (6 * n_here + 15) / 16;
+#pragma unroll
+            for (int t = 0; t < CF::NSREG; ++t) sreg[t] = zero4;
+            poly_odd_layer<CF, 64, L1, true, true>(bufB, wu, zacc, lane, live3);
+            poly_even_layer<CF, 64, 128, true>(bufB, bufA, wc, wsc, W + CF::OFF_S + CF::WS, W + CF::OFF_SC + CF::WSC, zacc, sreg, wave,
+                                               lane, live3);
+        }
+    } else {
+    f32x4 ws[12];
     load_weights<12>(ws, W + CF::OFF_S, wave, lane);
-    load_weights<4>(wsc, W + CF::OFF_SC, wave, lane);
     __syncthreads();
     if (tid < 64) ((f32x4*)bufA)[(tid & 31) + (tid >> 5) * (L1 * G + 1) * 32] = zero4;
     if (full)
@@ -1663,6 +1862,7 @@
             bufB, bufA, ws, nullptr, W + CF::OFF_S + CF::WS, sreg, 0u, dump, wave, lane, 0, live1);
     conv_layer<CF, 64, 128, 1, 2, 0, L0, L1, L1, CF::NSREG, MODE_TO_REGS, false, GEOM_WTRIPLE, 16, L1 * G, false, SW_W, SW_3>(
         bufB, nullptr, wsc, nullptr, W + CF::OFF_SC + CF::WSC, sreg, 0u, dump, wave, lane);
+    }
     f32x4 w3[2][5];
     auto slice = [&](int off) { return W + off + wave * (8 * 5 * 256) + lane * 4; };
 #pragma unroll
@@ -1703,6 +1903,15 @@
         dst[f] = *(const f32x4*)(bufB + img_off<128, SW_3>(1 + (f >> 5), f & 31));
 }
 
+template <int NB>
+__global__ __launch_bounds__(cc::Cfg::THREADS, 2) void compressor_kernel(CompressorArgs a) {
+    compressor_body<NB, false>(a);
+}
+template <int NB>
+__global__ __launch_bounds__(cc::Cfg::THREADS, 2) void compressor_poly_kernel(CompressorArgs a) {
+    compressor_body<NB, true>(a);
+}
+
 int small_launch_items_per_wg(long long n_items, int most) {
     const long long cus = device_cus();
     const long long n = (n_items + cus - 1) / cus;
@@ -1723,10 +1932,22 @@
             e = hipFuncSetAttribute((const void*)compressor_kernel<3>, hipFuncAttributeMaxDynamicSharedMemorySize, cc::Cfg::LDS_BYTES);
         if (e == hipSuccess)
             e = hipFuncSetAttribute((const void*)compressor_kernel<4>, hipFuncAttributeMaxDynamicSharedMemorySize, cc::Cfg::LDS_BYTES);
+        if (e == hipSuccess)
+            e = hipFuncSetAttribute((const void*)compressor_poly_kernel<2>, hipFuncAttributeMaxDynamicSharedMemorySize, cc::Cfg::LDS_BYTES);
+        if (e == hipSuccess)
+            e = hipFuncSetAttribute((const void*)compressor_poly_kernel<3>, hipFuncAttributeMaxDynamicSharedMemorySize, cc::Cfg::LDS_BYTES);
+        if (e == hipSuccess)
+            e = hipFuncSetAttribute((const void*)compressor_poly_kernel<4>, hipFuncAttributeMaxDynamicSharedMemorySize, cc::Cfg::LDS_BYTES);
         if (e != hipSuccess) return e;
         configured_on[dev] = true;
     }
     const unsigned grid = (unsigned)((a.n_items + a.items_per_wg - 1) / a.items_per_wg);
+    if (a.polyphase) {
+        if (a.blocks == 2) hipLaunchKernelGGL(compressor_poly_kernel<2>, dim3(grid), dim3(cc::Cfg::THREADS), cc::Cfg::LDS_BYTES, stream, a);
+        else if (a.blocks == 3) hipLaunchKernelGGL(compressor_poly_kernel<3>, dim3(grid), dim3(cc::Cfg::THREADS), cc::Cfg::LDS_BYTES, stream, a);
+        else hipLaunchKernelGGL(compressor_poly_kernel<4>, dim3(grid), dim3(cc::Cfg::THREADS), cc::Cfg::LDS_BYTES, stream, a);
+        return hipGetLastError();
+    }
     if (a.blocks == 2) hipLaunchKernelGGL(compressor_kernel<2>, dim3(grid), dim3(cc::Cfg::THREADS), cc::Cfg::LDS_BYTES, stream, a);
     else if (a.blocks == 3) hipLaunchKernelGGL(compressor_kernel<3>, dim3(grid), dim3(cc::Cfg::THREADS), cc::Cfg::LDS_BYTES, stream, a);
     else hipLaunchKernelGGL(compressor_kernel<4>, dim3(grid), dim3(cc::Cfg::THREADS), cc::Cfg::LDS_BYTES, stream, a);
diff --git a/hello_amd/engine.py b/hello_amd/engine.py
--- a/hello_amd/engine.py
+++ b/hello_amd/engine.py
@@ -127,13 +127,16 @@
 class Engine:
 
     def __init__(self, spec: ns.ModelSpec, state, device: int = 0, fused: bool = True, winograd: bool = True,
-                 program: Optional["compiler.Program"] = None, arithmetic: Optional[str] = None, lanes_max_sites: Optional[int] = None):
+                 program: Optional["compiler.Program"] = None, arithmetic: Optional[str] = None, lanes_max_sites: Optional[int] = None,
+                 strided: Optional[str] = None):
+        strided = strided or os.environ.get("HELLO_STRIDED") or "polyphase"
         self.lib = load_library()
         self.spec = spec
         self.lanes_max_sites = lanes_max_sites
-        self._lanes_recipe = None if program is not None else dict(state=state, fused=fused, winograd=winograd, arithmetic=arithmetic or "fp32")
+        self._lanes_recipe = None if program is not None else dict(state=state, fused=fused, winograd=winograd, arithmetic=arithmetic or "fp32",
+                                                                        strided=strided)
         if program is None:
-            program = compiler.compile_model(spec, state, fused=fused, winograd=winograd, arithmetic=arithmetic or "fp32")
+            program = compiler.compile_model(spec, state, fused=fused, winograd=winograd, arithmetic=arithmetic or "fp32", strided=strided)
         self.program = program
         p = self.program
         self.device = device
@@ -157,7 +160,8 @@
             return self.handle
         if self.lanes_handle is None:
             r = self._lanes_recipe
-            prog = compiler.compile_model(self.spec, r["state"], fused=r["fused"], winograd=r["winograd"], arithmetic=r["arithmetic"], lanes=True)
+            prog = compiler.compile_model(self.spec, r["state"], fused=r["fused"], winograd=r["winograd"], arithmetic=r["arithmetic"], lanes=True,
+                                          strided=r["strided"])
             if prog.n_lanes == 1:
                 self._lanes_recipe = None
                 return self.handle
diff --git a/hello_amd/readconv_pack.py b/hello_amd/readconv_pack.py
--- a/hello_amd/readconv_pack.py
+++ b/hello_amd/readconv_pack.py
@@ -69,6 +69,55 @@
         strided = t2 * 4 * 6 * 4 + t2 * 4 * 2 * 4 + t2 * 4 * 12 * 4
         blocks = 6 * (t1 * 2 * 6 * 4) + n64 * (t2 * 4 * 12 * 4)
     return (stem + strided + blocks) * 1024.0 / g
+
+
+STRIDED_FORMS = ("polyphase", "direct", "polyphase+compressor")
+
+
+def polyphase_available(winograd: bool, window: int, extra_blocks: int = 0, softplus: bool = False) -> bool:
+    return f33(winograd, window) and extra_blocks in EXTRA_BLOCKS and not softplus
+
+
+def polyphase_executed_macs_per_read(channels: int, extra_blocks: int = 0) -> float:
+    assert channels in (6, 7), channels
+    saved = (216 - (3 * 2 * 4 * 4 + 9 * 2 * 4)) + (10 if channels == 6 else 0)
+    return executed_macs_per_read(True, extra_blocks) - saved * 1024.0
+
+
+def polyphase_taps(w: np.ndarray, dtype=np.float32) -> np.ndarray:
+    g = w.astype(np.float64)
+    g0, g1 = g[..., 0], g[..., 2]
+    return np.stack([g0, (g0 + g1) / 2, (g0 - g1) / 2, g1], axis=-1).astype(dtype)
+
+
+def polyphase_reference(x: np.ndarray, w: np.ndarray, u: np.ndarray) -> np.ndarray:
+    x = np.asarray(x, np.float64)
+    cin, n = x.shape
+    lout = (n - 1) // 2 + 1
+    assert lout % 3 == 0, lout
+    o = np.zeros((cin, lout + 1))
+    odd = x[:, 1::2]
+    o[:, 1:1 + odd.shape[1]] = odd
+    e = x[:, 0::2]
+    uu = np.asarray(u, np.float64)
+    y = np.asarray(w, np.float64)[:, :, 1] @ e
+    for t in range(lout // 3):
+        d0, d1, d2, d3 = (o[:, 3 * t + i] for i in range(4))
+        m = [uu[:, :, 0] @ (d0 - d2), uu[:, :, 1] @ (d1 + d2), uu[:, :, 2] @ (d2 - d1), uu[:, :, 3] @ (d3 - d1)]
+        y[:, 3 * t] += m[0] + m[1] + m[2]
+        y[:, 3 * t + 1] += m[1] - m[2]
+        y[:, 3 * t + 2] += m[1] + m[2] + m[3]
+    return y
+
+
+def pack_polyphase(nodes, folded) -> np.ndarray:
+    w, b = folded[trunk_convs(nodes)[6].key]
+    assert w.shape == (64, 32, 3), w.shape
+    centre = _pack_conv(np.ascontiguousarray(w[:, :, 1:2]), b)[:4 * 2 * 256]
+    u = _pack_conv(polyphase_taps(w), b)[:4 * 4 * 2 * 256].reshape(4, 4, 2, 64, 4)
+    blob = np.concatenate([centre, u.transpose(0, 2, 1, 3, 4).ravel()])
+    assert blob.size == 2048 + 8192, blob.size
+    return blob
 
 
 def winograd_taps(w: np.ndarray) -> np.ndarray:
@@ -230,8 +279,19 @@
     return blob
 
 
-def compressor_executed_macs(blocks: int) -> float:
-    return 36 * 64 * 64 + 18 * 128 * 192 + 18 * 128 * 64 + (1 + 2 * blocks) * 6 * 5 * 128 * 128
+def compressor_executed_macs(blocks: int, polyphase: bool = False) -> float:
+    strided = (18 + 6 * 4) * 128 * 64 if polyphase else 18 * 128 * 192
+    return 36 * 64 * 64 + strided + 18 * 128 * 64 + (1 + 2 * blocks) * 6 * 5 * 128 * 128
+
+
+def pack_compressor_polyphase(nodes, folded) -> np.ndarray:
+    w, b = folded[nodes[1].body[0].key]
+    assert w.shape == (128, 64, 3), w.shape
+    centre = _pack_conv(np.ascontiguousarray(w[:, :, 1:2]), b)[:8 * 4 * 256]
+    u = _pack_conv(polyphase_taps(w), b)[:8 * 4 * 4 * 256].reshape(8, 4, 4, 64, 4)
+    blob = np.concatenate([centre, u.transpose(0, 2, 1, 3, 4).ravel()])
+    assert blob.size == 8192 + 32768, blob.size
+    return blob
 
 
 def wide_trunk_nodes(nodes, cin):
diff --git a/include/hello_mi355x.h b/include/hello_mi355x.h
--- a/include/hello_mi355x.h
+++ b/include/hello_mi355x.h
@@ -65,6 +65,7 @@
 #define HELLO_FLAG_BF16X3   64
 #define HELLO_FLAG_BF16X3_32 128
 #define HELLO_FLAG_MIX_REST 8
+#define HELLO_FLAG_POLYPHASE 2048
 #define HELLO_FLAG_LANE_SHIFT 8
 #define HELLO_FLAG_LANE_MASK  (7 << HELLO_FLAG_LANE_SHIFT)
 #define HELLO_MAX_LANES 8
```

New measurement: 495,200, median of 6. 1.01x the previous value.
